# refresh-bio/colord

Measured on AMD Instinct MI355X. Metric: input Gbases/s + archive size vs ref, ONT 50 Gb at 1/2/4/8 MI355X, higher is better.
Workload: dtype u64

## Files before the change

### colord_amd/_native.py

```python
from __future__ import annotations
import ctypes as C
import os

os.environ.setdefault("GPU_MAX_HW_QUEUES", "32")
_HERE = os.path.dirname(os.path.abspath(__file__))
LIB_PATH = os.environ.get("COLORD_HIP_LIBRARY") or os.path.join(_HERE, "libcolord_hip.so")

CL_OK, CL_E_INVALID, CL_E_HIP, CL_E_CAPACITY, CL_E_NOMEM, CL_E_UNSUPPORTED, CL_E_MISMATCH = 0, -1, -2, -3, -4, -5, -6


class ColordHipError(RuntimeError):
    def __init__(self, status, msg):
        super().__init__(f"colord_hip error {status}: {msg}")
        self.status = status


class QualParams(C.Structure):
    _fields_ = [("mode", C.c_int32), ("source", C.c_int32), ("level", C.c_int32), ("n_fwd", C.c_uint32), ("fwd", C.c_uint32 * 8),
                ("n_rev", C.c_uint32), ("rev", C.c_uint32 * 8)]


class KmerStats(C.Structure):
    _fields_ = [("n_reads", C.c_uint64), ("tot_kmers", C.c_uint64), ("n_unique", C.c_uint64),
                ("n_unique_counted", C.c_uint64), ("total_count_filtered", C.c_uint64)]
# ... 32 lines not shown


class PileupSums(C.Structure):
    _fields_ = [("covered", C.c_uint64), ("match", C.c_uint64), ("sub", C.c_uint64), ("del_", C.c_uint64), ("ins", C.c_uint64), ("ins_unplaced", C.c_uint64), ("reads", C.c_uint64)]
    NAMES = ("covered", "match", "sub", "del", "ins", "ins_unplaced", "reads")

    def as_dict(self):
        return {k: int(getattr(self, f[0])) for k, f in zip(self.NAMES, self._fields_)}


KSPEC_EXACT = 4096
class KSpec(C.Structure):
    _fields_ = [("kmers", C.c_uint64), ("distinct", C.c_uint64), ("max_count", C.c_uint64), ("exact", C.c_uint64 * KSPEC_EXACT),
                ("big", C.c_uint64 * 33), ("big_mass", C.c_uint64 * 33)]

    as_dict = Report.as_dict


class SketchEntry(C.Structure):
    _fields_ = [("hash", C.c_uint64), ("count", C.c_uint64)]


class Sketch:

    def __init__(self, size: int, min_count: int):
        self.lib, self.h = load(), _P()
        st = self.lib.cl_sketch_create(size, min_count, C.byref(self.h))
        if st != CL_OK:
            raise ColordHipError(st, "cl_sketch_create failed")

    def close(self):
        if self.h:
            self.lib.cl_sketch_free(self.h)
            self.h = None

    def __del__(self):
        try:
            self.close()
        except Exception:
            pass

    def info(self) -> dict:
        size, mc, q, n = C.c_uint32(0), C.c_uint32(0), C.c_uint64(0), C.c_uint64(0)
        st = self.lib.cl_sketch_info(self.h, C.byref(size), C.byref(mc), C.byref(q), C.byref(n))
        if st != CL_OK:
            raise ColordHipError(st, "cl_sketch_info failed")
        return {"size": size.value, "min_count": mc.value, "qualifying": q.value, "n": n.value}

    def entries(self):
        import numpy as np
        n = self.info()["n"]
        buf = np.zeros((n, 2), np.uint64)
        st = self.lib.cl_sketch_entries(self.h, buf.ctypes.data if n else None, n)
        if st != CL_OK:
            raise ColordHipError(st, "cl_sketch_entries failed")
        return buf[:, 0].copy(), buf[:, 1].copy()

    def as_dict(self) -> dict:
        d = self.info()
        d["hash"], d["count"] = self.entries()
        return d

    def merge(self, hashes, counts, qualifying: int):
        import numpy as np
        h, c = np.asarray(hashes, np.uint64), np.asarray(counts, np.uint64)
        assert h.shape == c.shape and h.ndim == 1
        buf = np.ascontiguousarray(np.stack([h, c], axis=1))
        st = self.lib.cl_sketch_merge(self.h, buf.ctypes.data if len(h) else None, len(h), qualifying)
        if st != CL_OK:
            raise ColordHipError(st, "cl_sketch_merge refused the entries")
        return self


class Overlap(C.Structure):
    _fields_ = [(k, C.c_uint32) for k in ("q", "t", "qlen", "tlen", "qs", "qe", "ts", "te", "matches", "subst", "anchor_bases", "flags")]


_P = C.c_void_p
class CompressParams(C.Structure):
    _fields_ = [("k", C.c_uint32), ("f", C.c_uint32), ("ci", C.c_uint32), ("cs", C.c_uint32), ("c", C.c_uint32),
                ("anchor_len", C.c_uint32), ("min_part_alt", C.c_uint32), ("max_rec", C.c_uint32), ("min_anchors", C.c_uint32),
                ("level", C.c_int32), ("source", C.c_int32), ("sparse", C.c_int32),
                ("sparse_g", C.c_double), ("sparse_exponent", C.c_double),
                ("cost_mult", C.c_double), ("frac_always", C.c_double), ("frac_min", C.c_double), ("max_matches_mult", C.c_double)]


class CompressInfo(C.Structure):
    _fields_ = [(n, C.c_uint64) for n in ("n_reads", "n_bases", "tot_kmers", "n_kept_kmers", "n_refs", "n_anchors", "tuple_bytes", "dna_bytes", "qual_bytes")] + \
               [("sparse_range", C.c_uint32), ("pad", C.c_uint32)]


_EXCH_GATHER_HOST = C.CFUNCTYPE(C.c_int32, C.c_void_p, C.POINTER(C.c_uint64), C.c_uint32, C.POINTER(C.c_uint64))
_EXCH_A2AV = C.CFUNCTYPE(C.c_int32, C.c_void_p, C.c_void_p, C.POINTER(C.c_uint64), C.c_void_p, C.POINTER(C.c_uint64))
_EXCH_GATHERV = C.CFUNCTYPE(C.c_int32, C.c_void_p, C.c_void_p, C.c_uint64, C.c_void_p, C.POINTER(C.c_uint64))


class Exchange(C.Structure):
    _fields_ = [("user", C.c_void_p), ("rank", C.c_uint32), ("world", C.c_uint32),
                ("all_gather_host", _EXCH_GATHER_HOST), ("all_to_all_v", _EXCH_A2AV), ("all_gather_v", _EXCH_GATHERV)]


_SIG = {
    "cl_ctx_create": (C.c_int32, [C.c_int, C.POINTER(_P)]),
    "cl_ctx_destroy": (None, [_P]),
    "cl_last_error": (C.c_char_p, [_P]),
    "cl_ctx_stream": (_P, [_P]),
    "cl_ctx_last_kernel_ms": (C.c_int32, [_P, C.c_char_p, C.POINTER(C.c_double), C.POINTER(C.c_uint32)]),
    "cl_ctx_set_timing": (None, [_P, C.c_int]),
    "cl_ctx_set_verify": (None, [_P, C.c_int]),
    "cl_ctx_verified": (C.c_int32, [_P, C.POINTER(C.c_uint64), C.POINTER(C.c_uint64)]),
    "cl_ctx_gap_paths": (C.c_int32, [_P, C.POINTER(C.c_uint64), C.c_uint32]),
    "cl_ctx_set_verify_streams": (None, [_P, C.c_int]),
    "cl_ctx_verified_streams": (C.c_int32, [_P, C.POINTER(C.c_uint64), C.POINTER(C.c_uint64), C.POINTER(C.c_uint64)]),
    "cl_compressor_verified_streams": (C.c_int32, [_P, C.POINTER(C.c_uint64), C.POINTER(C.c_uint64), C.POINTER(C.c_uint64)]),
    "cl_ctx_set_digest": (None, [_P, C.c_int]),
    "cl_ctx_digest": (C.c_int32, [_P, C.POINTER(Digest), C.POINTER(Digest)]),
    "cl_compressor_digest": (C.c_int32, [_P, C.POINTER(Digest), C.POINTER(Digest)]),
    "cl_ctx_set_digest_values": (None, [_P, C.c_int]),
    "cl_ctx_digest_values": (C.c_int32, [_P, C.POINTER(Digest)]),
    "cl_compressor_digest_values": (C.c_int32, [_P, C.POINTER(Digest)]),
    "cl_digest_qual_values": (C.c_int32, [_P, C.POINTER(QualParams), _P, _P, _P, C.c_uint64, C.POINTER(Digest)]),
    "cl_qual_values": (C.c_int32, [_P, C.POINTER(QualParams), _P, _P, _P, _P, C.c_uint64]),
    "cl_qual_values_host": (C.c_int32, [C.POINTER(QualParams), _P, _P, C.c_uint64, _P]),
    "cl_digest_qual_values_host": (C.c_int32, [_P, _P, C.c_uint64, C.c_uint64, C.POINTER(Digest)]),
    "cl_report_clear": (None, [C.POINTER(Report)]),
    "cl_report_add": (None, [C.POINTER(Report), C.POINTER(Report)]),
    "cl_report_bases": (C.c_int32, [_P, _P, C.POINTER(Report)]),
    "cl_report_quals": (C.c_int32, [_P, C.POINTER(QualParams), _P, _P, _P, C.c_uint64, C.c_uint32, C.POINTER(Report)]),
    "cl_report_bases_host": (C.c_int32, [_P, _P, C.c_uint64, C.POINTER(Report)]),
    "cl_report_quals_host": (C.c_int32, [C.POINTER(QualParams), _P, _P, C.c_uint64, C.POINTER(Report)]),
    "cl_report_values_host": (C.c_int32, [_P, _P, C.c_uint64, C.POINTER(Report)]),
    "cl_ctx_set_report": (None, [_P, C.c_int]),
    "cl_ctx_report": (C.c_int32, [_P, C.POINTER(Report)]),
    "cl_compressor_report": (C.c_int32, [_P, C.POINTER(Report)]),
    "cl_edits_clear": (None, [C.POINTER(Edits)]),
    "cl_edits_add": (None, [C.POINTER(Edits), C.POINTER(Edits)]),
    "cl_edit_profile": (C.c_int32, [_P, _P, _P, _P, C.c_uint32, C.c_uint64, C.c_uint32, C.POINTER(Edits)]),
    "cl_edit_profile_host": (C.c_int32, [_P, _P, C.c_uint32, _P, _P, C.c_uint64, C.POINTER(Edits), C.POINTER(C.c_uint64), C.POINTER(C.c_uint32)]),
    "cl_edit_profile_error": (C.c_char_p, [C.c_uint32]),
    "cl_ctx_set_edit_profile": (None, [_P, C.c_int]),
    "cl_ctx_edit_profile": (C.c_int32, [_P, C.POINTER(Edits)]),
    "cl_compressor_edit_profile": (C.c_int32, [_P, C.POINTER(Edits)]),
    "cl_kspec_clear": (None, [C.POINTER(KSpec)]),
    "cl_kspec_add": (None, [C.POINTER(KSpec), C.POINTER(KSpec)]),
    "cl_kmer_spectrum_heads": (C.c_int32, [_P, _P, C.c_uint64, C.c_uint64, C.c_uint32, C.POINTER(KSpec)]),
    "cl_ctx_set_kmer_spectrum": (None, [_P, C.c_int]),
    "cl_ctx_kmer_spectrum": (C.c_int32, [_P, C.POINTER(KSpec)]),
    "cl_compressor_kmer_spectrum": (C.c_int32, [_P, C.POINTER(KSpec)]),
    "cl_sketch_hash": (C.c_uint64, [C.c_uint64]),
    "cl_sketch_create": (C.c_int32, [C.c_uint32, C.c_uint32, C.POINTER(_P)]),
    "cl_sketch_free": (None, [_P]),
    "cl_sketch_info": (C.c_int32, [_P, C.POINTER(C.c_uint32), C.POINTER(C.c_uint32), C.POINTER(C.c_uint64), C.POINTER(C.c_uint64)]),
    "cl_sketch_entries": (C.c_int32, [_P, _P, C.c_uint64]),
    "cl_sketch_merge": (C.c_int32, [_P, _P, C.c_uint64, C.c_uint64]),
    "cl_kmer_sketch_runs": (C.c_int32, [_P, _P, _P, C.c_uint64, C.c_uint64, C.c_uint32, _P]),
    "cl_ctx_set_kmer_sketch": (C.c_int32, [_P, C.c_int, C.c_uint32, C.c_uint32]),
    "cl_ctx_kmer_sketch": (C.c_int32, [_P, _P]),
    "cl_compressor_kmer_sketch": (C.c_int32, [_P, _P]),
    "cl_overlaps_of": (C.c_int32, [_P, _P, _P, _P, C.c_uint32, C.c_uint64, _P, C.c_uint32, C.c_uint32, _P, C.c_uint64, C.POINTER(C.c_uint64)]),
    "cl_overlaps_host": (C.c_int32, [_P, _P, C.c_uint32, _P, _P, C.c_uint64, C.c_uint64, _P, C.c_uint32, _P, C.c_uint64, C.POINTER(C.c_uint64), C.POINTER(C.c_uint64),
                                     C.POINTER(C.c_uint32)]),
    "cl_ctx_set_overlaps": (None, [_P, C.c_int]),
    "cl_ctx_overlaps": (C.c_int32, [_P, _P, C.c_uint64, C.POINTER(C.c_uint64)]),
    "cl_compressor_overlaps": (C.c_int32, [_P, _P, C.c_uint64, C.POINTER(C.c_uint64)]),
    "cl_mappings_lift": (C.c_int32, [_P, _P, C.c_uint64, _P, C.c_uint32, C.c_uint32, C.c_uint32, _P, C.c_uint64, C.POINTER(C.c_uint64)]),
    "cl_mappings_lift_host": (C.c_int32, [_P, C.c_uint64, _P, C.c_uint32, C.c_uint32, C.c_uint32, _P, C.c_uint64, C.POINTER(C.c_uint64), C.POINTER(C.c_uint64), C.POINTER(C.c_uint32)]),
    "cl_ctx_set_mappings": (None, [_P, C.c_int]),
    "cl_ctx_mappings": (C.c_int32, [_P, _P, C.c_uint64, C.POINTER(C.c_uint64)]),
    "cl_compressor_mappings": (C.c_int32, [_P, _P, C.c_uint64, C.POINTER(C.c_uint64)]),
    "cl_cigars_of": (C.c_int32, [_P, _P, _P, _P, C.c_uint32, C.c_uint32, C.c_uint32, _P, C.c_uint64, C.POINTER(C.c_uint64), _P, C.c_uint64, C.POINTER(C.c_uint64)]),
    "cl_cigars_host": (C.c_int32, [_P, _P, C.c_uint32, _P, _P, C.c_uint64, C.c_uint32, _P, C.c_uint64, C.POINTER(C.c_uint64), _P, C.c_uint64, C.POINTER(C.c_uint64),
                                   C.POINTER(C.c_uint64), C.POINTER(C.c_uint32)]),
    "cl_cigars_error": (C.c_char_p, [C.c_uint32]),
    "cl_ctx_set_cigars": (C.c_int32, [_P, C.c_int]),
    "cl_ctx_cigars": (C.c_int32, [_P, _P, C.c_uint64, C.POINTER(C.c_uint64), _P, C.c_uint64, C.POINTER(C.c_uint64)]),
    "cl_compressor_cigars": (C.c_int32, [_P, _P, C.c_uint64, C.POINTER(C.c_uint64), _P, C.c_uint64, C.POINTER(C.c_uint64)]),
    "cl_compressor_genome_geometry": (C.c_int32, [_P, _P, C.c_uint32, C.c_uint32, C.c_uint32]),
    "cl_pileup_create": (C.c_int32, [_P, _P, _P, C.c_uint32, C.c_uint32, C.c_uint32, C.POINTER(_P)]),
    "cl_pileup_free": (None, [_P]),
    "cl_pileup_positions": (C.c_uint64, [_P]),
    "cl_pileup_add": (C.c_int32, [_P, _P, _P, _P, C.c_uint32, C.c_uint32]),
    "cl_pileup_finish": (C.c_int32, [_P]),
    "cl_pileup_columns": (C.c_int32, [_P, C.c_uint64, C.c_uint64, _P]),
    "cl_pileup_sites": (C.c_int32, [_P, C.c_uint32, C.c_uint32, C.c_uint32, _P, C.c_uint64, C.POINTER(C.c_uint64)]),
    "cl_pileup_totals": (C.c_int32, [_P, C.POINTER(PileupSums)]),
    "cl_pileup_host": (C.c_int32, [_P, _P, C.c_uint32, _P, C.c_uint32, C.c_uint32, C.c_uint32, _P, _P, C.c_uint64, C.c_uint32, C.c_uint32, C.c_uint32, _P, _P, C.c_uint64,
                                   C.POINTER(C.c_uint64), C.POINTER(PileupSums), C.POINTER(C.c_uint64), C.POINTER(C.c_uint32)]),
    "cl_ctx_set_pileup": (None, [_P, C.c_int]),
    "cl_compressor_pileup": (C.c_int32, [_P, C.POINTER(_P)]),
    "cl_digest_bases": (C.c_int32, [_P, _P, C.c_uint64, C.POINTER(Digest)]),
    "cl_digest_quals": (C.c_int32, [_P, C.POINTER(QualParams), _P, _P, _P, C.c_uint64, C.POINTER(Digest)]),
    "cl_digest_bases_host": (C.c_int32, [_P, _P, C.c_uint64, C.c_uint64, C.POINTER(Digest)]),
    "cl_digest_bytes_host": (C.c_int32, [C.c_uint32, _P, _P, C.c_uint64, C.c_uint64, C.POINTER(Digest)]),
    "cl_qual_decoder_set_digest": (C.c_int32, [_P, C.c_int, C.c_uint64]),
    "cl_qual_decoder_digest": (C.c_int32, [_P, C.POINTER(Digest)]),
    "cl_es_expand": (C.c_int32, [_P, _P, _P, _P, _P, C.c_uint32, _P, C.c_uint64, _P, C.POINTER(C.c_uint64)]),
    "cl_es_verify": (C.c_int32, [_P, _P, _P, _P, _P, _P, C.POINTER(C.c_uint64), C.POINTER(C.c_uint32)]),
    "cl_compressor_verified": (C.c_int32, [_P, C.POINTER(C.c_uint64), C.POINTER(C.c_uint64)]),
    "cl_ctx_kernel_times": (C.c_int32, [_P, C.c_char_p, C.c_uint64, C.POINTER(C.c_uint64)]),
    "cl_reads_pack": (C.c_int32, [_P, _P, _P, C.c_uint32, C.c_int, C.POINTER(_P)]),
    "cl_reads_free": (None, [_P]),
    "cl_reads_count": (C.c_uint32, [_P]),
    "cl_reads_total_bases": (C.c_uint64, [_P]),
    "cl_reads_total_words": (C.c_uint64, [_P]),
    "cl_reads_packed": (_P, [_P]),
    "cl_reads_invalid": (_P, [_P]),
    "cl_reads_word_offsets": (_P, [_P]),
    "cl_reads_lengths": (_P, [_P]),
    "cl_reads_has_n": (_P, [_P]),
    "cl_reads_compact": (C.c_int32, [_P, _P, C.c_uint32, _P, C.c_uint64, C.POINTER(C.c_uint64)]),
    "cl_kmer_scan": (C.c_int32, [_P, _P, C.c_uint32, C.c_uint32, _P, C.c_uint64, C.POINTER(C.c_uint64)]),
    "cl_kmer_count_filter": (C.c_int32, [_P, _P, C.c_uint64, C.c_uint32, C.c_uint32, C.c_uint32, C.POINTER(_P), C.POINTER(KmerStats)]),
    "cl_kmer_set_create": (C.c_int32, [_P, _P, _P, C.c_uint64, C.c_uint32, C.POINTER(_P)]),
    "cl_kmer_set_free": (None, [_P]),
    "cl_kmer_set_size": (C.c_uint64, [_P]),
    "cl_kmer_set_keys": (_P, [_P]),
    "cl_kmer_set_counts": (_P, [_P]),
    "cl_kmer_set_check": (C.c_int32, [_P, _P, _P, C.c_uint64, _P]),
    "cl_accepted_kmers": (C.c_int32, [_P, _P, _P, C.c_uint32, C.c_uint32, C.POINTER(_P)]),
    "cl_kmer_lists_free": (None, [_P]),
    "cl_kmer_lists_reads": (C.c_uint32, [_P]),
    "cl_kmer_lists_total": (C.c_uint64, [_P]),
    "cl_kmer_lists_offsets": (_P, [_P]),
    "cl_kmer_lists_kmers": (_P, [_P]),
    "cl_kmer_lists_ids": (_P, [_P]),
    "cl_kmer_lists_pos": (_P, [_P]),
    "cl_ref_accept": (C.c_int32, [C.c_uint32, C.c_uint32, C.c_uint32, C.c_double, _P]),
    "cl_index_build": (C.c_int32, [_P, _P, _P, _P, C.c_uint32, C.c_uint32, C.POINTER(_P)]),
    "cl_index_entries_of": (C.c_int32, [_P, _P, _P, C.c_uint32, _P, _P, C.c_uint64, C.POINTER(C.c_uint64), _P, C.POINTER(C.c_uint32)]),
    "cl_index_build_pairs": (C.c_int32, [_P, _P, _P, _P, C.c_uint64, _P, C.c_uint32, C.c_uint32, C.c_uint32, C.c_uint32, C.POINTER(_P)]),
    "cl_index_free": (None, [_P]),
    "cl_index_n_refs": (C.c_uint32, [_P]),
    "cl_index_entries": (C.c_uint64, [_P]),
    "cl_index_ref_rank": (_P, [_P]),
    "cl_candidates": (C.c_int32, [_P, _P, _P, C.c_uint32, _P, _P, _P]),
    "cl_candidates_common": (C.c_int32, [_P, _P, _P, C.c_uint32, _P, _P, _P, _P, C.c_uint64, C.POINTER(C.c_uint64)]),
    "cl_qual_coder_create": (C.c_int32, [_P, C.POINTER(QualParams), C.POINTER(_P)]),
    "cl_qual_coder_ctx": (_P, [_P]),
    "cl_qual_coder_free": (None, [_P]),
    "cl_qual_coder_set_domain_symbols": (C.c_int32, [_P, C.c_uint64]),
    "cl_qual_coder_domains": (C.c_int32, [_P, _P, C.c_uint64, C.POINTER(C.c_uint64)]),
    "cl_qual_coder_model": (C.c_int32, [_P, C.c_uint32, C.c_uint64, _P, C.c_uint32, C.POINTER(C.c_uint32)]),
    "cl_qual_coder_groups": (C.c_int32, [_P, C.POINTER(C.c_uint64)]),
    "cl_compressor_set_qual_domain_symbols": (C.c_int32, [_P, C.c_uint64]),
    "cl_compressor_qual_domains": (C.c_int32, [_P, _P, C.c_uint64, C.POINTER(C.c_uint64)]),
    "cl_qual_decode_domains": (C.c_int32, [_P, C.POINTER(QualParams), _P, _P, _P, C.c_uint64, _P, _P, C.c_uint32, _P, C.c_uint32, C.c_uint32, _P, _P, C.c_uint64, _P, C.c_uint64]),
    "cl_qual_encode": (C.c_int32, [_P, _P, _P, _P, _P, _P, _P, C.c_uint32, _P, C.c_uint64, _P, C.POINTER(C.c_uint64)]),
    "cl_anchor_candidates": (C.c_int32, [_P, _P, _P, _P, _P, C.c_uint32, C.c_uint32, C.c_double, C.c_double, C.c_double, C.c_uint32, C.POINTER(_P)]),
    "cl_anchor_candidates_hifi": (C.c_int32, [_P, _P, _P, _P, _P, C.c_uint32, C.c_uint32, C.c_double, C.c_double, C.c_double, C.c_uint32, C.c_uint32, C.c_uint32, _P, _P, C.POINTER(_P)]),
    "cl_anchors_free": (None, [_P]),
    "cl_anchors_total": (C.c_uint64, [_P]),
    "cl_anchors_wave_tasks": (C.c_uint64, [_P]),
    "cl_anchors_wave_pairs": (C.c_uint64, [_P]),
    "cl_anchors_lane_tasks": (C.c_uint64, [_P]),
    "cl_anchors_lane_pairs": (C.c_uint64, [_P]),
    "cl_anchors_n_cands": (_P, [_P]),
    "cl_anchors_cands": (_P, [_P]),
    "cl_anchors_cand_offsets": (_P, [_P]),
    "cl_anchors_data": (_P, [_P]),
    "cl_encode_plain": (C.c_int32, [_P, _P, _P, C.c_uint64, _P, _P, C.POINTER(C.c_uint64)]),
    "cl_reads_select": (C.c_int32, [_P, _P, _P, C.POINTER(_P)]),
    "cl_reads_from_arena": (C.c_int32, [_P, _P, _P, _P, C.c_uint32, C.POINTER(_P)]),
    "cl_estimator_logs": (C.c_int32, [_P, _P, _P, C.c_uint64, _P]),
    "cl_es_flags": (C.c_int32, [_P, _P, _P, _P, _P, _P]),
    "cl_id_coder_create": (C.c_int32, [C.c_int32, C.POINTER(_P)]),
    "cl_id_coder_free": (None, [_P]),
    "cl_id_coder_error": (C.c_char_p, [_P]),
    "cl_id_encode_part": (C.c_int32, [_P, _P, _P, _P, C.c_uint32, _P, C.c_uint64, C.POINTER(C.c_uint64)]),
    "cl_compress_shard": (C.c_int32, [_P, C.POINTER(CompressParams), _P, _P, _P, _P, C.c_uint32, _P, C.c_uint32, _P, _P, _P, C.c_uint64, _P, _P, C.c_uint64, _P,
                                      C.POINTER(CompressInfo)]),
    "cl_candidates_at": (C.c_int32, [_P, _P, _P, _P, C.c_uint32, _P, _P, _P]),
    "cl_compressor_create": (C.c_int32, [_P, _P, C.POINTER(CompressParams), C.POINTER(QualParams), C.POINTER(Exchange), C.c_uint64, C.POINTER(_P)]),
    "cl_compressor_free": (None, [_P]),
    "cl_compressor_count_add": (C.c_int32, [_P, _P]),
    "cl_compressor_count_finish": (C.c_int32, [_P, C.POINTER(KmerStats)]),
    "cl_compressor_refs_add": (C.c_int32, [_P, _P]),
    "cl_compressor_refs_finish": (C.c_int32, [_P]),
    "cl_compressor_encode": (C.c_int32, [_P, _P, _P, _P, _P, C.c_uint32, _P, C.c_uint32, _P, C.c_uint64, _P, _P, C.c_uint64, _P, C.POINTER(CompressInfo)]),
    "cl_compressor_genome_add": (C.c_int32, [_P, _P]),
    "cl_compressor_pseudo_reads": (C.c_int32, [_P, _P]),
    "cl_genome_encode": (C.c_int32, [_P, _P, C.c_uint32, _P, C.c_uint64, C.POINTER(C.c_uint64)]),
    "cl_genome_decode": (C.c_int32, [_P, C.c_uint64, C.c_uint32, _P, C.c_uint64, _P, C.POINTER(C.c_uint64)]),
    "cl_genome_md5": (C.c_int32, [_P, _P, C.c_uint32, _P]),
    "cl_compressor_prepare": (C.c_int32, [_P, _P, _P, C.c_uint32]),
    "cl_compressor_prepare_parts": (C.c_int32, [_P, _P, _P, C.c_uint32, _P, C.c_uint32, _P, _P]),
    "cl_compressor_info": (C.c_int32, [_P, C.POINTER(KmerStats), C.POINTER(C.c_uint64), C.POINTER(C.c_uint64), C.POINTER(C.c_uint64), C.POINTER(C.c_uint32), C.POINTER(C.c_uint32)]),
    "cl_dna_decoder_create": (C.c_int32, [C.c_uint32, C.c_int32, C.c_uint32, C.c_uint32, C.c_int32, C.c_uint32, C.c_double, C.POINTER(_P)]),
    "cl_dna_decoder_free": (None, [_P]),
    "cl_dna_decoder_error": (C.c_char_p, [_P]),
    "cl_dna_decoder_add_ref": (C.c_int32, [_P, _P, C.c_uint32]),
    "cl_dna_decoder_new_domain": (C.c_int32, [_P]),
    "cl_dna_decode_part": (C.c_int32, [_P, _P, C.c_uint64, C.c_uint32, _P, C.c_uint64, _P, C.POINTER(C.c_uint64)]),
    "cl_qual_decoder_create": (C.c_int32, [C.POINTER(QualParams), C.POINTER(_P)]),
    "cl_qual_decoder_free": (None, [_P]),
    "cl_qual_decoder_new_domain": (C.c_int32, [_P]),
    "cl_qual_decode_part": (C.c_int32, [_P, _P, C.c_uint64, _P, _P, C.c_uint32, _P]),
    "cl_id_decoder_create": (C.c_int32, [C.c_int32, C.POINTER(_P)]),
    "cl_id_decoder_free": (None, [_P]),
    "cl_id_decode_part": (C.c_int32, [_P, _P, C.c_uint64, C.c_uint32, _P, C.c_uint64, _P, _P, C.POINTER(C.c_uint64)]),
    "cl_encode_reads": (C.c_int32, [_P, _P, _P, _P, C.c_uint32, C.c_uint32, C.c_uint32, C.c_uint32, C.c_double, _P, C.c_uint32, _P, C.c_uint64, _P, _P, C.POINTER(C.c_uint64)]),
    "cl_dna_coder_create": (C.c_int32, [_P, C.c_uint32, C.c_int32, C.c_uint32, C.POINTER(_P)]),
    "cl_dna_coder_free": (None, [_P]),
    "cl_dna_coder_model": (C.c_int32, [_P, C.c_uint32, C.c_uint64, _P]),
    "cl_dna_encode": (C.c_int32, [_P, _P, _P, _P, _P, _P, C.c_uint32, _P, C.c_uint32, _P, C.c_uint64, _P, C.POINTER(C.c_uint64)]),
    "cl_sort_u64": (C.c_int32, [_P, _P, C.c_uint64, C.c_uint32, C.c_uint32]),
    "cl_sort_u64_u32": (C.c_int32, [_P, _P, _P, C.c_uint64, C.c_uint32, C.c_uint32]),
    "cl_sort_u32": (C.c_int32, [_P, _P, C.c_uint64, C.c_uint32, C.c_uint32]),
    "cl_sort_u32_u32": (C.c_int32, [_P, _P, _P, C.c_uint64, C.c_uint32, C.c_uint32]),
    "cl_sort_swap_u32_u32": (C.c_int32, [_P, _P, _P, C.c_uint64, C.c_uint32, C.c_uint32, _P, _P]),
    "cl_sort_swap_u64_u32": (C.c_int32, [_P, _P, _P, C.c_uint64, C.c_uint32, C.c_uint32, _P, _P]),
    "cl_scan_u32": (C.c_int32, [_P, _P, C.c_uint64, C.POINTER(C.c_uint64)]),
    "cl_scan_u32_u64": (C.c_int32, [_P, _P, _P, C.c_uint64, C.POINTER(C.c_uint64)]),
    "cl_run_starts_u32": (C.c_int32, [_P, _P, C.c_uint64, C.c_uint32, _P, C.c_uint64, C.POINTER(C.c_uint64)]),
    "cl_run_starts_u64": (C.c_int32, [_P, _P, C.c_uint64, C.c_uint32, _P, C.c_uint64, C.POINTER(C.c_uint64)]),
}

_lib = None


def load():
    global _lib
    if _lib is None:
        if not os.path.exists(LIB_PATH):
            raise ColordHipError(CL_E_HIP, f"{LIB_PATH} is missing: run `make -C colord_amd/csrc` "
                                 "(or __graft_entry__.build()); there is no CPU fallback")
        lib = C.CDLL(LIB_PATH)
        for name, (res, args) in _SIG.items():
            fn = getattr(lib, name)
            fn.restype, fn.argtypes = res, args
        _lib = lib
    return _lib


def exported_names():
    return sorted(_SIG)
```

### colord_amd/csrc/capi.hip

```cpp
#include "common.hpp"
#include "objects.hpp"
#include "sketch.hpp"
#include <cmath>
#include <random>

extern "C" cl_status cl_ctx_create(int device, cl_ctx** out)
{
	if (!out) return CL_E_INVALID;
	*out = nullptr;
	int n = 0;
	hipError_t e = hipGetDeviceCount(&n);
	if (e != hipSuccess || n <= 0) { fprintf(stderr, "colord_hip: no HIP device available (%s)\n", hipGetErrorString(e)); return CL_E_HIP; }
	if (device < 0 || device >= n) return CL_E_INVALID;
	if (hipSetDevice(device) != hipSuccess) return CL_E_HIP;
	cl_ctx* c = new cl_ctx(device);
	if (hipStreamCreateWithFlags(&c->stream, hipStreamNonBlocking) != hipSuccess) { cl_ctx_destroy(c); return CL_E_HIP; }
	hipDeviceProp_t p;
	if (hipGetDeviceProperties(&p, device) == hipSuccess) c->n_cu = p.multiProcessorCount;
	*out = c;
	return CL_OK;
}
void cl_ctx_set_priority(cl_ctx* c, int level, int role)
{
	if (!c) return;
	(void)hipSetDevice(c->device);
	int least = 0, greatest = 0;
	if (hipDeviceGetStreamPriorityRange(&least, &greatest) != hipSuccess) { (void)hipGetLastError(); least = greatest = 0; }
	level = cl_role_level(role >= 0 ? role : c->role, level);
	const int prio = level > 0 ? greatest : level < 0 ? least : 0;
	const bool role_changes = role >= 0 && role < CL_N_ROLES && cl_cu_mask_cfg().on[role] && (role != c->role || !c->masked);
	if (role >= 0) c->role = role;
	if (prio == c->prio && !role_changes) return;
	c->prio = prio; c->masked = c->role < CL_N_ROLES && cl_cu_mask_cfg().on[c->role];
	auto drop_scan_ctl = [&](hipStream_t old) {
		auto it = c->scan_ctl.find((void*)old);
		if (it == c->scan_ctl.end()) return;
		if (it->second.p) c->pool.put(it->second.p, it->second.got, c->pool_id);
		c->scan_ctl.erase(it);
	};
	if (c->stream)
	{
		(void)hipStreamSynchronize(c->stream); drop_scan_ctl(c->stream); (void)hipStreamDestroy(c->stream); c->stream = nullptr;
		if (cl_stream_create(c, &c->stream) != hipSuccess) { (void)hipGetLastError(); (void)hipStreamCreateWithFlags(&c->stream, hipStreamNonBlocking); }
	}
	for (std::atomic<hipStream_t>* s : { &c->side, &c->side2, &c->side3 })
		if (hipStream_t old = s->load())
		{
			(void)hipStreamSynchronize(old); drop_scan_ctl(old); (void)hipStreamDestroy(old);
			hipStream_t ns = nullptr;
			if (cl_stream_create(c, &ns) != hipSuccess) { (void)hipGetLastError(); (void)hipStreamCreateWithFlags(&ns, hipStreamNonBlocking); }
			s->store(ns);
		}
}
namespace { __global__ void k_poison_check(const uint32_t* __restrict__ p, uint64_t n, unsigned long long* __restrict__ bad)
{
	uint64_t mine = 0;
	for (uint64_t i = (uint64_t)blockIdx.x * blockDim.x + threadIdx.x; i < n; i += (uint64_t)gridDim.x * blockDim.x) mine += p[i] != 0xCDCDCDCDu;
	if (mine) atomicAdd(bad, (unsigned long long)mine);
} }
void cl_ctx_poison(cl_ctx* c, void* p, uint64_t bytes)
{
	if (!c || !c->stream) return;
	(void)hipSetDevice(c->device);
	if (hipMemsetAsync(p, 0xCD, bytes, c->stream) != hipSuccess) { (void)hipGetLastError(); return; }
	(void)hipStreamSynchronize(c->stream);
}
uint64_t cl_pool_poison_check(void* p, uint64_t bytes)
{
	static unsigned long long* d_bad = nullptr;
	if (!d_bad && hipMalloc((void**)&d_bad, 8) != hipSuccess) { (void)hipGetLastError(); return 0; }
	(void)hipDeviceSynchronize();
	(void)hipMemset(d_bad, 0, 8);
	hipLaunchKernelGGL(k_poison_check, dim3(1024), dim3(256), 0, nullptr, (const uint32_t*)p, bytes / 4, d_bad);
	unsigned long long h = 0;
	if (hipGetLastError() != hipSuccess || hipMemcpy(&h, d_bad, 8, hipMemcpyDeviceToHost) != hipSuccess) { (void)hipGetLastError(); fprintf(stderr, "colord_hip: pool poison: the check itself failed\n"); return 0; }
	return h;
}
void cl_ctx_drain(cl_ctx* c)
{
	if (!c) return;
	(void)hipSetDevice(c->device);
	for (hipStream_t s : { c->stream, c->side.load(std::memory_order_acquire), c->side2.load(std::memory_order_acquire), c->side3.load(std::memory_order_acquire) }) if (s) (void)hipStreamSynchronize(s);
}
int cl_ctx_fence(cl_ctx* c, hipEvent_t* ev)
{
	if (!c) return 0;
	int n = 0;
	for (hipStream_t s : { c->stream, c->side.load(std::memory_order_acquire), c->side2.load(std::memory_order_acquire), c->side3.load(std::memory_order_acquire) }) if (s && n < 4) { if (hipEventRecord(ev[n], s) == hipSuccess) ++n; else (void)hipGetLastError(); }
	return n;
}
extern "C" void cl_ctx_destroy(cl_ctx* c)
{
	if (!c) return;
	for (cl_ctx* l : c->lanes) cl_ctx_destroy(l);
	c->lanes.clear();
	if (c->prep) { cl_ctx_destroy(c->prep); c->prep = nullptr; }
	if (c->qprep) { cl_ctx_destroy(c->qprep); c->qprep = nullptr; }
	(void)hipSetDevice(c->device);
	cl_ctx_drain(c);
	for (auto& kv : c->scan_ctl) if (kv.second.p) c->pool.put(kv.second.p, kv.second.got, c->pool_id);
	c->scan_ctl.clear();
	c->pool.drop_owner(c->pool_id);
	for (auto& p : c->pending) { (void)hipEventDestroy(p.second.first); (void)hipEventDestroy(p.second.second); }
	for (auto e : c->ev_pool) (void)hipEventDestroy(e);
	if (c->stream) (void)hipStreamDestroy(c->stream);
	for (std::atomic<hipStream_t>* s : { &c->side, &c->side2, &c->side3 }) if (hipStream_t x = s->load()) (void)hipStreamDestroy(x);
	if (c->inv_tab) (void)hipFree(c->inv_tab);
	if (c->slots_h) (void)hipHostFree(c->slots_h);
	delete c->report_acc;
	delete c->edits_acc;
	delete c->kspec_acc;
	delete c->sketch_acc;
	const int dev = c->device;
	delete c;
	cl_device_pool_release(dev);
}
extern "C" const char* cl_last_error(const cl_ctx* c) { return c ? c->err.c_str() : "null context"; }
extern "C" void* cl_ctx_stream(cl_ctx* c) { return c ? (void*)c->stream : nullptr; }
extern "C" void cl_ctx_set_timing(cl_ctx* c, int on) { if (c) c->timing = on != 0; }
extern "C" void cl_ctx_set_verify(cl_ctx* c, int on) { if (c) c->verify = on != 0; }
extern "C" cl_status cl_ctx_verified(const cl_ctx* c, uint64_t* reads, uint64_t* bases)
{
	if (!c) return CL_E_INVALID;
	uint64_t r = c->verified_reads.load(), b = c->verified_bases.load();
	for (const cl_ctx* l : c->lanes) { r += l->verified_reads.load(); b += l->verified_bases.load(); }
	if (reads) *reads = r;
	if (bases) *bases = b;
	return CL_OK;
}
extern "C" cl_status cl_ctx_gap_paths(const cl_ctx* c, uint64_t* out, uint32_t cap)
{
	if (!c || (!out && cap)) return CL_E_INVALID;
	for (uint32_t i = 0; i < cap && i < 11; ++i) out[i] = c->gap_paths[i];
	return CL_OK;
}
extern "C" cl_status cl_dna_coder_model(const cl_dna_coder* d, uint32_t family, uint64_t context, uint32_t* out)
{
	if (!d || !out) return CL_E_INVALID;
	return cl_dna_model_read(d, family, context, out);
}
extern "C" cl_status cl_qual_coder_model(const cl_qual_coder* q, uint32_t family, uint64_t context, uint32_t* out, uint32_t cap, uint32_t* n_out)
{
	if (!q || !out || !n_out) return CL_E_INVALID;
	return cl_qual_model_read(q, family, context, out, cap, n_out);
}
extern "C" void cl_ctx_set_verify_streams(cl_ctx* c, int on) { if (c) c->verify_streams = on != 0; }
extern "C" cl_status cl_ctx_verified_streams(const cl_ctx* c, uint64_t* parts, uint64_t* symbols, uint64_t* bytes)
{
	if (!c) return CL_E_INVALID;
	if (parts) *parts = c->verified_stream_parts.load();
	if (symbols) *symbols = c->verified_stream_symbols.load();
	if (bytes) *bytes = c->verified_stream_bytes.load();
	return CL_OK;
}
extern "C" cl_status cl_ctx_last_kernel_ms(const cl_ctx* c, const char* kernel, double* ms, uint32_t* launches)
{
	if (!c || !kernel) return CL_E_INVALID;
	auto it = c->times.find(kernel);
	if (it == c->times.end()) { if (ms) *ms = 0; if (launches) *launches = 0; return CL_E_INVALID; }
	if (ms) *ms = it->second.ms;
	if (launches) *launches = it->second.launches;
	return CL_OK;
}

extern "C" cl_status cl_ctx_kernel_times(cl_ctx* c, char* buf, uint64_t cap, uint64_t* needed)
{
	if (!c) return CL_E_INVALID;
	cl_timing_collect(c);
	std::string out;
	for (auto& kv : c->times) out += kv.first + "\t" + std::to_string(kv.second.ms) + "\t" + std::to_string(kv.second.launches) + "\t" + std::to_string(kv.second.bytes) + "\t" + std::to_string(kv.second.cells) + "\n";
	if (needed) *needed = out.size() + 1;
	if (!buf || cap < out.size() + 1) return CL_E_CAPACITY;
	memcpy(buf, out.c_str(), out.size() + 1);
	c->times.clear();
	return CL_OK;
}

extern "C" cl_status cl_ref_accept(uint32_t n_reads, uint32_t n_pseudo, uint32_t range, double exponent, uint8_t* h_out)
{
	if (!h_out || range == 0) return CL_E_INVALID;
	std::mt19937 mt;
	std::uniform_real_distribution<double> dist(0.0, 1.0);
	for (uint64_t i = 0; i < (uint64_t)n_reads + n_pseudo; ++i)
	{
		if (i < n_pseudo) { h_out[i] = 1; continue; }
		uint32_t range_no = (uint32_t)((i - n_pseudo) / range);
		double p = std::pow(1.0 / (range_no + 1ul), exponent);
		h_out[i] = dist(mt) <= p;
	}
	return CL_OK;
}

extern "C" cl_status cl_sort_u64(cl_ctx* ctx, uint64_t* d_keys, uint64_t n, uint32_t begin_bit, uint32_t end_bit)
{
	if (!ctx || (!d_keys && n)) return cl_fail(ctx, CL_E_INVALID, "cl_sort_u64: null argument");
	HIP_TRY(ctx, hipSetDevice(ctx->device));
	cl_timing_begin(ctx);
	cl_status s = dev_sort_pairs(ctx, d_keys, nullptr, n, begin_bit, end_bit);
	cl_timing_collect(ctx);
	return s;
}
extern "C" cl_status cl_sort_u64_u32(cl_ctx* ctx, uint64_t* d_keys, uint32_t* d_vals, uint64_t n, uint32_t begin_bit, uint32_t end_bit)
{
	if (!ctx || ((!d_keys || !d_vals) && n)) return cl_fail(ctx, CL_E_INVALID, "cl_sort_u64_u32: null argument");
	HIP_TRY(ctx, hipSetDevice(ctx->device));
	cl_timing_begin(ctx);
	cl_status s = dev_sort_pairs(ctx, d_keys, d_vals, n, begin_bit, end_bit);
	cl_timing_collect(ctx);
	return s;
}

extern "C" cl_status cl_scan_u32(cl_ctx* ctx, uint32_t* d_data, uint64_t n, uint64_t* h_total)
{
	if (!ctx || (!d_data && n)) return cl_fail(ctx, CL_E_INVALID, "cl_scan_u32: null argument");
	HIP_TRY(ctx, hipSetDevice(ctx->device));
	cl_timing_begin(ctx);
	cl_status s = dev_exclusive_scan_u32(ctx, d_data, n, h_total);
	hipError_t e = hipStreamSynchronize(ctx->stream);
	cl_timing_collect(ctx);
	if (s == CL_OK) HIP_TRY(ctx, e);
	return s;
}
extern "C" cl_status cl_scan_u32_u64(cl_ctx* ctx, const uint32_t* d_in, uint64_t* d_out, uint64_t n, uint64_t* h_total)
{
	if (!ctx || !d_out || (!d_in && n)) return cl_fail(ctx, CL_E_INVALID, "cl_scan_u32_u64: null argument");
	HIP_TRY(ctx, hipSetDevice(ctx->device));
	cl_timing_begin(ctx);
	cl_status s = dev_exclusive_scan_u64(ctx, d_in, d_out, n, h_total);
	hipError_t e = hipStreamSynchronize(ctx->stream);
	cl_timing_collect(ctx);
	if (s == CL_OK) HIP_TRY(ctx, e);
	return s;
}
extern "C" cl_status cl_run_starts_u32(cl_ctx* ctx, const uint32_t* d_keys, uint64_t n, uint32_t shift, uint32_t* d_seg, uint64_t seg_cap, uint64_t* h_n_runs)
{
	if (!ctx || !h_n_runs || ((!d_keys || !d_seg) && n)) return cl_fail(ctx, CL_E_INVALID, "cl_run_starts_u32: null argument");
	HIP_TRY(ctx, hipSetDevice(ctx->device));
	cl_timing_begin(ctx);
	cl_status s = dev_run_starts_u32(ctx, d_keys, n, shift, d_seg, seg_cap, h_n_runs);
	cl_timing_collect(ctx);
	return s;
}
extern "C" cl_status cl_run_starts_u64(cl_ctx* ctx, const uint64_t* d_keys, uint64_t n, uint32_t shift, uint32_t* d_seg, uint64_t seg_cap, uint64_t* h_n_runs)
{
	if (!ctx || !h_n_runs || ((!d_keys || !d_seg) && n)) return cl_fail(ctx, CL_E_INVALID, "cl_run_starts_u64: null argument");
	HIP_TRY(ctx, hipSetDevice(ctx->device));
	cl_timing_begin(ctx);
	cl_status s = dev_run_starts_u64(ctx, d_keys, n, shift, d_seg, seg_cap, h_n_runs);
	cl_timing_collect(ctx);
	return s;
}
extern "C" cl_status cl_sort_u32(cl_ctx* ctx, uint32_t* d_keys, uint64_t n, uint32_t begin_bit, uint32_t end_bit)
{
	return cl_sort_u32_u32(ctx, d_keys, nullptr, n, begin_bit, end_bit);
}
extern "C" cl_status cl_sort_u32_u32(cl_ctx* ctx, uint32_t* d_keys, uint32_t* d_vals, uint64_t n, uint32_t begin_bit, uint32_t end_bit)
{
	if (!ctx || (!d_keys && n)) return cl_fail(ctx, CL_E_INVALID, "cl_sort_u32_u32: null argument");
	HIP_TRY(ctx, hipSetDevice(ctx->device));
	cl_timing_begin(ctx);
	cl_status s = dev_sort_keys32_pairs(ctx, d_keys, d_vals, n, begin_bit, end_bit);
	cl_timing_collect(ctx);
	return s;
}
namespace {
template<typename K, typename Sort>
cl_status sort_swap_copy(cl_ctx* ctx, const char* who, const K* d_keys_in, const uint32_t* d_vals_in, uint64_t n, uint32_t begin_bit, uint32_t end_bit, K* d_keys_out, uint32_t* d_vals_out, Sort sort)
{
	if (!ctx || ((!d_keys_in || !d_vals_in || !d_keys_out || !d_vals_out) && n)) return cl_fail(ctx, CL_E_INVALID, std::string(who) + ": null argument");
	HIP_TRY(ctx, hipSetDevice(ctx->device));
	cl_timing_begin(ctx);
	DevBuf<K> keys; DEV_ALLOC(ctx, keys, n);
	DevBuf<uint32_t> vals; DEV_ALLOC(ctx, vals, n);
	if (n)
	{
		HIP_TRY(ctx, hipMemcpyAsync(keys.p, d_keys_in, n * sizeof(K), hipMemcpyDeviceToDevice, ctx->stream));
		HIP_TRY(ctx, hipMemcpyAsync(vals.p, d_vals_in, n * 4, hipMemcpyDeviceToDevice, ctx->stream));
	}
	cl_status s = sort(ctx, keys, vals, n, begin_bit, end_bit);
	if (s == CL_OK && n)
	{
		HIP_TRY(ctx, hipMemcpyAsync(d_keys_out, keys.p, n * sizeof(K), hipMemcpyDeviceToDevice, ctx->stream));
		HIP_TRY(ctx, hipMemcpyAsync(d_vals_out, vals.p, n * 4, hipMemcpyDeviceToDevice, ctx->stream));
	}
	hipError_t e = hipStreamSynchronize(ctx->stream);
	cl_timing_collect(ctx);
	if (s == CL_OK) HIP_TRY(ctx, e);
	return s;
}
}
extern "C" cl_status cl_sort_swap_u32_u32(cl_ctx* ctx, const uint32_t* d_keys_in, const uint32_t* d_vals_in, uint64_t n, uint32_t begin_bit, uint32_t end_bit, uint32_t* d_keys_out, uint32_t* d_vals_out)
{
	return sort_swap_copy<uint32_t>(ctx, "cl_sort_swap_u32_u32", d_keys_in, d_vals_in, n, begin_bit, end_bit, d_keys_out, d_vals_out, dev_sort_keys32_pairs_swap);
}
extern "C" cl_status cl_sort_swap_u64_u32(cl_ctx* ctx, const uint64_t* d_keys_in, const uint32_t* d_vals_in, uint64_t n, uint32_t begin_bit, uint32_t end_bit, uint64_t* d_keys_out, uint32_t* d_vals_out)
{
	return sort_swap_copy<uint64_t>(ctx, "cl_sort_swap_u64_u32", d_keys_in, d_vals_in, n, begin_bit, end_bit, d_keys_out, d_vals_out, dev_sort_pairs_swap);
}
```

### colord_amd/csrc/dna.hip

```cpp
#include "common.hpp"
#include <functional>
#include "objects.hpp"
#include "rc_dev.hpp"
#include "rc_check.hpp"
#include "es_format.hpp"
#include <algorithm>
#include <deque>
#include <thread>
#include <chrono>

namespace {
enum { F_READ_TYPE = 0, F_REV_COMP, F_SEEN, F_LEN_BITS, F_LEN_DATA, F_SYMBOLS, F_SYMBOLS_N, F_READ_ID, F_READ_ID_SHORT,
       F_ANCHOR_LEN, F_SKIP_LOCAL, F_SKIP_DISTANT, F_TUPLE_TYPE, N_FAM };
constexpr uint32_t MAX_ALT = 64;

struct FamTab {
	uint32_t n_sym[N_FAM], max_total[N_FAM], adder[N_FAM];
	uint32_t ctx_base[N_FAM + 1];
	uint64_t state_base[N_FAM + 1];
	uint32_t n_ctx[N_FAM];
	int32_t level, T, S;
	uint32_t sym_B;
	uint32_t max_alt;
	uint32_t long_run;
// ... 384 lines not shown
			break;
		case T_SUBST:
		{
			const uint32_t rs = ref_symbol & 3;
			const uint32_t sym = (rs == 0) ? (v1 == 0 ? 1u : v1 == 1 ? 2u : 3u) : (rs == 1) ? (v1 == 0 ? 0u : v1 == 1 ? 2u : 3u)
			                   : (rs == 2) ? (v1 == 0 ? 0u : v1 == 1 ? 1u : 3u) : (v1 == 0 ? 0u : v1 == 1 ? 1u : 2u);
			uint32_t shift = 2, c = 1;
			c += (uint32_t)(ctx_symbol & 0x3f) << shift; shift += 6;
			if (ft.level == 3) { c += (uint32_t)(((ctx_symbol >> 6) & 3) == ((ctx_symbol >> 4) & 3)) << shift; ++shift; }
			c += rs << shift; shift += 2;
			c += (uint32_t)(ctx_tuple & 07777) << shift;
			em(F_SYMBOLS, c, sym, (int)rs);
			ctx_symbol = ((ctx_symbol << 2) + sym) & mask_symbol; ++known;
			if (is_main) ++ref_pos; else ++alt_pos;
			break;
		}
		case T_SKIP:
		{
			const int32_t skip_len = (int32_t)v2;
			delta -= skip_len;
			if (!is_main && last_type == T_ALT_ID)
			{
				const int32_t mod = skip_len - (alt_slot >= 0 ? alt_pos_of[alt_slot] : 0);
				if (mod > 0) emit_skip_len(em, (uint32_t)mod, false);
				else { emit_skip_len(em, 0, false); emit_skip_len(em, (uint32_t)(-mod), false); }
			}
			else emit_skip_len(em, (uint32_t)skip_len, last_type != T_ALT_ID && last_type != T_NONE);
			if (is_main) ref_pos += v2; else alt_pos += v2;
			break;
		}
		case T_MAIN_REF:
			is_main = true;
			if (alt_slot >= 0) alt_pos_of[alt_slot] = (int32_t)alt_pos;
			delta = 0;
			break;
		default: break;
		}
		last_type = type;
	}
	em.finish();
	if (!WRITE)
	{
		hdr_counts[r] = em.count; counts[r] = em.count;
		if (t_idx != ntup - 1 && err) atomicOr(err, 2u);
	}
}

__global__ void k_read_flags(const uint8_t* __restrict__ es, const uint64_t* __restrict__ es_off, uint32_t r0, uint32_t r1, uint8_t* __restrict__ flag)
{
	uint32_t r = r0 + blockIdx.x * blockDim.x + threadIdx.x;
	if (r >= r1) return;
	uint32_t t = es[es_off[r]] >> 4;
	flag[r - r0] = t == T_START_PLAIN ? 0 : t == T_START_PLAIN_N ? 1 : 2;
}

__global__ __launch_bounds__(256) void k_fill_sidx(const uint64_t* __restrict__ sym_off, uint64_t s0, uint32_t r0, uint32_t r1, TripLayoutDev lay, uint32_t* __restrict__ sidx)
{
	const uint32_t r = r0 + blockIdx.x * 4 + (threadIdx.x >> 6);
	if (r >= r1) return;
	const uint32_t lane = threadIdx.x & 63;
	const uint64_t a = sym_off[r] - s0, b = sym_off[r + 1] - s0;
	if (a == b) return;
	const uint32_t part = part_of_read(lay, r), pl = lay.rank ? lay.rank[part] : part;
	const uint64_t gb = lay.group_base[pl >> 6], p0 = lay.part_sym_start[part];
	for (uint64_t i = a + lane; i < b; i += 64) sidx[i] = (uint32_t)trip_slot(gb, pl & 63, i - p0);
}
template<typename K>
__global__ __launch_bounds__(256) void k_dna_plain(const FamTab* __restrict__ ftp, const uint8_t* __restrict__ es, const uint64_t* __restrict__ es_off,
                                                  const uint32_t* __restrict__ es_ntup, const uint8_t* __restrict__ read_flag, const uint32_t* __restrict__ hdr_counts,
                                                  const uint64_t* __restrict__ sym_off, uint32_t r0, uint32_t r1, K* __restrict__ key)
{
	const uint32_t r = r0 + blockIdx.x * 4 + (threadIdx.x >> 6);
	if (r >= r1) return;
	const uint32_t fl = read_flag[r - r0];
	if (fl == 2) return;
	const FamTab& ft = *ftp;
	const uint32_t lane = threadIdx.x & 63;
	const uint8_t* b = es + es_off[r] + 1;
	const uint32_t len = es_ntup[r] - 1;
	const uint64_t off = sym_off[r - r0] + hdr_counts[r - r0];
	const uint32_t S2 = 2 * ft.S; const uint32_t mask = (1u << S2) - 1;
	const uint32_t fam = fl == 0 ? F_SYMBOLS : F_SYMBOLS_N;
	const uint32_t cbase = ft.ctx_base[fam];
	for (uint32_t i = lane; i < len; i += 64)
	{
		uint32_t ctx = mask;
		if (fl == 0)
		{
			const uint32_t n = i < (uint32_t)ft.S ? i : (uint32_t)ft.S;
			for (uint32_t t = n; t >= 1; --t) ctx = ((ctx << 2) + (b[i - t] & 3u)) & mask;
			ctx <<= 2;
		}
		else
		{
			const uint32_t n = i < 4 ? i : 4;
			for (uint32_t t = n; t >= 1; --t) ctx = ((ctx << 4) + (b[i - t] & 0xfu)) & mask;
		}
		key[off + i] = KeyFmt<K>::make(cbase + ctx, b[i] & 0xfu);
	}
}


constexpr uint32_t LONG_RUN = 1u << 19;
struct LongRun { uint32_t s, e, fam, gctx; uint64_t step0, group0, epoch0; uint32_t epoch_cap, pad; };
template<int NS> struct EpochRec { uint32_t start, tot; uint32_t st[NS]; uint32_t cnt0[NS]; };
__device__ inline uint32_t find_run(const LongRun* runs, uint32_t n_runs, uint64_t step)
{
	uint32_t lo = 0, hi = n_runs;
	while (hi - lo > 1) { const uint32_t mid = (lo + hi) >> 1; if (runs[mid].step0 <= step) lo = mid; else hi = mid; }
	return lo;
}
template<typename K>
__global__ void k_long_find(const uint32_t* __restrict__ seg_start, uint32_t n_seg, const K* __restrict__ skey, const FamTab* __restrict__ ftp, LongRun* __restrict__ runs , uint32_t cap, uint32_t* __restrict__ n_runs )
{
	const uint32_t sg = blockIdx.x * blockDim.x + threadIdx.x;
	if (sg >= n_seg) return;
	const uint32_t s = seg_start[sg], e = seg_start[sg + 1];
	const FamTab& ft = *ftp;
	if (e - s < ft.long_run) return;
	const uint32_t gctx = KeyFmt<K>::ctx(skey[s]);
	uint32_t fam = 0;
	for (uint32_t f = 1; f < N_FAM; ++f) if (gctx >= ft.ctx_base[f]) fam = f;
	if (ft.n_sym[fam] > 32) return;
	const uint32_t which = ft.n_sym[fam] > 8 ? 1u : 0u;
	const uint32_t i = atomicAdd(n_runs + which, 1u);
	if (i < cap) { LongRun r; r.s = s; r.e = e; r.fam = fam; r.gctx = gctx; r.step0 = r.group0 = r.epoch0 = 0; r.epoch_cap = 0; r.pad = 0; runs[which * cap + i] = r; }
}
template<int NS, typename K>
__global__ __launch_bounds__(256) void k_long_hist(const LongRun* __restrict__ runs, uint32_t n_runs, uint64_t n_groups, const K* __restrict__ skey,
                                                  uint32_t* __restrict__ step_pfx, uint32_t* __restrict__ group_tot)
{
	const uint64_t g = ((uint64_t)blockIdx.x * blockDim.x + threadIdx.x) >> 6; const uint32_t lane = threadIdx.x & 63;
	if (g >= n_groups) return;
	uint32_t lo = 0, hi = n_runs;
	while (hi - lo > 1) { const uint32_t mid = (lo + hi) >> 1; if (runs[mid].group0 <= g) lo = mid; else hi = mid; }
	const LongRun R = runs[lo];
	const uint64_t gl = g - R.group0;
	const uint32_t smask = key_sym_mask(R.fam);
	uint32_t c[NS];
#pragma unroll
	for (int a = 0; a < NS; ++a) c[a] = 0;
	for (uint32_t k = 0; k < 64; ++k)
	{
		const uint64_t j = (uint64_t)R.s + (gl * 64 + k) * 64 + lane;
		const bool valid = j < R.e;
		const uint32_t sym = valid ? (uint32_t)skey[j] & smask : 0xffu;
#pragma unroll
		for (uint32_t a = 0; a < NS; ++a) { const uint32_t n = (uint32_t)__popcll(__ballot(sym == a)); if (lane == k) c[a] = n; }
	}
	const uint64_t n_steps = ((uint64_t)(R.e - R.s) + 63) / 64;
	const uint64_t step = R.step0 + gl * 64 + lane;
#pragma unroll
	for (uint32_t a = 0; a < NS; ++a)
	{
		const uint32_t incl = wave_incl_scan(c[a]);
		if (gl * 64 + lane < n_steps) step_pfx[step * NS + a] = incl - c[a];
		if (lane == 63) group_tot[g * NS + a] = incl;
	}
}
template<int NS>
__global__ __launch_bounds__(64) void k_long_groups(const LongRun* __restrict__ runs, uint32_t n_runs, uint32_t* __restrict__ group_tot )
{
	const uint32_t r = blockIdx.x, lane = threadIdx.x;
	if (r >= n_runs) return;
	const LongRun R = runs[r];
	const uint64_t n_steps = ((uint64_t)(R.e - R.s) + 63) / 64, n_groups = (n_steps + 63) / 64;
	uint32_t carry[NS];
#pragma unroll
	for (int a = 0; a < NS; ++a) carry[a] = 0;
	for (uint64_t g0 = 0; g0 < n_groups; g0 += 64)
	{
		const uint64_t g = g0 + lane; const bool valid = g < n_groups;
#pragma unroll
		for (uint32_t a = 0; a < NS; ++a)
		{
			const uint32_t v = valid ? group_tot[(R.group0 + g) * NS + a] : 0u;
			const uint32_t incl = wave_incl_scan(v);
			if (valid) group_tot[(R.group0 + g) * NS + a] = carry[a] + incl - v;
			carry[a] += __shfl(incl, 63);
		}
	}
}
template<int NS, typename K>
__device__ inline uint32_t long_prefix(const LongRun& R, const K* skey, const uint32_t* step_pfx, const uint32_t* group_pfx, uint32_t x, uint32_t lane)
{
	const uint32_t smask = key_sym_mask(R.fam);
	const uint64_t step = x >> 6; const uint32_t off = x & 63;
	const uint32_t a = lane & (NS - 1);
	uint32_t v = group_pfx[(R.group0 + (step >> 6)) * NS + a] + (step * 64 < (uint64_t)(R.e - R.s) || off ? step_pfx[(R.step0 + step) * NS + a] : 0u);
	if (x == R.e - R.s && off == 0)
	{
		const uint64_t last = step - 1;
		const uint64_t j = (uint64_t)R.s + last * 64 + lane; const uint32_t sym = j < R.e ? (uint32_t)skey[j] & smask : 0xffu;
		uint32_t mine = 0;
#pragma unroll
		for (uint32_t b = 0; b < NS; ++b) { const uint32_t n = (uint32_t)__popcll(__ballot(sym == b)); if (a == b) mine = n; }
		return group_pfx[(R.group0 + (last >> 6)) * NS + a] + step_pfx[(R.step0 + last) * NS + a] + mine;
	}
	if (off)
	{
		const uint64_t j = (uint64_t)R.s + step * 64 + lane; const uint32_t sym = j < R.e ? (uint32_t)skey[j] & smask : 0xffu;
		const uint64_t below = (1ULL << off) - 1;
		uint32_t mine = 0;
#pragma unroll
		for (uint32_t b = 0; b < NS; ++b) { const uint32_t n = (uint32_t)__popcll(__ballot(sym == b) & below); if (a == b) mine = n; }
		v += mine;
	}
	return v;
}
template<int NS, typename K>
__global__ __launch_bounds__(64) void k_long_epochs(const FamTab* __restrict__ ftp, const LongRun* __restrict__ runs, uint32_t n_runs, const K* __restrict__ skey,
                                                   const uint32_t* __restrict__ step_pfx, const uint32_t* __restrict__ group_pfx, uint32_t* __restrict__ state,
                                                   EpochRec<NS>* __restrict__ epochs, uint32_t* __restrict__ n_epochs, uint32_t* __restrict__ group_epoch, uint32_t* __restrict__ err)
{
	const uint32_t r = blockIdx.x, lane = threadIdx.x;
	if (r >= n_runs) return;
	const LongRun R = runs[r];
	const FamTab& ft = *ftp;
	const uint32_t n_sym = ft.n_sym[R.fam], max_total = ft.max_total[R.fam], adder = ft.adder[R.fam];
	uint32_t* sp = state + ft.state_base[R.fam] + (uint64_t)(R.gctx - ft.ctx_base[R.fam]) * (n_sym + 1);
	const uint32_t L = R.e - R.s;
	uint32_t st = lane < n_sym ? sp[lane] : 0u, tot = sp[n_sym];
	uint32_t cnt0 = 0, p = 0, ne = 0;
	EpochRec<NS>* E = epochs + R.epoch0;
	for (;;)
	{
		if (ne >= R.epoch_cap) { if (lane == 0) atomicOr(err, 8u); break; }
		if (lane < NS) { E[ne].st[lane] = st; E[ne].cnt0[lane] = cnt0; }
		if (lane == 0) { E[ne].start = p; E[ne].tot = tot; }
		++ne;
		const uint32_t rr = (max_total - tot + adder - 1) / adder;
		if ((uint64_t)p + rr > L) break;
		p += rr;
		const uint32_t c1 = long_prefix<NS, K>(R, skey, step_pfx, group_pfx, p, lane);
		st += adder * (c1 - cnt0); cnt0 = c1;
		tot += adder * rr;
		while (tot >= max_total)
		{
			st = (st + 1) / 2;
			uint32_t sm = lane < NS ? st : 0u;
			for (int o = NS / 2; o; o >>= 1) sm += __shfl_xor(sm, o);
			tot = __shfl(sm, 0);
		}
		if (p == L) { if (lane < NS && ne < R.epoch_cap) { E[ne].st[lane] = st; E[ne].cnt0[lane] = cnt0; } if (lane == 0 && ne < R.epoch_cap) { E[ne].start = p; E[ne].tot = tot; } ++ne; break; }
	}
	const uint32_t cl = long_prefix<NS, K>(R, skey, step_pfx, group_pfx, L, lane);
	if (p < L) { st += adder * (cl - cnt0); tot += adder * (L - p); }
	if (lane < n_sym) sp[lane] = st;
	if (lane == 0) { sp[n_sym] = tot; n_epochs[r] = ne; }
	__builtin_amdgcn_s_waitcnt(0);
	__builtin_amdgcn_fence(__ATOMIC_SEQ_CST, "workgroup");
	const uint64_t n_groups = (((uint64_t)L + 63) / 64 + 63) / 64;
	for (uint64_t g0 = 0; g0 < n_groups; g0 += 64)
	{
		const uint64_t g = g0 + lane;
		if (g >= n_groups) continue;
		const uint32_t pos = (uint32_t)(g * 4096);
		uint32_t lo = 0, hi = ne;
		while (hi - lo > 1) { const uint32_t mid = (lo + hi) >> 1; if (E[mid].start <= pos) lo = mid; else hi = mid; }
		group_epoch[R.group0 + g] = lo;
	}
}
template<int NS, typename K>
__global__ __launch_bounds__(256) void k_long_apply(const LongRun* __restrict__ runs, uint32_t n_runs, uint64_t n_steps, const K* __restrict__ skey, const uint32_t* __restrict__ sval,
                                                   const uint32_t* __restrict__ step_pfx, const uint32_t* __restrict__ group_pfx, const EpochRec<NS>* __restrict__ epochs,
                                                   const uint32_t* __restrict__ n_epochs, const uint32_t* __restrict__ group_epoch, const FamTab* __restrict__ ftp, triple_t* __restrict__ trip)
{
	const uint64_t step = ((uint64_t)blockIdx.x * blockDim.x + threadIdx.x) >> 6; const uint32_t lane = threadIdx.x & 63;
	if (step >= n_steps) return;
	const uint32_t ri = find_run(runs, n_runs, step);
	const LongRun R = runs[ri];
	const uint32_t adder = ftp->adder[R.fam];
	const uint64_t sl = step - R.step0;
	const uint32_t x0 = (uint32_t)(sl * 64), x = x0 + lane;
	const uint64_t j = (uint64_t)R.s + x; const bool valid = j < R.e;
	uint32_t sym = 0xffu, e1 = 15u, e2 = 15u;
	if (valid) key_decode(R.fam, KeyFmt<K>::payload(skey[j]), sym, e1, e2);
	uint64_t m[NS];
#pragma unroll
	for (uint32_t a = 0; a < NS; ++a) m[a] = __ballot(sym == a);
	const EpochRec<NS>* E = epochs + R.epoch0; const uint32_t ne = n_epochs[ri];
	uint32_t e = group_epoch[R.group0 + (sl >> 6)];
	while (e + 1 < ne && E[e + 1].start <= x0) ++e;
	uint32_t me = e;
	while (me + 1 < ne && E[me + 1].start <= x) ++me;
	if (!valid) return;
	const EpochRec<NS>& ep = E[me];
	const uint64_t lt = (1ULL << lane) - 1;
	uint32_t cum = 0, freq = 0, excl = 0;
#pragma unroll
	for (uint32_t a = 0; a < NS; ++a)
	{
		const uint32_t pre = group_pfx[(R.group0 + (sl >> 6)) * NS + a] + step_pfx[step * NS + a] + (uint32_t)__popcll(m[a] & lt);
		const uint32_t v = ep.st[a] + adder * (pre - ep.cnt0[a]);
		const bool ex = NS <= 8 && (a == e1 || a == e2);
		if (ex) excl += v;
		if (a < sym && !ex) cum += v;
		if (a == sym) freq = v;
	}
	trip[sval[j]] = pack_triple(cum, freq, ep.tot + adder * (x - ep.start) - excl);
}

template<typename K>
__global__ __launch_bounds__(256) void k_dna_evolve(const FamTab* __restrict__ ftp, const K* __restrict__ skey, const uint32_t* __restrict__ sval,
                                                   const uint32_t* __restrict__ seg_start, uint32_t n_seg, uint32_t* __restrict__ state, triple_t* __restrict__ trip)
{
	__shared__ uint32_t s_cnt[4][256];
	__shared__ uint32_t s_pre[4][256];
	const uint32_t w = threadIdx.x >> 6, lane = threadIdx.x & 63;
	const uint32_t sg = blockIdx.x * 4 + w;
	if (sg >= n_seg) return;
	const uint32_t s = seg_start[sg], e = seg_start[sg + 1];
	const FamTab& ft = *ftp;
	const uint32_t gctx = KeyFmt<K>::ctx(skey[s]);
	uint32_t fam = 0;
	for (uint32_t f = 1; f < N_FAM; ++f) if (gctx >= ft.ctx_base[f]) fam = f;
	const uint32_t n_sym = ft.n_sym[fam], max_total = ft.max_total[fam], adder = ft.adder[fam];
	uint32_t* sp = state + ft.state_base[fam] + (uint64_t)(gctx - ft.ctx_base[fam]) * (n_sym + 1);
	const uint64_t lt = (1ULL << lane) - 1;
	if (n_sym <= 8)
	{
		if (e - s >= ft.long_run) return;
		uint32_t st[8]; uint32_t tot = sp[n_sym];
#pragma unroll
		for (uint32_t a = 0; a < 8; ++a) st[a] = a < n_sym ? sp[a] : 0u;
		for (uint32_t j0 = s; j0 < e; j0 += 64)
		{
			const uint32_t j = j0 + lane; const bool valid = j < e;
			uint32_t sym = 0xffu, e1 = 15u, e2 = 15u;
			if (valid) key_decode(fam, KeyFmt<K>::payload(skey[j]), sym, e1, e2);
			const uint32_t dst = valid ? sval[j] : 0u;
			uint64_t m[8];
#pragma unroll
			for (uint32_t a = 0; a < 8; ++a) m[a] = __ballot(valid && sym == a);
			const uint32_t cnt = (e - j0) < 64 ? (e - j0) : 64;
			uint32_t start = 0;
			while (start < cnt)
			{
				const uint32_t r = (max_total - tot + adder - 1) / adder;
				const uint32_t now = (cnt - start) < r ? (cnt - start) : r;
				const uint64_t win = (now == 64 ? ~0ULL : ((1ULL << now) - 1)) << start;
				if (lane >= start && lane < start + now)
				{
					const uint64_t before = lt & win;
					uint32_t cum = 0, freq = 0, excl = 0;
#pragma unroll
					for (uint32_t a = 0; a < 8; ++a)
					{
						const uint32_t v = st[a] + adder * (uint32_t)__popcll(m[a] & before);
						const bool ex = a == e1 || a == e2;
						if (ex) excl += v;
						if (a < sym && !ex) cum += v;
						if (a == sym) freq = v;
					}
					trip[dst] = pack_triple(cum, freq, tot + adder * (lane - start) - excl);
				}
#pragma unroll
				for (uint32_t a = 0; a < 8; ++a) st[a] += adder * (uint32_t)__popcll(m[a] & win);
				tot += adder * now;
				while (tot >= max_total)
				{
					tot = 0;
#pragma unroll
					for (uint32_t a = 0; a < 8; ++a) { st[a] = (st[a] + 1) / 2; tot += st[a]; }
				}
				start += now;
			}
		}
		if (lane == 0)
		{
			for (uint32_t a = 0; a < n_sym; ++a) sp[a] = st[a];
			sp[n_sym] = tot;
		}
		return;
	}
	if (n_sym <= 32 && e - s >= ft.long_run) return;
	uint32_t* cnt = s_cnt[w]; uint32_t* pre = s_pre[w];
#pragma unroll
	for (uint32_t t = 0; t < 4; ++t) { uint32_t a = lane * 4 + t; cnt[a] = a < n_sym ? sp[a] : 0u; }
	uint32_t tot = sp[n_sym];
	auto rebuild_prefix = [&]() {
		uint32_t v0 = cnt[lane * 4], v1 = cnt[lane * 4 + 1], v2 = cnt[lane * 4 + 2], v3 = cnt[lane * 4 + 3];
		uint32_t sum = v0 + v1 + v2 + v3;
		uint32_t ex = wave_incl_scan(sum) - sum;
		pre[lane * 4] = ex; pre[lane * 4 + 1] = ex + v0; pre[lane * 4 + 2] = ex + v0 + v1; pre[lane * 4 + 3] = ex + v0 + v1 + v2;
		__builtin_amdgcn_wave_barrier();
	};
	__builtin_amdgcn_wave_barrier();
	rebuild_prefix();
	for (uint32_t j0 = s; j0 < e; j0 += 64)
	{
		const uint32_t j = j0 + lane; const bool valid = j < e;
		const uint32_t sym = valid ? KeyFmt<K>::payload(skey[j]) : 0u;
		const uint32_t dst = valid ? sval[j] : 0u;
		const uint32_t n_here = (e - j0) < 64 ? (e - j0) : 64;
		uint32_t start = 0;
		while (start < n_here)
		{
			const uint32_t r = (max_total - tot + adder - 1) / adder;
			const uint32_t now = (n_here - start) < r ? (n_here - start) : r;
			uint32_t less = 0, eq = 0;
			for (uint32_t l = start; l < start + now; ++l)
			{
				const uint32_t o = __builtin_amdgcn_readlane(sym, l);
				if (l < lane) { less += (o < sym) ? 1u : 0u; eq += (o == sym) ? 1u : 0u; }
			}
			const bool mine = lane >= start && lane < start + now;
			if (mine) trip[dst] = pack_triple(pre[sym] + adder * less, cnt[sym] + adder * eq, tot + adder * (lane - start));
			__builtin_amdgcn_wave_barrier();
			if (mine) atomicAdd(&cnt[sym], adder);
			__builtin_amdgcn_wave_barrier();
			tot += adder * now;
			while (tot >= max_total)
			{
				uint32_t sum = 0;
#pragma unroll
				for (uint32_t t = 0; t < 4; ++t) { uint32_t a = lane * 4 + t; if (a < n_sym) { uint32_t v = (cnt[a] + 1) / 2; cnt[a] = v; sum += v; } }
				tot = wave_sum(sum);
			}
			__builtin_amdgcn_wave_barrier();
			rebuild_prefix();
			start += now;
		}
	}
#pragma unroll
	for (uint32_t t = 0; t < 4; ++t) { uint32_t a = lane * 4 + t; if (a < n_sym) sp[a] = cnt[a]; }
	if (lane == 0) sp[n_sym] = tot;
}

__global__ void k_init_fam_state(const FamTab* __restrict__ ftp, uint32_t fam, uint32_t* __restrict__ state)
{
	const FamTab& ft = *ftp;
	const uint32_t ns = ft.n_sym[fam];
	const uint64_t n = (uint64_t)ft.n_ctx[fam] * (ns + 1);
	for (uint64_t i = (uint64_t)blockIdx.x * blockDim.x + threadIdx.x; i < n; i += (uint64_t)gridDim.x * blockDim.x)
		state[ft.state_base[fam] + i] = (i % (ns + 1)) == ns ? ns : 1u;
}
__global__ void k_gather_bytes2(const uint8_t* __restrict__ src, const uint64_t* __restrict__ src_off, const uint64_t* __restrict__ dst_off,
                                const uint64_t* __restrict__ size, uint8_t* __restrict__ dst)
{
	const uint32_t p = blockIdx.x;
	const uint64_t n = size[p]; const uint8_t* s = src + src_off[p]; uint8_t* d = dst + dst_off[p];
	for (uint64_t i = threadIdx.x; i < n; i += blockDim.x) d[i] = s[i];
}
__global__ void k_last_types(const uint8_t* __restrict__ flag, uint32_t n, uint32_t prev, uint32_t* __restrict__ out)
{
	uint32_t v = prev;
	uint32_t start = n > 4 ? n - 4 : 0;
	for (uint32_t i = start; i < n; ++i) v = ((v << 2) + flag[i]) & 0xff;
	*out = v;
}
}

struct DnaGroupPrep {
	uint32_t p0 = 0, p1 = 0, r0 = 0, r1 = 0; uint64_t s0 = 0, n_syms = 0, n_seg = 0, trip_words = 0;
	std::vector<uint32_t> rank, plen_r;
	DevBuf<uint64_t> d_gbase; DevBuf<uint32_t> d_plen;
	DevBuf<uint32_t> sidx, seg;
	struct LongPrep { uint32_t n_runs = 0; uint64_t steps = 0, groups = 0, eps = 0; DevBuf<LongRun> runs; DevBuf<uint32_t> step_pfx, group_pfx; } lp[2];
	bool long_ready = false;
};
struct DnaWalked {
	const uint8_t* d_es = nullptr; uint32_t n_reads = 0;
	uint32_t prev_types_in = 0, cur_read_id_in = 0, prev_types_out = 0;
	DevBuf<uint8_t> rflag; DevBuf<uint32_t> hdr; DevBuf<uint64_t> sym_off, key; DevBuf<uint32_t> key32; bool narrow = false;
	std::vector<uint64_t> h_sym_off;
	bool presorted = false; std::vector<uint32_t> part_bounds; std::vector<std::unique_ptr<DnaGroupPrep>> groups;
};
struct cl_dna_coder {
	cl_ctx* ctx = nullptr;
	FamTab ft;
	DevBuf<FamTab> d_ft;
	DevBuf<uint32_t> state;
	uint32_t ctx_bits = 0; bool narrow = false;
	uint32_t cur_read_id = 0;
	uint32_t prev_types = 0;
	uint32_t next_read_id = 0, next_prev_types = 0; bool next_valid = false;
	std::unique_ptr<DnaWalked> ahead;
	std::function<cl_status()> before_tail;
	std::deque<std::unique_ptr<struct DnaEvolved>> evolved;
	uint32_t ahead_prev_types = 0, ahead_read_id = 0;
	std::vector<hipStream_t> cstreams; uint32_t next_cstream = 0;
	~cl_dna_coder();
};

extern "C" cl_status cl_dna_coder_create(cl_ctx* ctx, uint32_t max_alt_refs, int32_t level, uint32_t start_read_id, cl_dna_coder** out)
{
	if (!ctx || !out) return cl_fail(ctx, CL_E_INVALID, "cl_dna_coder_create: null argument");
	if (level < 1 || level > 3 || max_alt_refs < 1 || max_alt_refs > MAX_ALT) return cl_fail(ctx, CL_E_INVALID, "cl_dna_coder_create: level 1..3, 1 <= max_alt_refs <= 64");
	HIP_TRY(ctx, hipSetDevice(ctx->device));
	cl_dna_coder* D = new cl_dna_coder(); D->ctx = ctx; D->cur_read_id = start_read_id;
	std::unique_ptr<cl_dna_coder> guard(D);
	FamTab& f = D->ft; memset(&f, 0, sizeof(f));
	f.level = level; f.max_alt = max_alt_refs;
	f.T = level == 3 ? 4 : level == 2 ? 3 : 2;
	f.S = level == 3 ? 8 : level == 2 ? 7 : 5;
	f.sym_B = level == 3 ? 24 : level == 2 ? 23 : 22;
	f.long_run = LONG_RUN;
	if (const char* lr = getenv("COLORD_HIP_LONG_RUN")) f.long_run = (uint32_t)std::max(64, atoi(lr));
	f.walk_chunk = WALK_CHUNK; f.walk_warm = WALK_WARM;
	if (const char* v = getenv("COLORD_HIP_WALK_CHUNK")) f.walk_chunk = (uint32_t)std::min(1 << 20, std::max(32, atoi(v)));
	if (const char* v = getenv("COLORD_HIP_WALK_WARM")) f.walk_warm = (uint32_t)std::max(0, atoi(v));
	f.walk_warm = std::min(f.walk_warm, f.walk_chunk / 2);
	auto set = [&](int i, uint32_t ns, uint32_t mt, uint32_t ad, uint32_t nc) { f.n_sym[i] = ns; f.max_total[i] = mt; f.adder[i] = ad; f.n_ctx[i] = nc; };
	set(F_READ_TYPE, 3, 1u << 15, 1, 256);
	set(F_REV_COMP, 2, 1u << 15, 1, 16);
	set(F_SEEN, 2, 1u << 15, 1, MAX_ALT + 1);
	set(F_LEN_BITS, 32, 1u << 18, 8, 1);
	set(F_LEN_DATA, 256, 1u << 18, 8, 512);
	set(F_SYMBOLS, 4, 1u << 10, 1, 1u << (f.sym_B + 1));
	set(F_SYMBOLS_N, 5, 1u << 10, 1, 1u << 16);
	set(F_READ_ID, 256, 1u << 13, 1, 2048);
	set(F_READ_ID_SHORT, max_alt_refs, 1u << 13, 1, MAX_ALT + 1);
	set(F_ANCHOR_LEN, 24, 1u << 15, 1, 1u << 17);
	set(F_SKIP_LOCAL, 256, 1u << 15, 1, 1u << 14);
	set(F_SKIP_DISTANT, 256, 1u << 15, 1, 256);
	set(F_TUPLE_TYPE, 8, 1u << 15, 1, 1u << (3 * f.T + 10));
	uint64_t cb = 0, sb = 0;
	for (int i = 0; i < N_FAM; ++i) { f.ctx_base[i] = (uint32_t)cb; f.state_base[i] = sb; cb += f.n_ctx[i]; sb += (uint64_t)f.n_ctx[i] * (f.n_sym[i] + 1); }
	f.ctx_base[N_FAM] = (uint32_t)cb; f.state_base[N_FAM] = sb;
	if (cb >= (1ull << 32)) return cl_fail(ctx, CL_E_UNSUPPORTED, "cl_dna_coder_create: context space too large");
	D->ctx_bits = 1; while ((1ull << D->ctx_bits) < cb) ++D->ctx_bits;
	D->narrow = D->ctx_bits + 8 <= 32 && !getenv("COLORD_HIP_DNA_WIDE_KEYS");
	DEV_ALLOC(ctx, D->d_ft, 1);
	HIP_TRY(ctx, hipMemcpyAsync(D->d_ft.p, &f, sizeof(f), hipMemcpyHostToDevice, ctx->stream));
	DEV_ALLOC(ctx, D->state, sb);
	for (uint32_t i = 0; i < N_FAM; ++i) LAUNCH(ctx, k_init_fam_state, 2048, 256, (const FamTab*)D->d_ft.p, i, D->state.p);
	HIP_TRY(ctx, hipGetLastError());
	HIP_TRY(ctx, hipStreamSynchronize(ctx->stream));
	*out = guard.release();
	return CL_OK;
}
extern "C" void cl_dna_coder_free(cl_dna_coder* d) { delete d; }

namespace {
struct SideSync { hipStream_t s = nullptr; ~SideSync() { if (s) (void)hipStreamSynchronize(s); } };
struct PendingGroup {
	DevBuf<triple_t> trip; DevBuf<uint64_t> d_gbase, d_out_off, d_size, d_dst_off; DevBuf<uint32_t> d_plen; DevBuf<uint8_t> tmp;
	std::vector<uint64_t> out_off; std::vector<uint32_t> rank; uint32_t p0 = 0, np = 0; uint64_t n_syms = 0;
	hipStream_t stream = nullptr;
	SideSync sync;
};
}
struct DnaEvolved {
	const uint8_t* d_es = nullptr; uint32_t n_reads = 0, prev_types_in = 0, read_id_in = 0, prev_types_out = 0;
	std::vector<uint32_t> part_bounds;
	std::vector<std::unique_ptr<PendingGroup>> groups;
};
cl_dna_coder::~cl_dna_coder() { evolved.clear(); for (hipStream_t s : cstreams) (void)hipStreamDestroy(s); }

namespace {
cl_status dna_walk(cl_ctx* ctx, cl_dna_coder* D, const cl_reads* refs, const uint8_t* d_es, const uint64_t* d_es_off, const uint32_t* d_es_ntuples, uint32_t n_reads,
                   uint32_t prev_types, uint32_t cur_read_id, DnaWalked& W)
{
	const FamTab& f = D->ft;
	RefStore R{ refs->packed.p, refs->word_off.p, refs->lens.p, refs->n_reads };
	W.d_es = d_es; W.n_reads = n_reads; W.prev_types_in = prev_types; W.cur_read_id_in = cur_read_id;
	DevBuf<uint8_t>& rflag = W.rflag; DevBuf<uint32_t>& hdr = W.hdr; DevBuf<uint64_t>& sym_off = W.sym_off; std::vector<uint64_t>& h_sym_off = W.h_sym_off;
	W.narrow = D->narrow;
	DEV_ALLOC(ctx, rflag, (uint64_t)n_reads + 1); DEV_ALLOC(ctx, hdr, (uint64_t)n_reads + 1); DEV_ALLOC(ctx, sym_off, (uint64_t)n_reads + 1);
	DevBuf<uint32_t> err; DEV_ALLOC(ctx, err, 1);
	HIP_TRY(ctx, hipMemsetAsync(err.p, 0, 4, ctx->stream));
	h_sym_off.assign((size_t)n_reads + 1, 0);
	if (n_reads)
	{
		uint64_t total_syms = 0, h_eb[2] = { 0, 0 };
		HIP_TRY(ctx, hipMemcpyAsync(&h_eb[0], d_es_off, 8, hipMemcpyDeviceToHost, ctx->stream));
		HIP_TRY(ctx, hipMemcpyAsync(&h_eb[1], d_es_off + n_reads, 8, hipMemcpyDeviceToHost, ctx->stream));
		HIP_TRY(ctx, hipStreamSynchronize(ctx->stream));
		DevBuf<uint64_t> chunk_off; DEV_ALLOC(ctx, chunk_off, (uint64_t)n_reads + 1);
		DevBuf<WalkCk> cks; uint64_t n_chunks = 0;
		{
			DevBuf<uint32_t> counts; DEV_ALLOC(ctx, counts, n_reads);
			LAUNCH(ctx, k_read_flags, grid_for(n_reads, 256), 256, d_es, d_es_off, 0u, n_reads, rflag.p);
			LAUNCH(ctx, k_walk_chunks, grid_for(n_reads, 256), 256, d_es_ntuples, (const uint8_t*)rflag.p, n_reads, f.walk_chunk, counts.p);
			CL_TRY(dev_exclusive_scan_u64(ctx, counts.p, chunk_off.p, n_reads, &n_chunks));
			if (n_chunks >= (1ull << 32)) return cl_fail(ctx, CL_E_UNSUPPORTED, "cl_dna_encode: too many tuples in one call");
			DEV_ALLOC(ctx, cks, n_chunks);
			LAUNCHB_NAMED(ctx, "k_dna_walk<false>", (double)(h_eb[1] - h_eb[0]) + 8.0 * n_reads + (double)n_chunks * sizeof(WalkCk), (k_dna_walk<false, uint32_t>), grid_for(n_reads, WALK_LPW), 64,
				(const FamTab*)D->d_ft.p, R, d_es, d_es_off, d_es_ntuples, (const uint8_t*)rflag.p, n_reads,
				prev_types, cur_read_id, (const uint64_t*)chunk_off.p, cks.p, (uint32_t)n_chunks, counts.p, hdr.p, (const uint64_t*)nullptr, (uint32_t*)nullptr, err.p, 0u);
			HIP_TRY(ctx, hipGetLastError());
			CL_TRY(dev_exclusive_scan_u64(ctx, counts.p, sym_off.p, n_reads, &total_syms));
		}
		HIP_TRY(ctx, hipMemcpy(h_sym_off.data(), sym_off.p, ((uint64_t)n_reads + 1) * 8, hipMemcpyDeviceToHost));
		uint32_t herr0 = 0;
		HIP_TRY(ctx, hipMemcpy(&herr0, err.p, 4, hipMemcpyDeviceToHost));
		if (herr0 & 2) return cl_fail(ctx, CL_E_INVALID, "cl_dna_encode: the tuple count of a read does not match its stream");
		if (herr0) return cl_fail(ctx, CL_E_UNSUPPORTED, "cl_dna_encode: a read uses more than 64 alternative references");
		if (W.narrow)
		{
			DEV_ALLOC(ctx, W.key32, total_syms);
			LAUNCHB_NAMED(ctx, "k_dna_walk<true>", total_syms * 5.0, (k_dna_walk<true, uint32_t>), grid_for(n_chunks, WALK_LPW), 64,
				(const FamTab*)D->d_ft.p, R, d_es, d_es_off, d_es_ntuples, (const uint8_t*)rflag.p, n_reads,
				prev_types, cur_read_id, (const uint64_t*)chunk_off.p, cks.p, (uint32_t)n_chunks, (uint32_t*)nullptr, (uint32_t*)nullptr, (const uint64_t*)sym_off.p, W.key32.p, err.p, 1u);
			LAUNCH_NAMED(ctx, "k_dna_plain", (k_dna_plain<uint32_t>), grid_for(n_reads, 4), 256, (const FamTab*)D->d_ft.p, d_es, d_es_off, d_es_ntuples, (const uint8_t*)rflag.p, (const uint32_t*)hdr.p,
				(const uint64_t*)sym_off.p, 0u, n_reads, W.key32.p);
		}
		else
		{
			DEV_ALLOC(ctx, W.key, total_syms);
			LAUNCHB_NAMED(ctx, "k_dna_walk<true>", total_syms * 9.0, (k_dna_walk<true, uint64_t>), grid_for(n_chunks, WALK_LPW), 64,
				(const FamTab*)D->d_ft.p, R, d_es, d_es_off, d_es_ntuples, (const uint8_t*)rflag.p, n_reads,
				prev_types, cur_read_id, (const uint64_t*)chunk_off.p, cks.p, (uint32_t)n_chunks, (uint32_t*)nullptr, (uint32_t*)nullptr, (const uint64_t*)sym_off.p, W.key.p, err.p, 1u);
			LAUNCH_NAMED(ctx, "k_dna_plain", (k_dna_plain<uint64_t>), grid_for(n_reads, 4), 256, (const FamTab*)D->d_ft.p, d_es, d_es_off, d_es_ntuples, (const uint8_t*)rflag.p, (const uint32_t*)hdr.p,
				(const uint64_t*)sym_off.p, 0u, n_reads, W.key.p);
		}
		HIP_TRY(ctx, hipGetLastError());
	}
	{
		DevBuf<uint32_t> lt; DEV_ALLOC(ctx, lt, 1);
		LAUNCH(ctx, k_last_types, 1, 1, (const uint8_t*)rflag.p, n_reads, prev_types, lt.p);
		HIP_TRY(ctx, hipGetLastError());
		HIP_TRY(ctx, hipMemcpyAsync(&W.prev_types_out, lt.p, 4, hipMemcpyDeviceToHost, ctx->stream));
		HIP_TRY(ctx, hipStreamSynchronize(ctx->stream));
	}
	return CL_OK;
}
}

namespace {
template<typename K>
cl_status dna_long_prepare(cl_ctx* ctx, cl_dna_coder* D, const K* gkey, uint64_t n_syms, DnaGroupPrep& G)
{
	const FamTab& f = D->ft;
	const uint32_t RUN_CAP = (uint32_t)std::max<uint64_t>(4096, n_syms / f.long_run + 2);
	DevBuf<LongRun> runs; DEV_ALLOC(ctx, runs, 2 * RUN_CAP);
	DevBuf<uint32_t> n_runs; DEV_ALLOC(ctx, n_runs, 2);
	HIP_TRY(ctx, hipMemsetAsync(n_runs.p, 0, 8, ctx->stream));
	LAUNCH_NAMED(ctx, "k_long_find", (k_long_find<K>), grid_for(G.n_seg, 256), 256, (const uint32_t*)G.seg.p, (uint32_t)G.n_seg, gkey, (const FamTab*)D->d_ft.p, runs.p, RUN_CAP, n_runs.p);
	uint32_t nlr2[2] = { 0, 0 };
	HIP_TRY(ctx, hipMemcpyAsync(nlr2, n_runs.p, 8, hipMemcpyDeviceToHost, ctx->stream));
	HIP_TRY(ctx, hipStreamSynchronize(ctx->stream));
	if (nlr2[0] > RUN_CAP || nlr2[1] > RUN_CAP) return cl_fail(ctx, CL_E_UNSUPPORTED, "cl_dna_encode: more than 4096 long context runs in one group");
	for (int which = 0; which < 2; ++which)
	{
		DnaGroupPrep::LongPrep& L = G.lp[which];
		const uint32_t nlr = nlr2[which], NS = which ? 32 : 8;
		L.n_runs = nlr; L.steps = L.groups = L.eps = 0;
		if (!nlr) continue;
		std::vector<LongRun> h(nlr);
		HIP_TRY(ctx, hipMemcpy(h.data(), runs.p + (uint64_t)which * RUN_CAP, nlr * sizeof(LongRun), hipMemcpyDeviceToHost));
		std::sort(h.begin(), h.end(), [](const LongRun& a, const LongRun& b) { return a.s < b.s; });
		for (auto& r : h)
		{
			const uint64_t Ln = r.e - r.s, ns = (Ln + 63) / 64, ngp = (ns + 63) / 64;
			const uint64_t half = f.max_total[r.fam] / 2 / f.adder[r.fam];
			r.step0 = L.steps; r.group0 = L.groups; r.epoch0 = L.eps; r.epoch_cap = (uint32_t)(Ln / (half > 80 ? half - 40 : 1) + 8);
			L.steps += ns; L.groups += ngp; L.eps += r.epoch_cap;
		}
		DEV_ALLOC(ctx, L.runs, nlr);
		HIP_TRY(ctx, hipMemcpyAsync(L.runs.p, h.data(), nlr * sizeof(LongRun), hipMemcpyHostToDevice, ctx->stream));
		DEV_ALLOC(ctx, L.step_pfx, (L.steps + 1) * NS); DEV_ALLOC(ctx, L.group_pfx, (L.groups + 1) * NS);
		const LongRun* cr = L.runs.p;
		if (which == 0)
		{
			LAUNCHB_NAMED(ctx, "k_long_hist<8>", L.steps * 64.0 * sizeof(K), (k_long_hist<8, K>), grid_for(L.groups * 64, 256), 256, cr, nlr, L.groups, gkey, L.step_pfx.p, L.group_pfx.p);
			LAUNCH(ctx, (k_long_groups<8>), nlr, 64, cr, nlr, L.group_pfx.p);
		}
		else
		{
			LAUNCHB_NAMED(ctx, "k_long_hist<32>", L.steps * 64.0 * sizeof(K), (k_long_hist<32, K>), grid_for(L.groups * 64, 256), 256, cr, nlr, L.groups, gkey, L.step_pfx.p, L.group_pfx.p);
			LAUNCH(ctx, (k_long_groups<32>), nlr, 64, cr, nlr, L.group_pfx.p);
		}
		HIP_TRY(ctx, hipGetLastError());
		HIP_TRY(ctx, hipStreamSynchronize(ctx->stream));
	}
	G.long_ready = true;
	return CL_OK;
}
}

namespace {
cl_status dna_group_prepare(cl_ctx* ctx, cl_dna_coder* D, DnaWalked& W, uint32_t p0, const uint32_t* h_part_bounds, uint32_t n_parts, DnaGroupPrep& G)
{
	const std::vector<uint64_t>& h_sym_off = W.h_sym_off;
	const uint64_t GROUP_SYMS = 5ull << 28;
	uint32_t p1 = p0; const uint32_t r0 = h_part_bounds[p0];
	while (p1 < n_parts)
	{
		const uint64_t pl = h_sym_off[h_part_bounds[p1 + 1]] - h_sym_off[h_part_bounds[p1]];
		if (pl >= (1ull << 31) - 64) return cl_fail(ctx, CL_E_UNSUPPORTED, "cl_dna_encode: one part has >= 2^31 symbols");
		if (p1 > p0 && h_sym_off[h_part_bounds[p1 + 1]] - h_sym_off[r0] >= GROUP_SYMS) break;
		++p1;
	}
	const uint32_t r1 = h_part_bounds[p1], nr = r1 - r0, np = p1 - p0, ng = (np + 63) / 64;
	const uint64_t s0 = h_sym_off[r0], n_syms = h_sym_off[r1] - s0;
	G.p0 = p0; G.p1 = p1; G.r0 = r0; G.r1 = r1; G.s0 = s0; G.n_syms = n_syms;
	std::vector<uint64_t> sym_start(np + 1);
	std::vector<uint32_t> plen(np), pfirst(np + 1);
	for (uint32_t p = 0; p <= np; ++p) { pfirst[p] = h_part_bounds[p0 + p]; sym_start[p] = h_sym_off[pfirst[p]] - s0; }
	for (uint32_t p = 0; p < np; ++p) plen[p] = (uint32_t)(sym_start[p + 1] - sym_start[p]);
	std::vector<uint32_t> order(np); std::vector<uint32_t>& rank = G.rank; std::vector<uint32_t>& plen_r = G.plen_r;
	rank.resize(np); plen_r.resize(np);
	for (uint32_t p = 0; p < np; ++p) order[p] = p;
	std::stable_sort(order.begin(), order.end(), [&](uint32_t a, uint32_t b) { return plen[a] > plen[b]; });
	for (uint32_t i = 0; i < np; ++i) { rank[order[i]] = i; plen_r[i] = plen[order[i]]; }
	std::vector<uint64_t> gbase(ng + 1, 0);
	for (uint32_t g = 0; g < ng; ++g) gbase[g + 1] = gbase[g] + trip_group_words(plen_r[g * 64]);
	if (gbase[ng] >= (1ull << 32)) return cl_fail(ctx, CL_E_UNSUPPORTED, "cl_dna_encode: group too large for 32-bit triple indices");
	G.trip_words = gbase[ng];
	DevBuf<uint64_t> d_sym_start; DevBuf<uint32_t> d_pfirst, d_rank;
	DEV_ALLOC(ctx, d_rank, np);
	HIP_TRY(ctx, hipMemcpyAsync(d_rank.p, rank.data(), np * 4, hipMemcpyHostToDevice, ctx->stream));
	DEV_ALLOC(ctx, d_sym_start, np + 1); DEV_ALLOC(ctx, G.d_gbase, ng + 1); DEV_ALLOC(ctx, G.d_plen, np); DEV_ALLOC(ctx, d_pfirst, np + 1);
	HIP_TRY(ctx, hipMemcpyAsync(d_sym_start.p, sym_start.data(), (np + 1) * 8, hipMemcpyHostToDevice, ctx->stream));
	HIP_TRY(ctx, hipMemcpyAsync(G.d_gbase.p, gbase.data(), (ng + 1) * 8, hipMemcpyHostToDevice, ctx->stream));
	HIP_TRY(ctx, hipMemcpyAsync(G.d_plen.p, plen_r.data(), np * 4, hipMemcpyHostToDevice, ctx->stream));
	HIP_TRY(ctx, hipMemcpyAsync(d_pfirst.p, pfirst.data(), (np + 1) * 4, hipMemcpyHostToDevice, ctx->stream));
	TripLayoutDev lay{ d_pfirst.p, d_sym_start.p, G.d_gbase.p, np, d_rank.p };
	if (n_syms)
	{
		DEV_ALLOC(ctx, G.sidx, n_syms);
		LAUNCHB(ctx, n_syms * 4.0, k_fill_sidx, grid_for(nr, 4), 256, (const uint64_t*)W.sym_off.p, s0, r0, r1, lay, G.sidx.p);
		HIP_TRY(ctx, hipGetLastError());
		const uint32_t cbits = D->ctx_bits;
		const uint64_t seg_cap = std::min<uint64_t>(n_syms, D->ft.ctx_base[N_FAM]) + 1;
		DEV_ALLOC(ctx, G.seg, seg_cap);
		if (W.narrow)
		{
			if (s0 == 0 && W.key32.n == n_syms) CL_TRY(dev_sort_keys32_pairs_swap(ctx, W.key32, G.sidx, n_syms, 8, 8 + cbits));
			else CL_TRY(dev_sort_keys32_pairs(ctx, W.key32.p + s0, G.sidx.p, n_syms, 8, 8 + cbits));
			CL_TRY(dev_run_starts_u32(ctx, W.key32.p + s0, n_syms, 8, G.seg.p, seg_cap, &G.n_seg));
			CL_TRY(dna_long_prepare<uint32_t>(ctx, D, W.key32.p + s0, n_syms, G));
		}
		else
		{
			if (s0 == 0 && W.key.n == n_syms) CL_TRY(dev_sort_pairs_swap(ctx, W.key, G.sidx, n_syms, 8, 8 + cbits));
			else CL_TRY(dev_sort_pairs(ctx, W.key.p + s0, G.sidx.p, n_syms, 8, 8 + cbits));
			CL_TRY(dev_run_starts_u64(ctx, W.key.p + s0, n_syms, 8, G.seg.p, seg_cap, &G.n_seg));
			CL_TRY(dna_long_prepare<uint64_t>(ctx, D, W.key.p + s0, n_syms, G));
		}
	}
	HIP_TRY(ctx, hipStreamSynchronize(ctx->stream));
	return CL_OK;
}
}

cl_status cl_dna_prepare_batch(cl_ctx* ctx, cl_dna_coder* D, const cl_reads* refs, const uint8_t* d_es, const uint64_t* d_es_off, const uint32_t* d_es_ntuples, uint32_t n_reads,
                               uint32_t prev_types, uint32_t read_id, const uint32_t* h_part_bounds, uint32_t n_parts, DnaWalked** out, uint32_t* prev_types_out)
{
	if (!ctx || !D || !refs || !d_es || !d_es_off || !d_es_ntuples || !n_reads || !out) return CL_E_INVALID;
	HIP_TRY(ctx, hipSetDevice(ctx->device));
	auto W = std::make_unique<DnaWalked>();
	CL_TRY(dna_walk(ctx, D, refs, d_es, d_es_off, d_es_ntuples, n_reads, prev_types, read_id, *W));
	if (h_part_bounds && n_parts && h_part_bounds[0] == 0 && h_part_bounds[n_parts] == n_reads)
	{
		W->part_bounds.assign(h_part_bounds, h_part_bounds + n_parts + 1);
		for (uint32_t p0 = 0; p0 < n_parts; )
		{
			auto G = std::make_unique<DnaGroupPrep>();
			CL_TRY(dna_group_prepare(ctx, D, *W, p0, h_part_bounds, n_parts, *G));
			p0 = G->p1;
			W->groups.push_back(std::move(G));
		}
		W->presorted = true;
	}
	if (prev_types_out) *prev_types_out = W->prev_types_out;
	*out = W.release();
	return CL_OK;
}
namespace {
__global__ void k_batch_types(const uint8_t* __restrict__ es, const uint64_t* __restrict__ es_off, uint32_t n_reads, uint64_t es_bytes, uint32_t prev, unsigned long long* __restrict__ out)
{
	uint32_t v = prev; bool ok = true;
	const uint32_t start = n_reads > 4 ? n_reads - 4 : 0;
	for (uint32_t r = start; r < n_reads; ++r)
	{
		const uint64_t a = es_off[r], b = es_off[r + 1];
		if (a >= b || b > es_bytes) { ok = false; break; }
		const uint32_t t = es[a] >> 4;
		v = ((v << 2) + (t == T_START_PLAIN ? 0u : t == T_START_PLAIN_N ? 1u : 2u)) & 0xff;
	}
	*out = ok ? (unsigned long long)v : ~0ull;
}
}
cl_status cl_dna_batch_types(cl_ctx* ctx, const uint8_t* d_es, const uint64_t* d_es_off, uint32_t n_reads, uint64_t es_bytes, uint32_t prev_types, uint32_t* out)
{
	if (!ctx || !d_es || !d_es_off || !out) return CL_E_INVALID;
	HIP_TRY(ctx, hipSetDevice(ctx->device));
	uint64_t* hs = nullptr; uint64_t* ds = nullptr;
	HIP_TRY(ctx, cl_slot(ctx, 1, &hs, &ds));
	LAUNCH(ctx, k_batch_types, 1, 1, d_es, d_es_off, n_reads, es_bytes, prev_types, (unsigned long long*)ds);
	HIP_TRY(ctx, hipGetLastError());
	HIP_TRY(ctx, hipStreamSynchronize(ctx->stream));
	const uint64_t v = *(volatile uint64_t*)hs;
	if (v == ~0ull) return cl_fail(ctx, CL_E_INVALID, "cl_dna_batch_types: a tuple stream offset of the last reads lies outside the stream");
	*out = (uint32_t)v;
	return CL_OK;
}
void cl_dna_walked_free(DnaWalked* W) { delete W; }
void cl_dna_set_ahead(cl_dna_coder* D, DnaWalked* W) { if (D) D->ahead.reset(W); else delete W; }
cl_status cl_dna_model_read(const cl_dna_coder* D, uint32_t family, uint64_t context, uint32_t* out)
{
	cl_ctx* ctx = D->ctx;
	const FamTab& f = D->ft;
	if (family >= N_FAM || context >= f.n_ctx[family]) return cl_fail(ctx, CL_E_INVALID, "cl_dna_coder_model: no such family or context");
	if (!D->evolved.empty()) return cl_fail(ctx, CL_E_INVALID, "cl_dna_coder_model: a batch evolved ahead has changed the models");
	HIP_TRY(ctx, hipSetDevice(ctx->device));
	HIP_TRY(ctx, hipStreamSynchronize(ctx->stream));
	const uint32_t n = f.n_sym[family] + 1;
	HIP_TRY(ctx, hipMemcpy(out, D->state.p + f.state_base[family] + context * n, (size_t)n * 4, hipMemcpyDeviceToHost));
	return CL_OK;
}
void cl_dna_coder_state(const cl_dna_coder* D, uint32_t* prev_types, uint32_t* read_id) { if (prev_types) *prev_types = D->prev_types; if (read_id) *read_id = D->cur_read_id; }

cl_status cl_dna_walk_ahead(cl_ctx* ctx, cl_dna_coder* D, const cl_reads* refs, const uint8_t* d_es, const uint64_t* d_es_off, const uint32_t* d_es_ntuples, uint32_t n_reads)
{
	if (!ctx || !D || !refs || !d_es || !d_es_off || !d_es_ntuples || !n_reads) return CL_E_INVALID;
	if (!D->next_valid) return cl_fail(ctx, CL_E_INVALID, "cl_dna_walk_ahead: only while a batch is being coded");
	auto W = std::make_unique<DnaWalked>();
	CL_TRY(dna_walk(ctx, D, refs, d_es, d_es_off, d_es_ntuples, n_reads, D->next_prev_types, D->next_read_id, *W));
	D->ahead = std::move(W);
	return CL_OK;
}
void cl_dna_set_before_tail(cl_dna_coder* D, std::function<cl_status()> fn) { if (D) D->before_tail = std::move(fn); }

namespace {
cl_status dna_evolve_batch(cl_ctx* ctx, cl_dna_coder* D, const cl_reads* refs, const uint8_t* d_es, const uint64_t* d_es_off, const uint32_t* d_es_ntuples, uint32_t n_reads,
                           const uint32_t* h_part_bounds, uint32_t n_parts, std::unique_ptr<DnaWalked> Wp, uint32_t prev_types, uint32_t read_id, DnaEvolved& E)
{
	const uint64_t* inv_tab = nullptr;
	CL_TRY(cl_inv_table(ctx, &inv_tab));
	if (Wp && Wp->presorted && (Wp->part_bounds.size() != (size_t)n_parts + 1 || memcmp(Wp->part_bounds.data(), h_part_bounds, ((size_t)n_parts + 1) * 4) != 0)) Wp.reset();
	if (!Wp) { Wp = std::make_unique<DnaWalked>(); CL_TRY(dna_walk(ctx, D, refs, d_es, d_es_off, d_es_ntuples, n_reads, prev_types, read_id, *Wp)); }
	DnaWalked& W = *Wp;
	DevBuf<uint32_t> err; DEV_ALLOC(ctx, err, 1);
	HIP_TRY(ctx, hipMemsetAsync(err.p, 0, 4, ctx->stream));
	E.d_es = d_es; E.n_reads = n_reads; E.prev_types_in = prev_types; E.read_id_in = read_id; E.prev_types_out = W.prev_types_out;
	E.part_bounds.assign(h_part_bounds, h_part_bounds + n_parts + 1);
	uint32_t p0 = 0; size_t gi = 0;
	while (p0 < n_parts)
	{
		std::unique_ptr<DnaGroupPrep> GP;
		if (W.presorted) { if (gi >= W.groups.size() || !W.groups[gi] || W.groups[gi]->p0 != p0) return cl_fail(ctx, CL_E_INVALID, "cl_dna_encode: prepared groups do not match"); GP = std::move(W.groups[gi++]); }
		else { GP = std::make_unique<DnaGroupPrep>(); CL_TRY(dna_group_prepare(ctx, D, W, p0, h_part_bounds, n_parts, *GP)); }
		const uint32_t p1 = GP->p1, np = p1 - p0, ng = (np + 63) / 64;
		const uint64_t s0 = GP->s0, n_syms = GP->n_syms;
		const std::vector<uint32_t>& rank = GP->rank; const std::vector<uint32_t>& plen_r = GP->plen_r;
		auto G = std::make_unique<PendingGroup>(); G->p0 = p0; G->np = np; G->rank = rank; G->n_syms = GP->n_syms;
		G->d_gbase = std::move(GP->d_gbase); G->d_plen = std::move(GP->d_plen);
		DevBuf<uint64_t>& d_gbase = G->d_gbase; DevBuf<uint32_t>& d_plen = G->d_plen; DevBuf<triple_t>& trip = G->trip;
		DEV_ALLOC(ctx, trip, GP->trip_words);
		if (n_syms)
		{
			DevBuf<uint32_t>& sidx = GP->sidx; DevBuf<uint32_t>& seg = GP->seg; const uint64_t n_seg = GP->n_seg;
			auto models = [&](auto* gkey) -> cl_status {
				typedef std::remove_cv_t<std::remove_pointer_t<decltype(gkey)>> K;
				LAUNCHB_NAMED(ctx, "k_dna_evolve", n_syms * (12.0 + sizeof(K)), (k_dna_evolve<K>), grid_for(n_seg, 4), 256, (const FamTab*)D->d_ft.p, (const K*)gkey, (const uint32_t*)sidx.p, (const uint32_t*)seg.p,
					(uint32_t)n_seg, D->state.p, trip.p);
				HIP_TRY(ctx, hipGetLastError());
				for (int which = 0; which < 2; ++which)
				{
					DnaGroupPrep::LongPrep& L = GP->lp[which];
					const uint32_t nlr = L.n_runs, NS = which ? 32 : 8;
					if (!nlr) continue;
					DevBuf<uint32_t> d_ne, group_epoch, epochs;
					DEV_ALLOC(ctx, d_ne, nlr); DEV_ALLOC(ctx, group_epoch, L.groups + 1); DEV_ALLOC(ctx, epochs, (L.eps + 1) * (2 + 2 * NS));
					const LongRun* cr = L.runs.p; const uint64_t steps = L.steps;
					if (which == 0)
					{
						LAUNCH_NAMED(ctx, "k_long_epochs<8>", (k_long_epochs<8, K>), nlr, 64, (const FamTab*)D->d_ft.p, cr, nlr, (const K*)gkey, (const uint32_t*)L.step_pfx.p, (const uint32_t*)L.group_pfx.p,
							D->state.p, (EpochRec<8>*)epochs.p, d_ne.p, group_epoch.p, err.p);
						LAUNCHB_NAMED(ctx, "k_long_apply<8>", steps * 64 * (12.0 + sizeof(K)), (k_long_apply<8, K>), grid_for(steps * 64, 256), 256, cr, nlr, steps, (const K*)gkey, (const uint32_t*)sidx.p,
							(const uint32_t*)L.step_pfx.p, (const uint32_t*)L.group_pfx.p, (const EpochRec<8>*)epochs.p, (const uint32_t*)d_ne.p, (const uint32_t*)group_epoch.p, (const FamTab*)D->d_ft.p, trip.p);
					}
					else
					{
						LAUNCH_NAMED(ctx, "k_long_epochs<32>", (k_long_epochs<32, K>), nlr, 64, (const FamTab*)D->d_ft.p, cr, nlr, (const K*)gkey, (const uint32_t*)L.step_pfx.p, (const uint32_t*)L.group_pfx.p,
							D->state.p, (EpochRec<32>*)epochs.p, d_ne.p, group_epoch.p, err.p);
						LAUNCHB_NAMED(ctx, "k_long_apply<32>", steps * 64 * (12.0 + sizeof(K)), (k_long_apply<32, K>), grid_for(steps * 64, 256), 256, cr, nlr, steps, (const K*)gkey, (const uint32_t*)sidx.p,
							(const uint32_t*)L.step_pfx.p, (const uint32_t*)L.group_pfx.p, (const EpochRec<32>*)epochs.p, (const uint32_t*)d_ne.p, (const uint32_t*)group_epoch.p, (const FamTab*)D->d_ft.p, trip.p);
					}
					HIP_TRY(ctx, hipGetLastError());
					HIP_TRY(ctx, hipStreamSynchronize(ctx->stream));
				}
				return CL_OK;
			};
			if (W.narrow) CL_TRY(models((const uint32_t*)(W.key32.p + s0))); else CL_TRY(models((const uint64_t*)(W.key.p + s0)));
			HIP_TRY(ctx, hipStreamSynchronize(ctx->stream));
		}
		uint32_t herr = 0;
		HIP_TRY(ctx, hipMemcpy(&herr, err.p, 4, hipMemcpyDeviceToHost));
		if (herr & 8) return cl_fail(ctx, CL_E_UNSUPPORTED, "cl_dna_encode: epoch table of a long context run too small");
		if (herr) return cl_fail(ctx, CL_E_UNSUPPORTED, "cl_dna_encode: a read uses more than 64 alternative references");
		if (D->cstreams.size() < 4) { hipStream_t ns = nullptr; HIP_TRY(ctx, cl_stream_create_role(CL_ROLE_CODER, cl_level_to_prio(cl_role_level(CL_ROLE_CODER, 0)), &ns)); D->cstreams.push_back(ns); }
		G->stream = D->cstreams[D->next_cstream++ % D->cstreams.size()];
		G->out_off.resize(np + 1);
		G->out_off[0] = 0;
		for (uint32_t p = 0; p < np; ++p) { uint64_t sy = plen_r[p]; G->out_off[p + 1] = G->out_off[p] + ((sy * 18 + 7) / 8 + sy / 16 + 64 + 7) / 8 * 8; }
		DEV_ALLOC(ctx, G->tmp, G->out_off[np]);
		DEV_ALLOC(ctx, G->d_out_off, np + 1); DEV_ALLOC(ctx, G->d_size, np); DEV_ALLOC(ctx, G->d_dst_off, np);
		HIP_TRY(ctx, hipStreamSynchronize(ctx->stream));
		{
			LaunchOn on(ctx, G->stream);
			G->sync.s = G->stream;
			hipError_t e1 = hipMemcpyAsync(G->d_out_off.p, G->out_off.data(), (np + 1) * 8, hipMemcpyHostToDevice, G->stream);
			LAUNCH_RANGE_CODE(ctx, n_syms * 8.0, ng, (const triple_t*)trip.p, (const uint64_t*)d_gbase.p, (const uint32_t*)d_plen.p, np, G->tmp.p, (const uint64_t*)G->d_out_off.p, G->d_size.p, inv_tab);
			hipError_t e2 = hipGetLastError();
			HIP_TRY(ctx, e1); HIP_TRY(ctx, e2);
		}
		E.groups.push_back(std::move(G));
		p0 = p1;
	}
	return CL_OK;
}
}

cl_status cl_dna_evolve_ahead(cl_ctx* ctx, cl_dna_coder* D, const cl_reads* refs, const uint8_t* d_es, const uint64_t* d_es_off, const uint32_t* d_es_ntuples, uint32_t n_reads,
                              const uint32_t* h_part_bounds, uint32_t n_parts, DnaWalked* W)
{
	std::unique_ptr<DnaWalked> Wp(W);
	if (!ctx || !D || !refs || !d_es || !h_part_bounds || !n_parts || !W) return CL_E_INVALID;
	if (!D->next_valid || D->evolved.size() >= 4) return cl_fail(ctx, CL_E_INVALID, "cl_dna_evolve_ahead: only while a batch is being coded, at most four batches ahead");
	const uint32_t pt = D->evolved.empty() ? D->next_prev_types : D->ahead_prev_types, rid = D->evolved.empty() ? D->next_read_id : D->ahead_read_id;
	if (W->prev_types_in != pt || W->cur_read_id_in != rid || W->d_es != d_es || W->n_reads != n_reads) return cl_fail(ctx, CL_E_INVALID, "cl_dna_evolve_ahead: not the batch that follows");
	auto E = std::make_unique<DnaEvolved>();
	CL_TRY(dna_evolve_batch(ctx, D, refs, d_es, d_es_off, d_es_ntuples, n_reads, h_part_bounds, n_parts, std::move(Wp), pt, rid, *E));
	D->ahead_prev_types = E->prev_types_out; D->ahead_read_id = rid + n_reads;
	D->evolved.push_back(std::move(E));
	return CL_OK;
}

extern "C" cl_status cl_dna_encode(cl_ctx* ctx, cl_dna_coder* D, const cl_reads* refs, const uint8_t* d_es, const uint64_t* d_es_off,
                                   const uint32_t* d_es_ntuples, uint32_t n_reads, const uint32_t* h_part_bounds, uint32_t n_parts,
                                   uint8_t* d_out, uint64_t cap, uint64_t* h_part_sizes, uint64_t* n_out)
{
	if (!ctx || !D || !refs || !d_es || !d_es_off || !d_es_ntuples || !h_part_bounds || !h_part_sizes || !n_out) return cl_fail(ctx, CL_E_INVALID, "cl_dna_encode: null argument");
	HIP_TRY(ctx, hipSetDevice(ctx->device));
	for (uint32_t p = 0; p < n_parts; ++p) if (h_part_bounds[p] > h_part_bounds[p + 1]) return cl_fail(ctx, CL_E_INVALID, "cl_dna_encode: part bounds must ascend");
	if (n_parts && (h_part_bounds[0] != 0 || h_part_bounds[n_parts] != n_reads)) return cl_fail(ctx, CL_E_INVALID, "cl_dna_encode: parts must cover reads [0, n_reads)");
	*n_out = 0;
	if (!n_parts) return CL_OK;
	uint64_t written = 0;
	std::unique_ptr<DnaEvolved> Ep;
	if (!D->evolved.empty()) { Ep = std::move(D->evolved.front()); D->evolved.pop_front(); }
	if (Ep)
	{
		if (Ep->d_es != d_es || Ep->n_reads != n_reads || Ep->prev_types_in != D->prev_types || Ep->read_id_in != D->cur_read_id || Ep->part_bounds.size() != (size_t)n_parts + 1 ||
		    memcmp(Ep->part_bounds.data(), h_part_bounds, ((size_t)n_parts + 1) * 4) != 0)
			return cl_fail(ctx, CL_E_INVALID, "cl_dna_encode: the batch evolved ahead is not the one encoded next");
		D->ahead.reset();
	}
	else
	{
		std::unique_ptr<DnaWalked> Wp;
		if (D->ahead && D->ahead->d_es == d_es && D->ahead->n_reads == n_reads && D->ahead->prev_types_in == D->prev_types && D->ahead->cur_read_id_in == D->cur_read_id) Wp = std::move(D->ahead);
		D->ahead.reset();
		Ep = std::make_unique<DnaEvolved>();
		CL_TRY(dna_evolve_batch(ctx, D, refs, d_es, d_es_off, d_es_ntuples, n_reads, h_part_bounds, n_parts, std::move(Wp), D->prev_types, D->cur_read_id, *Ep));
	}
	DnaEvolved& E = *Ep;
	D->next_prev_types = E.prev_types_out; D->next_read_id = D->cur_read_id + n_reads; D->next_valid = true;
	struct NextOff { cl_dna_coder* D; ~NextOff() { D->next_valid = false; } } next_off{ D };
	auto finish_group = [&](PendingGroup& g) -> cl_status {
		HIP_TRY(ctx, hipStreamSynchronize(g.stream));
		g.sync.s = nullptr;
		std::vector<uint64_t> size_r(g.np);
		HIP_TRY(ctx, hipMemcpy(size_r.data(), g.d_size.p, g.np * 8, hipMemcpyDeviceToHost));
		for (uint32_t p = 0; p < g.np; ++p) { h_part_sizes[g.p0 + p] = size_r[g.rank[p]]; if (h_part_sizes[g.p0 + p] == ~0ULL) return cl_fail(ctx, CL_E_CAPACITY, "cl_dna_encode: internal part buffer overflow"); }
		std::vector<uint64_t> dst_off(g.np);
		uint64_t w = written;
		for (uint32_t p = 0; p < g.np; ++p) { dst_off[g.rank[p]] = w; w += h_part_sizes[g.p0 + p]; }
		if (w > cap) { *n_out = w; return cl_fail(ctx, CL_E_CAPACITY, "cl_dna_encode: output capacity " + std::to_string(cap) + " too small"); }
		HIP_TRY(ctx, hipMemcpyAsync(g.d_dst_off.p, dst_off.data(), g.np * 8, hipMemcpyHostToDevice, ctx->stream));
		LAUNCH(ctx, k_gather_bytes2, g.np, 256, (const uint8_t*)g.tmp.p, (const uint64_t*)g.d_out_off.p, (const uint64_t*)g.d_dst_off.p, (const uint64_t*)g.d_size.p, d_out);
		HIP_TRY(ctx, hipGetLastError());
		RcCheckRun check;
		if (ctx->verify_streams) CL_TRY(rc_check_launch(ctx, check, g.trip.p, g.d_gbase.p, g.d_plen.p, g.np, g.n_syms, d_out, w, w - written, g.d_dst_off.p, g.d_size.p));
		HIP_TRY(ctx, hipStreamSynchronize(ctx->stream));
		if (ctx->verify_streams) CL_TRY(rc_check_collect(ctx, check, "dna", g.trip.p, g.d_gbase.p, g.d_plen.p, d_out, dst_off, g.rank, g.p0, h_part_sizes + g.p0));
		written = w;
		return CL_OK;
	};
	if (D->before_tail)
		for (;;)
		{
			const cl_status hs = D->before_tail();
			if (hs == CL_OK) break;
			if (hs != CL_HOOK_RETRY) return hs;
			bool running = false;
			for (auto& g : E.groups) if (hipStreamQuery(g->stream) == hipErrorNotReady) running = true;
			(void)hipGetLastError();
			if (!running) break;
			std::this_thread::sleep_for(std::chrono::milliseconds(1));
		}
	for (auto& g : E.groups) CL_TRY(finish_group(*g));
	D->prev_types = E.prev_types_out;
	D->cur_read_id += n_reads;
	cl_timing_collect(ctx);
	*n_out = written;
	return CL_OK;
}
```

### colord_amd/csrc/objects.hpp

```cpp
#pragma once
#include "common.hpp"
#include <memory>

struct cl_reads {
	cl_ctx* ctx = nullptr;
	uint32_t n_reads = 0;
	uint64_t total_bases = 0, total_words = 0;
	DevBuf<uint64_t> packed;
	DevBuf<uint32_t> inv;
	DevBuf<uint64_t> word_off;
	DevBuf<uint32_t> lens;
	DevBuf<uint8_t> has_n;
};

struct cl_kmer_set {
	cl_ctx* ctx = nullptr;
	uint32_t k = 0;
	uint64_t n = 0;
	DevBuf<uint64_t> keys;
	DevBuf<uint32_t> counts;
	DevBuf<uint64_t> slots;
	uint64_t bmask = 0;
};

struct cl_kmer_lists {
	cl_ctx* ctx = nullptr;
	uint32_t n_reads = 0;
	uint64_t total = 0;
	DevBuf<uint64_t> off;
	DevBuf<uint64_t> kmers;
	DevBuf<uint32_t> ids;
	DevBuf<uint32_t> pos;
	DevBuf<uint32_t> read;
};

struct cl_index {
	cl_ctx* ctx = nullptr;
	uint32_t n_reads = 0, n_refs = 0, n_pseudo = 0;
	uint64_t n_keys = 0, n_entries = 0;
	DevBuf<uint32_t> ref_rank;
	DevBuf<uint64_t> off;
	DevBuf<uint32_t> refs;
};

uint32_t cl_part_shift(uint32_t k);
cl_status cl_key_histogram(cl_ctx* ctx, const uint64_t* d_kmers, uint64_t n, uint32_t k, std::vector<uint64_t>& h_bins);
cl_status cl_key_gather(cl_ctx* ctx, const uint64_t* d_kmers, uint64_t n, uint32_t k, uint32_t b0, uint32_t b1, uint64_t* d_out, uint64_t expect);

cl_status cl_ref_bounds(cl_ctx* ctx, const uint8_t* d_accept, uint32_t n, uint32_t ref_base, uint32_t* d_bounds, uint32_t* n_accepted);

cl_status cl_es_verify_at(cl_ctx* ctx, const cl_reads* reads, const cl_reads* refs, const uint8_t* d_es, const uint64_t* d_es_off, const uint32_t* d_es_ntuples,
                          uint64_t es_bytes, uint64_t* n_bad, uint32_t* first_bad, uint32_t* first_diff);

cl_status digest_chunk(cl_ctx* ctx, const cl_reads* reads, const cl_qual_params* qparams, const uint8_t* d_quals, const uint64_t* d_base_off, uint64_t first_read);
cl_status digest_values_chunk(cl_ctx* ctx, const cl_reads* reads, const cl_qual_params* qparams, const uint8_t* d_quals, const uint64_t* d_base_off, uint64_t first_read);
cl_status report_chunk(cl_ctx* ctx, const cl_reads* reads, const cl_qual_params* qparams, const uint8_t* d_quals, const uint64_t* d_base_off);
cl_status edit_profile_chunk(cl_ctx* ctx, const cl_reads* refs, const uint8_t* d_es, const uint64_t* d_es_off, uint32_t n_reads);
cl_status kmer_spectrum_range(cl_ctx* ctx, const uint32_t* d_head_pos, uint64_t n_heads, uint64_t n);
cl_status kmer_sketch_range(cl_ctx* ctx, const uint64_t* d_keys, const uint32_t* d_head_pos, uint64_t n_heads, uint64_t n);
cl_status overlaps_chunk(cl_ctx* ctx, const cl_reads* refs, const uint8_t* d_es, const uint64_t* d_es_off, uint32_t n_reads, uint64_t first_read, const uint32_t* d_ref_read, uint32_t n_ref_read);
cl_status overlaps_ref_reads(cl_ctx* ctx, const uint32_t* d_bounds, uint32_t n, uint32_t first_read, uint32_t* d_ref_read, uint32_t n_ref_read);
cl_status overlaps_records(cl_ctx* ctx, const cl_reads* refs, const uint8_t* d_es, const uint64_t* d_es_off, uint32_t n_reads, uint64_t first_read, DevBuf<cl_overlap>& out, uint64_t* n_out,
                           DevBuf<uint64_t>* rec_off = nullptr);
cl_status overlaps_offsets(cl_ctx* ctx, const char* who, const cl_reads* refs, const uint8_t* d_es, const uint64_t* d_es_off, uint32_t n_reads, uint32_t max_blocks, DevBuf<uint64_t>& rec_off,
                           uint64_t* n_out);
cl_status cigars_chunk(cl_ctx* ctx, const cl_reads* refs, const uint8_t* d_es, const uint64_t* d_es_off, uint32_t n_reads, uint64_t first_read, uint32_t id_limit, const uint64_t* d_rec_off,
                       uint64_t n_rec, uint64_t n_lifted);
struct MapGeom;
cl_status mappings_chunk(cl_ctx* ctx, const cl_reads* refs, const uint8_t* d_es, const uint64_t* d_es_off, uint32_t n_reads, uint64_t first_read, const MapGeom* geom);
struct cl_compressor;
cl_status pileup_chunk(cl_ctx* ctx, cl_pileup* p, const cl_reads* refs, const uint8_t* d_es, const uint64_t* d_es_off, uint32_t n_reads);
cl_status pileup_for_compressor(cl_compressor* c);
const cl_qual_params* cl_qual_coder_params(const cl_qual_coder* q);

#include <functional>
struct cl_dna_coder;
cl_status cl_dna_walk_ahead(cl_ctx* ctx, cl_dna_coder* D, const cl_reads* refs, const uint8_t* d_es, const uint64_t* d_es_off, const uint32_t* d_es_ntuples, uint32_t n_reads);
void cl_dna_set_before_tail(cl_dna_coder* D, std::function<cl_status()> fn);
struct DnaWalked;
cl_status cl_dna_prepare_batch(cl_ctx* ctx, cl_dna_coder* D, const cl_reads* refs, const uint8_t* d_es, const uint64_t* d_es_off, const uint32_t* d_es_ntuples, uint32_t n_reads,
                               uint32_t prev_types, uint32_t read_id, const uint32_t* h_part_bounds, uint32_t n_parts, DnaWalked** out, uint32_t* prev_types_out);
void cl_dna_walked_free(DnaWalked* W);
void cl_dna_set_ahead(cl_dna_coder* D, DnaWalked* W);
void cl_dna_coder_state(const cl_dna_coder* D, uint32_t* prev_types, uint32_t* read_id);
cl_status cl_dna_model_read(const cl_dna_coder* D, uint32_t family, uint64_t context, uint32_t* out);
cl_status cl_qual_model_read(const cl_qual_coder* Q, uint32_t family, uint64_t context, uint32_t* out, uint32_t cap, uint32_t* n_out);
cl_status cl_dna_batch_types(cl_ctx* ctx, const uint8_t* d_es, const uint64_t* d_es_off, uint32_t n_reads, uint64_t es_bytes, uint32_t prev_types, uint32_t* out);
struct QualPrepared;
cl_status cl_qual_prepare_batch(cl_ctx* ctx, cl_qual_coder* Q, const cl_reads* R, const uint8_t* d_quals, const uint64_t* d_qual_off,
                                const uint8_t* d_flags, const uint32_t* h_part_bounds, uint32_t n_parts, QualPrepared** out);
void cl_qual_prepared_free(QualPrepared* P);
void cl_qual_set_ahead(cl_qual_coder* Q, QualPrepared* P);
cl_status cl_dna_evolve_ahead(cl_ctx* ctx, cl_dna_coder* D, const cl_reads* refs, const uint8_t* d_es, const uint64_t* d_es_off, const uint32_t* d_es_ntuples, uint32_t n_reads,
                              const uint32_t* h_part_bounds, uint32_t n_parts, DnaWalked* W);
cl_status cl_qual_evolve_ahead(cl_ctx* ctx, cl_qual_coder* Q, const cl_reads* R, const uint8_t* d_quals, const uint64_t* d_qual_off, const uint32_t* h_part_bounds, uint32_t n_parts, QualPrepared* P);
void cl_qual_set_before_tail(cl_qual_coder* Q, std::function<cl_status()> fn);
constexpr cl_status CL_HOOK_RETRY = (cl_status)1000;
```

### colord_amd/device.py

```python
from __future__ import annotations
import ctypes as C
import numpy as np
import torch
from . import _native as N


def _check(ctx, st):
    if ctx is not None and getattr(ctx, "timing", False):
        for n, (ms, k, b, cells) in ctx.kernel_times().items():
            a = ctx.acc.setdefault(n, [0.0, 0, 0.0, 0.0])
            a[0] += ms
            a[1] += k
            a[2] += b
            a[3] += cells
    if st != N.CL_OK:
        msg = N.load().cl_last_error(ctx.h).decode() if ctx is not None and ctx.h else ""
        raise N.ColordHipError(st, msg)


def _view(ptr, n, dtype, device):
    out = torch.empty(int(n), dtype=dtype, device=device)
    if n:
        torch.cuda.synchronize(device)
        rc = _hip().hipMemcpy(C.c_void_p(out.data_ptr()), C.c_void_p(ptr), C.c_size_t(int(n) * out.element_size()), 3)
# ... 680 lines not shown

    def finish(self):
        _check(self.ctx, self.ctx.lib.cl_pileup_finish(self.h))

    def columns(self, first: int = 0, n: "int | None" = None) -> np.ndarray:
        n = self.n_pos - first if n is None else n
        out = np.zeros((n, 8), np.uint32)
        _check(self.ctx, self.ctx.lib.cl_pileup_columns(self.h, first, n, out.ctypes.data if n else None))
        return out

    def sites(self, min_depth: int = 4, min_alt: int = 3, min_permille: int = 250, cap: "int | None" = None) -> np.ndarray:
        need = C.c_uint64(0)
        args = (self.h, min_depth, min_alt, min_permille)
        if cap is None:
            st = self.ctx.lib.cl_pileup_sites(*args, None, 0, C.byref(need))
            if st not in (N.CL_OK, N.CL_E_CAPACITY):
                _check(self.ctx, st)
            cap = need.value
        out = np.zeros((cap, 12), np.uint32)
        _check(self.ctx, self.ctx.lib.cl_pileup_sites(*args, out.ctypes.data if cap else None, cap, C.byref(need)))
        return out[:need.value]

    def totals(self) -> dict:
        s = N.PileupSums()
        _check(self.ctx, self.ctx.lib.cl_pileup_totals(self.h, C.byref(s)))
        return s.as_dict()


class Reads(_Obj):
    _free = "cl_reads_free"

    @property
    def n_reads(self): return self.ctx.lib.cl_reads_count(self.h)
    @property
    def total_bases(self): return self.ctx.lib.cl_reads_total_bases(self.h)
    @property
    def total_words(self): return self.ctx.lib.cl_reads_total_words(self.h)
    def packed(self): return self._arr("cl_reads_packed", self.total_words + 1, torch.int64)
    def invalid(self): return self._arr("cl_reads_invalid", self.total_words + 1, torch.int32)
    def word_offsets(self): return self._arr("cl_reads_word_offsets", self.n_reads + 1, torch.int64)
    def lengths(self): return self._arr("cl_reads_lengths", self.n_reads, torch.int32)
    def has_n(self): return self._arr("cl_reads_has_n", self.n_reads, torch.uint8)

    def compact(self, i: int) -> bytes:
        buf = np.zeros(1 << 20, np.uint8)
        n = C.c_uint64(0)
        st = self.ctx.lib.cl_reads_compact(self.ctx.h, self.h, i, buf.ctypes.data, buf.size, C.byref(n))
        if st == N.CL_E_CAPACITY:
            buf = np.zeros(n.value, np.uint8)
            st = self.ctx.lib.cl_reads_compact(self.ctx.h, self.h, i, buf.ctypes.data, buf.size, C.byref(n))
        _check(self.ctx, st)
        return bytes(buf[:n.value])


class KmerSet(_Obj):
    _free = "cl_kmer_set_free"

    @property
    def size(self): return self.ctx.lib.cl_kmer_set_size(self.h)
    def keys(self): return self._arr("cl_kmer_set_keys", self.size, torch.int64)
    def counts(self): return self._arr("cl_kmer_set_counts", self.size, torch.int32)

    def check(self, kmers: torch.Tensor) -> torch.Tensor:
        out = torch.empty(kmers.numel(), dtype=torch.uint8, device=self.ctx.device)
        _check(self.ctx, self.ctx.lib.cl_kmer_set_check(self.ctx.h, self.h, kmers.data_ptr(), kmers.numel(), out.data_ptr()))
        return out


class KmerLists(_Obj):
    _free = "cl_kmer_lists_free"

    @property
    def n_reads(self): return self.ctx.lib.cl_kmer_lists_reads(self.h)
    @property
    def total(self): return self.ctx.lib.cl_kmer_lists_total(self.h)
    def offsets(self): return self._arr("cl_kmer_lists_offsets", self.n_reads + 1, torch.int64)
    def kmers(self): return self._arr("cl_kmer_lists_kmers", self.total, torch.int64)
    def ids(self): return self._arr("cl_kmer_lists_ids", self.total, torch.int32)
    def pos(self): return self._arr("cl_kmer_lists_pos", self.total, torch.int32)


class Index(_Obj):
    _free = "cl_index_free"

    @property
    def n_refs(self): return self.ctx.lib.cl_index_n_refs(self.h)
    @property
    def entries(self): return self.ctx.lib.cl_index_entries(self.h)


class QualCoder(_Obj):
    _free = "cl_qual_coder_free"

    def encode(self, reads: "Reads", quals: torch.Tensor, qual_off: torch.Tensor, part_bounds, flags: torch.Tensor | None = None):
        ctx = self.ctx
        pb = np.ascontiguousarray(part_bounds, dtype=np.uint32)
        n_parts = len(pb) - 1
        sizes = np.zeros(max(n_parts, 1), np.uint64)
        cap = max(4096, int(quals.numel() * 1.35) + 64 * n_parts)
        while True:
            out = torch.empty(cap, dtype=torch.uint8, device=ctx.device)
            n = C.c_uint64(0)
            st = ctx.lib.cl_qual_encode(ctx.h, self.h, reads.h, quals.data_ptr(), qual_off.data_ptr(),
                                        None if flags is None else flags.data_ptr(), pb.ctypes.data, n_parts,
                                        out.data_ptr(), cap, sizes.ctypes.data, C.byref(n))
            if st == N.CL_E_CAPACITY and n.value > cap:
                raise N.ColordHipError(st, "qual output capacity exceeded after models advanced; retry with a larger cap")
            _check(ctx, st)
            return out[:n.value], [int(x) for x in sizes[:n_parts]]

    def set_domain_symbols(self, n: int):
        _check(self.ctx, self.ctx.lib.cl_qual_coder_set_domain_symbols(self.h, n))

    def domains(self) -> list:
        return _domain_list(self.ctx, self.ctx.lib.cl_qual_coder_domains, self.h)

    def model(self, family: int, context: int) -> np.ndarray:
        out = np.zeros(257, np.uint32)
        n = C.c_uint32(0)
        _check(self.ctx, self.ctx.lib.cl_qual_coder_model(self.h, family, context, out.ctypes.data, len(out), C.byref(n)))
        return out[:n.value].copy()

    def groups(self) -> int:
        n = C.c_uint64(0)
        _check(self.ctx, self.ctx.lib.cl_qual_coder_groups(self.h, C.byref(n)))
        return n.value


def _domain_list(ctx, fn, h):
    n = C.c_uint64(0)
    st = fn(h, None, 0, C.byref(n))
    if st not in (N.CL_OK, N.CL_E_CAPACITY):
        _check(ctx, st)
    out = np.zeros(max(1, n.value), np.uint64)
    _check(ctx, fn(h, out.ctypes.data, out.size, C.byref(n)))
    return [int(x) for x in out[:n.value]]


def _overlap_records(fn, h) -> np.ndarray:
    n = C.c_uint64(0)
    st = fn(h, None, 0, C.byref(n))
    if st not in (N.CL_OK, N.CL_E_CAPACITY):
        _check(None, st)
    out = np.zeros((n.value, 12), np.uint32)
    if n.value:
        _check(None, fn(h, out.ctypes.data, n.value, C.byref(n)))
    return out[:n.value]


def _cigar_records(fn, h):
    nr, no = C.c_uint64(0), C.c_uint64(0)
    st = fn(h, None, 0, C.byref(nr), None, 0, C.byref(no))
    if st not in (N.CL_OK, N.CL_E_CAPACITY):
        _check(None, st)
    rec, ops = np.zeros(nr.value, np.uint32), np.zeros(no.value, np.uint32)
    if nr.value:
        _check(None, fn(h, rec.ctypes.data, nr.value, C.byref(nr), ops.ctypes.data if no.value else None, no.value, C.byref(no)))
    return rec[:nr.value], ops[:no.value]


class Compressor(_Obj):
    _free = "cl_compressor_free"

    def cigars(self):
        return _cigar_records(self.ctx.lib.cl_compressor_cigars, self.h)

    def overlaps(self) -> np.ndarray:
        return _overlap_records(self.ctx.lib.cl_compressor_overlaps, self.h)

    def __init__(self, ctx, h, qual_ctx, has_qual, exchange):
        super().__init__(ctx, h)
        self.qual_ctx, self.has_qual, self.exchange = qual_ctx, has_qual, exchange

    def count_add(self, reads: "Reads"):
        _check(self.ctx, self.ctx.lib.cl_compressor_count_add(self.h, reads.h))

    def count_finish(self):
        st = N.KmerStats()
        _check(self.ctx, self.ctx.lib.cl_compressor_count_finish(self.h, C.byref(st)))
        return st

    def refs_add(self, reads: "Reads"):
        _check(self.ctx, self.ctx.lib.cl_compressor_refs_add(self.h, reads.h))

    def refs_finish(self):
        _check(self.ctx, self.ctx.lib.cl_compressor_refs_finish(self.h))

    def info(self) -> dict:
        st = N.KmerStats(); a, b, m = C.c_uint64(0), C.c_uint64(0), C.c_uint64(0); r, nr = C.c_uint32(0), C.c_uint32(0)
        _check(self.ctx, self.ctx.lib.cl_compressor_info(self.h, C.byref(st), C.byref(a), C.byref(b), C.byref(m), C.byref(r), C.byref(nr)))
        return dict(tot_kmers=st.tot_kmers, n_unique_counted=st.n_unique_counted, first_read=a.value, n_reads_total=b.value, mean_read_len=m.value,
                    sparse_range=r.value, n_refs_total=nr.value)

    def verified(self):
        r, b = C.c_uint64(0), C.c_uint64(0)
        _check(None, self.ctx.lib.cl_compressor_verified(self.h, C.byref(r), C.byref(b)))
        return r.value, b.value

    def verified_streams(self):
        p, s, b = C.c_uint64(0), C.c_uint64(0), C.c_uint64(0)
        _check(None, self.ctx.lib.cl_compressor_verified_streams(self.h, C.byref(p), C.byref(s), C.byref(b)))
        return p.value, s.value, b.value

    def digest(self):
        d, q = N.Digest(), N.Digest()
        _check(None, self.ctx.lib.cl_compressor_digest(self.h, C.byref(d), C.byref(q)))
        return d.triple(), q.triple()

    def edit_profile(self) -> "N.Edits":
        e = N.Edits()
        _check(None, self.ctx.lib.cl_compressor_edit_profile(self.h, C.byref(e)))
        return e

    def report(self) -> "N.Report":
        r = N.Report()
        _check(None, self.ctx.lib.cl_compressor_report(self.h, C.byref(r)))
        return r

    def digest_values(self):
        d = N.Digest()
        _check(None, self.ctx.lib.cl_compressor_digest_values(self.h, C.byref(d)))
        return d.triple()

    def set_qual_domain_symbols(self, n: int):
        _check(self.ctx, self.ctx.lib.cl_compressor_set_qual_domain_symbols(self.h, n))

    def qual_domains(self) -> list:
        return _domain_list(self.ctx, self.ctx.lib.cl_compressor_qual_domains, self.h)

    def genome_add(self, sequences: "Reads"):
        _check(self.ctx, self.ctx.lib.cl_compressor_genome_add(self.h, sequences.h))

    def pseudo_reads(self, pseudo: "Reads"):
        _check(self.ctx, self.ctx.lib.cl_compressor_pseudo_reads(self.h, pseudo.h))

    def genome_geometry(self, seq_len, read_len: int, overlap: int):
        sl = np.ascontiguousarray(np.asarray(seq_len, dtype=np.uint64))
        _check(self.ctx, self.ctx.lib.cl_compressor_genome_geometry(self.h, sl.ctypes.data if len(sl) else None, len(sl), read_len, overlap))

    def mappings(self) -> np.ndarray:
        return _overlap_records(self.ctx.lib.cl_compressor_mappings, self.h)

    def pileup(self) -> "Pileup":
        h = N._P()
        _check(self.ctx, self.ctx.lib.cl_compressor_pileup(self.h, C.byref(h)))
        return Pileup(self.ctx, h, owned=False)

    def prepare(self, reads: "Reads", pack_bounds, part_bounds=None, quals: torch.Tensor | None = None, base_off: torch.Tensor | None = None):
        kb = np.ascontiguousarray(np.asarray(pack_bounds, dtype=np.uint32))
        if part_bounds is None:
            _check(self.ctx, self.ctx.lib.cl_compressor_prepare(self.h, reads.h, kb.ctypes.data, len(kb) - 1))
        else:
            pb = np.ascontiguousarray(np.asarray(part_bounds, dtype=np.uint32))
            _check(self.ctx, self.ctx.lib.cl_compressor_prepare_parts(self.h, reads.h, kb.ctypes.data, len(kb) - 1, pb.ctypes.data, len(pb) - 1,
                                                                      quals.data_ptr() if quals is not None else None, base_off.data_ptr() if (quals is not None and base_off is not None) else None))

    def encode(self, reads: "Reads", part_bounds, pack_bounds, quals: torch.Tensor | None = None, base_off: torch.Tensor | None = None,
               dna_out: torch.Tensor | None = None, qual_out: torch.Tensor | None = None):
        ctx = self.ctx
        pb = np.ascontiguousarray(np.asarray(part_bounds, dtype=np.uint32)); kb = np.ascontiguousarray(np.asarray(pack_bounds, dtype=np.uint32))
        npart = len(pb) - 1
        if dna_out is None:
            dna_out = torch.empty(int(reads.total_bases) + 64 * npart + 4096, dtype=torch.uint8, device=ctx.device)
        dsz, qsz = np.zeros(max(npart, 1), np.uint64), np.zeros(max(npart, 1), np.uint64)
        if self.has_qual and qual_out is None:
            qual_out = torch.empty(int(int(reads.total_bases) * 1.35) + 64 * npart + 4096, dtype=torch.uint8, device=ctx.device)
        info = N.CompressInfo()
        _check(ctx, ctx.lib.cl_compressor_encode(self.h, reads.h, quals.data_ptr() if self.has_qual else None, base_off.contiguous().data_ptr() if self.has_qual else None,
                                                 pb.ctypes.data, npart, kb.ctypes.data, len(kb) - 1, dna_out.data_ptr(), dna_out.numel(), dsz.ctypes.data,
                                                 qual_out.data_ptr() if self.has_qual else None, qual_out.numel() if self.has_qual else 0, qsz.ctypes.data, C.byref(info)))
        if self.qual_ctx is not None and self.qual_ctx is not ctx:
            _check(self.qual_ctx, N.CL_OK)
        inf = {n_: getattr(info, n_) for n_, _ in N.CompressInfo._fields_ if n_ != "pad"}
        return dna_out[:inf["dna_bytes"]], dsz[:npart], (qual_out[:inf["qual_bytes"]] if self.has_qual else None), qsz[:npart], inf


class DnaCoder(_Obj):
    _free = "cl_dna_coder_free"
    N_SYM = (3, 2, 2, 32, 256, 4, 5, 256, 0, 24, 256, 256, 8)

    def __init__(self, ctx, h, max_alt_refs):
        super().__init__(ctx, h)
        self.max_alt_refs = max_alt_refs

    def encode(self, refs: "Reads", es: torch.Tensor, es_off: torch.Tensor, es_ntuples: torch.Tensor, part_bounds):
        ctx = self.ctx
        pb = np.ascontiguousarray(part_bounds, dtype=np.uint32)
        n_parts = len(pb) - 1
        n_reads = es_off.numel() - 1
        sizes = np.zeros(max(n_parts, 1), np.uint64)
        cap = max(4096, int(es.numel() * 0.6) + 64 * n_parts)
        out = torch.empty(cap, dtype=torch.uint8, device=ctx.device)
        n = C.c_uint64(0)
        st = ctx.lib.cl_dna_encode(ctx.h, self.h, refs.h, es.data_ptr(), es_off.data_ptr(), es_ntuples.data_ptr(), n_reads,
                                   pb.ctypes.data, n_parts, out.data_ptr(), cap, sizes.ctypes.data, C.byref(n))
        _check(ctx, st)
        return out[:n.value], [int(x) for x in sizes[:n_parts]]

    def model(self, family: int, context: int) -> np.ndarray:
        out = np.zeros(257, np.uint32)
        _check(self.ctx, self.ctx.lib.cl_dna_coder_model(self.h, family, context, out.ctypes.data))
        return out[:(self.N_SYM[family] or self.max_alt_refs) + 1].copy()


class Anchors(_Obj):
    _free = "cl_anchors_free"

    def __init__(self, ctx, h, n_reads, c):
        super().__init__(ctx, h)
        self.n_reads, self.c = n_reads, c

    @property
    def total(self): return self.ctx.lib.cl_anchors_total(self.h)

    def lis_counts(self):
        lib = self.ctx.lib
        return ((lib.cl_anchors_wave_tasks(self.h), lib.cl_anchors_wave_pairs(self.h)), (lib.cl_anchors_lane_tasks(self.h), lib.cl_anchors_lane_pairs(self.h)))

    def n_cands(self): return self._arr("cl_anchors_n_cands", self.n_reads, torch.int32)
    def cands(self): return self._arr("cl_anchors_cands", self.n_reads * self.c * 4, torch.int32).view(self.n_reads, self.c, 4)
    def cand_offsets(self): return self._arr("cl_anchors_cand_offsets", self.n_reads * self.c + 1, torch.int64)
    def data(self): return self._arr("cl_anchors_data", self.total * 3, torch.int32).view(-1, 3)
```

### include/colord_hip.h

```cpp
#ifndef COLORD_HIP_H
#define COLORD_HIP_H
#include <stdint.h>
#include <stddef.h>

#ifdef __cplusplus
extern "C" {
#endif

typedef int32_t cl_status;
enum {
	CL_OK = 0,
	CL_E_INVALID = -1,
	CL_E_HIP = -2,
	CL_E_CAPACITY = -3,
	CL_E_NOMEM = -4,
	CL_E_UNSUPPORTED = -5,
	CL_E_MISMATCH = -6
};

typedef struct cl_ctx cl_ctx;
typedef struct cl_reads cl_reads;
typedef struct cl_kmer_set cl_kmer_set;
typedef struct cl_kmer_lists cl_kmer_lists;
typedef struct cl_index cl_index;

cl_status cl_ctx_create(int device, cl_ctx** out);
void cl_ctx_destroy(cl_ctx* ctx);
const char* cl_last_error(const cl_ctx* ctx);
void* cl_ctx_stream(cl_ctx* ctx);
cl_status cl_ctx_last_kernel_ms(const cl_ctx* ctx, const char* kernel, double* ms, uint32_t* launches);
cl_status cl_ctx_kernel_times(cl_ctx* ctx, char* buf, uint64_t cap, uint64_t* needed);
void cl_ctx_set_timing(cl_ctx* ctx, int on);
void cl_ctx_set_verify(cl_ctx* ctx, int on);
cl_status cl_ctx_verified(const cl_ctx* ctx, uint64_t* reads, uint64_t* bases);
void cl_ctx_set_verify_streams(cl_ctx* ctx, int on);
cl_status cl_ctx_verified_streams(const cl_ctx* ctx, uint64_t* parts, uint64_t* symbols, uint64_t* bytes);
cl_status cl_ctx_gap_paths(const cl_ctx* ctx, uint64_t* out, uint32_t cap);
typedef struct cl_digest { uint64_t reads, symbols, sum; } cl_digest;
void cl_ctx_set_digest(cl_ctx* ctx, int on);
cl_status cl_ctx_digest(const cl_ctx* ctx, cl_digest* dna, cl_digest* qual);
void cl_ctx_set_digest_values(cl_ctx* ctx, int on);
cl_status cl_ctx_digest_values(const cl_ctx* ctx, cl_digest* out);

cl_status cl_reads_pack(cl_ctx* ctx, const uint8_t* d_codes, const uint64_t* d_offsets, uint32_t n_reads,
                        int ascii, cl_reads** out);
void cl_reads_free(cl_reads* r);
uint32_t cl_reads_count(const cl_reads* r);
uint64_t cl_reads_total_bases(const cl_reads* r);
uint64_t cl_reads_total_words(const cl_reads* r);
const uint64_t* cl_reads_packed(const cl_reads* r);
const uint32_t* cl_reads_invalid(const cl_reads* r);
const uint64_t* cl_reads_word_offsets(const cl_reads* r);
const uint32_t* cl_reads_lengths(const cl_reads* r);
const uint8_t* cl_reads_has_n(const cl_reads* r);

cl_status cl_kmer_scan(cl_ctx* ctx, const cl_reads* reads, uint32_t k, uint32_t f,
                       uint64_t* d_out, uint64_t cap, uint64_t* n_out);

typedef struct {
	uint64_t n_reads;
	uint64_t tot_kmers;
	uint64_t n_unique;
	uint64_t n_unique_counted;
	uint64_t total_count_filtered;
} cl_kmer_stats;
cl_status cl_kmer_count_filter(cl_ctx* ctx, uint64_t* d_kmers, uint64_t n, uint32_t k, uint32_t ci, uint32_t cs,
                               cl_kmer_set** out, cl_kmer_stats* stats);
cl_status cl_kmer_set_create(cl_ctx* ctx, const uint64_t* d_keys, const uint32_t* d_counts, uint64_t n, uint32_t k, cl_kmer_set** out);
void cl_kmer_set_free(cl_kmer_set* s);
uint64_t cl_kmer_set_size(const cl_kmer_set* s);
const uint64_t* cl_kmer_set_keys(const cl_kmer_set* s);
const uint32_t* cl_kmer_set_counts(const cl_kmer_set* s);
cl_status cl_kmer_set_check(cl_ctx* ctx, const cl_kmer_set* s, const uint64_t* d_kmers, uint64_t n, uint8_t* d_found);

cl_status cl_accepted_kmers(cl_ctx* ctx, const cl_kmer_set* set, const cl_reads* reads, uint32_t k, uint32_t f,
                            cl_kmer_lists** out);
void cl_kmer_lists_free(cl_kmer_lists* l);
uint32_t cl_kmer_lists_reads(const cl_kmer_lists* l);
uint64_t cl_kmer_lists_total(const cl_kmer_lists* l);
const uint64_t* cl_kmer_lists_offsets(const cl_kmer_lists* l);
const uint64_t* cl_kmer_lists_kmers(const cl_kmer_lists* l);
const uint32_t* cl_kmer_lists_ids(const cl_kmer_lists* l);
const uint32_t* cl_kmer_lists_pos(const cl_kmer_lists* l);

cl_status cl_ref_accept(uint32_t n_reads, uint32_t n_pseudo, uint32_t range, double exponent, uint8_t* h_out);

cl_status cl_index_build(cl_ctx* ctx, const cl_kmer_set* set, const cl_kmer_lists* lists, const uint8_t* d_accept,
                         uint32_t n_pseudo, uint32_t max_kmer_count, cl_index** out);
cl_status cl_index_entries_of(cl_ctx* ctx, const cl_kmer_lists* lists, const uint8_t* d_accept, uint32_t ref_base,
                              uint32_t* d_ids, uint32_t* d_refs, uint64_t cap, uint64_t* n_out,
                              uint32_t* d_bounds, uint32_t* n_accepted);
cl_status cl_index_build_pairs(cl_ctx* ctx, const cl_kmer_set* set, uint32_t* d_ids, uint32_t* d_refs, uint64_t n,
                               const uint32_t* d_bounds, uint32_t n_reads, uint32_t n_refs_total,
                               uint32_t n_pseudo, uint32_t max_kmer_count, cl_index** out);
void cl_index_free(cl_index* ix);
uint32_t cl_index_n_refs(const cl_index* ix);
uint64_t cl_index_entries(const cl_index* ix);
const uint32_t* cl_index_ref_rank(const cl_index* ix);
cl_status cl_candidates(cl_ctx* ctx, const cl_index* ix, const cl_kmer_lists* lists, uint32_t max_candidates,
                        uint32_t* d_refs, uint32_t* d_votes, uint32_t* d_n);
cl_status cl_candidates_at(cl_ctx* ctx, const cl_index* ix, const cl_kmer_lists* lists, const uint32_t* d_bounds, uint32_t max_candidates,
                           uint32_t* d_refs, uint32_t* d_votes, uint32_t* d_n);
cl_status cl_candidates_common(cl_ctx* ctx, const cl_index* ix, const cl_kmer_lists* lists, uint32_t max_candidates,
                               const uint32_t* d_refs, const uint32_t* d_n,
                               uint64_t* d_common_off, uint64_t* d_common, uint64_t cap, uint64_t* n_common);

typedef struct cl_qual_coder cl_qual_coder;
typedef struct {
	int32_t mode;
	int32_t source;
	int32_t level;
	uint32_t n_fwd;
	uint32_t fwd[8];
	uint32_t n_rev;
	uint32_t rev[8];
} cl_qual_params;
cl_status cl_qual_coder_create(cl_ctx* ctx, const cl_qual_params* params, cl_qual_coder** out);
void cl_qual_coder_free(cl_qual_coder* q);
cl_ctx* cl_qual_coder_ctx(const cl_qual_coder* q);
cl_status cl_qual_encode(cl_ctx* ctx, cl_qual_coder* q, const cl_reads* reads, const uint8_t* d_quals, const uint64_t* d_qual_off,
                         const uint8_t* d_flags, const uint32_t* h_part_bounds, uint32_t n_parts,
                         uint8_t* d_out, uint64_t cap, uint64_t* h_part_sizes, uint64_t* n_out);

cl_status cl_qual_coder_set_domain_symbols(cl_qual_coder* q, uint64_t n);
cl_status cl_qual_coder_domains(const cl_qual_coder* q, uint64_t* h_first_part, uint64_t cap, uint64_t* n_out);
cl_status cl_qual_coder_model(const cl_qual_coder* q, uint32_t family, uint64_t context, uint32_t* out, uint32_t cap, uint32_t* n_out);
cl_status cl_qual_coder_groups(const cl_qual_coder* q, uint64_t* n_out);

typedef struct cl_anchors cl_anchors;
cl_status cl_anchor_candidates(cl_ctx* ctx, const cl_reads* reads, const cl_reads* refs, const uint32_t* d_cand_refs, const uint32_t* d_cand_n,
                               uint32_t c, uint32_t anchor_len, double frac_always, double frac_min, double max_matches_mult,
                               uint32_t min_anchors, cl_anchors** out);
cl_status cl_anchor_candidates_hifi(cl_ctx* ctx, const cl_reads* reads, const cl_reads* refs, const uint32_t* d_cand_refs, const uint32_t* d_cand_n,
                                    uint32_t c, uint32_t anchor_len, double frac_always, double frac_min, double max_matches_mult,
                                    uint32_t min_anchors, uint32_t kmer_len, uint32_t modulo, const uint64_t* d_common_off, const uint64_t* d_common,
                                    cl_anchors** out);
void cl_anchors_free(cl_anchors* a);
uint64_t cl_anchors_total(const cl_anchors* a);
uint64_t cl_anchors_wave_tasks(const cl_anchors* a);
uint64_t cl_anchors_wave_pairs(const cl_anchors* a);
uint64_t cl_anchors_lane_tasks(const cl_anchors* a);
uint64_t cl_anchors_lane_pairs(const cl_anchors* a);
const uint32_t* cl_anchors_n_cands(const cl_anchors* a);
const uint32_t* cl_anchors_cands(const cl_anchors* a);
const uint64_t* cl_anchors_cand_offsets(const cl_anchors* a);
const uint32_t* cl_anchors_data(const cl_anchors* a);

cl_status cl_encode_plain(cl_ctx* ctx, const cl_reads* reads, uint8_t* d_es, uint64_t cap, uint64_t* d_es_off,
                          uint32_t* d_es_ntuples, uint64_t* n_out);

cl_status cl_encode_reads(cl_ctx* ctx, const cl_reads* reads, const cl_reads* refs, const cl_anchors* anchors, uint32_t c, uint32_t anchor_len,
                          uint32_t min_part_alt, uint32_t max_rec, double cost_mult, const uint32_t* h_pack_bounds, uint32_t n_packs,
                          uint8_t* d_es, uint64_t cap, uint64_t* d_es_off, uint32_t* d_es_ntuples, uint64_t* n_out);

cl_status cl_estimator_logs(cl_ctx* ctx, const uint32_t* d_count, const uint32_t* d_total, uint64_t n, double* d_out);

cl_status cl_es_flags(cl_ctx* ctx, const cl_reads* reads, const uint8_t* d_es, const uint64_t* d_es_off, const uint64_t* d_base_off, uint8_t* d_flags);

cl_status cl_es_expand(cl_ctx* ctx, const cl_reads* refs, const uint8_t* d_es, const uint64_t* d_es_off, const uint32_t* d_es_ntuples, uint32_t n_reads,
                       uint8_t* d_codes, uint64_t cap, uint64_t* d_base_off, uint64_t* n_out);
cl_status cl_es_verify(cl_ctx* ctx, const cl_reads* reads, const cl_reads* refs, const uint8_t* d_es, const uint64_t* d_es_off, const uint32_t* d_es_ntuples,
                       uint64_t* n_bad, uint32_t* first_bad);

cl_status cl_digest_bases(cl_ctx* ctx, const cl_reads* reads, uint64_t first_read, cl_digest* acc);
cl_status cl_digest_quals(cl_ctx* ctx, const cl_qual_params* qparams, const cl_reads* reads, const uint8_t* d_quals, const uint64_t* d_qual_off,
                          uint64_t first_read, cl_digest* acc);
cl_status cl_digest_bases_host(const uint8_t* h_codes, const uint64_t* h_off, uint64_t n, uint64_t first_read, cl_digest* acc);
cl_status cl_digest_bytes_host(uint32_t kind, const uint8_t* h_bytes, const uint64_t* h_off, uint64_t n, uint64_t first_read, cl_digest* acc);
cl_status cl_digest_qual_values(cl_ctx* ctx, const cl_qual_params* qparams, const cl_reads* reads, const uint8_t* d_quals, const uint64_t* d_qual_off,
                                uint64_t first_read, cl_digest* acc);
cl_status cl_qual_values(cl_ctx* ctx, const cl_qual_params* qparams, const cl_reads* reads, const uint8_t* d_quals, const uint64_t* d_qual_off,
                         uint8_t* d_values, uint64_t cap);
cl_status cl_qual_values_host(const cl_qual_params* qparams, const uint8_t* h_quals, const uint64_t* h_off, uint64_t n, uint8_t* h_values);
cl_status cl_digest_qual_values_host(const uint8_t* h_ascii_quals, const uint64_t* h_off, uint64_t n, uint64_t first_read, cl_digest* acc);

typedef struct cl_report {
	uint64_t reads, bases, base_count[5], len_min, len_max, len_hist[33], len_bases[33];
	uint64_t has_qual, q_reads, q_symbols, mean_q_hist[96], q_joint[96][96];
} cl_report;
void cl_report_clear(cl_report* r);
void cl_report_add(cl_report* dst, const cl_report* src);
cl_status cl_report_bases(cl_ctx* ctx, const cl_reads* reads, cl_report* acc);
cl_status cl_report_quals(cl_ctx* ctx, const cl_qual_params* qparams, const cl_reads* reads, const uint8_t* d_quals, const uint64_t* d_qual_off,
                          uint64_t flush_bytes, uint32_t max_blocks, cl_report* acc);
cl_status cl_report_bases_host(const uint8_t* h_codes, const uint64_t* h_off, uint64_t n, cl_report* acc);
cl_status cl_report_quals_host(const cl_qual_params* qparams, const uint8_t* h_ascii_quals_in, const uint64_t* h_off, uint64_t n, cl_report* acc);
cl_status cl_report_values_host(const uint8_t* h_ascii_values_out, const uint64_t* h_off, uint64_t n, cl_report* acc);
void cl_ctx_set_report(cl_ctx* ctx, int on);
cl_status cl_ctx_report(const cl_ctx* ctx, cl_report* out);

typedef struct cl_edits {
	uint64_t reads, bases, kind_reads[3], kind_bases[3], kind_bytes[3], main_rev[2], tuples[8];
	uint64_t anchor_bases, anchor_len_hist[29], skip_entries, skip_entry_sum, skip_bases, skip_len_hist[29];
	uint64_t ins_base[4], del_base[4], match_base[4], sub[4][4], ins_run_hist[17], del_run_hist[17];
	uint64_t identity_hist[101], identity_none, alt_hist[65];
} cl_edits;
void cl_edits_clear(cl_edits* e);
void cl_edits_add(cl_edits* dst, const cl_edits* src);
cl_status cl_edit_profile(cl_ctx* ctx, const cl_reads* refs, const uint8_t* d_es, const uint64_t* d_es_off, uint32_t n_reads,
                          uint64_t flush_bytes, uint32_t max_blocks, cl_edits* acc);
cl_status cl_edit_profile_host(const uint8_t* h_ref_codes, const uint64_t* h_ref_off, uint32_t n_refs, const uint8_t* h_es, const uint64_t* h_es_off,
                               uint64_t n_reads, cl_edits* acc, uint64_t* bad_read, uint32_t* bad_code);
const char* cl_edit_profile_error(uint32_t code);
void cl_ctx_set_edit_profile(cl_ctx* ctx, int on);
cl_status cl_ctx_edit_profile(const cl_ctx* ctx, cl_edits* out);

#define CL_KSPEC_EXACT 4096
typedef struct cl_kspec {
	uint64_t kmers, distinct, max_count;
	uint64_t exact[CL_KSPEC_EXACT];
	uint64_t big[33], big_mass[33];
} cl_kspec;
void cl_kspec_clear(cl_kspec* s);
void cl_kspec_add(cl_kspec* dst, const cl_kspec* src);
cl_status cl_kmer_spectrum_heads(cl_ctx* ctx, const uint32_t* d_head_pos, uint64_t n_heads, uint64_t n, uint32_t max_blocks, cl_kspec* acc);
void cl_ctx_set_kmer_spectrum(cl_ctx* ctx, int on);
cl_status cl_ctx_kmer_spectrum(const cl_ctx* ctx, cl_kspec* out);

#define CL_SKETCH_MAX_SIZE (1u << 20)
typedef struct cl_sketch_entry { uint64_t hash, count; } cl_sketch_entry;
typedef struct cl_sketch cl_sketch;
uint64_t cl_sketch_hash(uint64_t kmer);
cl_status cl_sketch_create(uint32_t size, uint32_t min_count, cl_sketch** out);
void cl_sketch_free(cl_sketch* s);
cl_status cl_sketch_info(const cl_sketch* s, uint32_t* size, uint32_t* min_count, uint64_t* qualifying, uint64_t* n);
cl_status cl_sketch_entries(const cl_sketch* s, cl_sketch_entry* h_out, uint64_t cap);
cl_status cl_sketch_merge(cl_sketch* dst, const cl_sketch_entry* e, uint64_t n, uint64_t qualifying);
cl_status cl_kmer_sketch_runs(cl_ctx* ctx, const uint64_t* d_keys, const uint32_t* d_head_pos, uint64_t n_heads, uint64_t n, uint32_t max_blocks, cl_sketch* acc);
cl_status cl_ctx_set_kmer_sketch(cl_ctx* ctx, int on, uint32_t size, uint32_t min_count);
cl_status cl_ctx_kmer_sketch(const cl_ctx* ctx, cl_sketch* out);

typedef struct cl_overlap { uint32_t q, t, qlen, tlen, qs, qe, ts, te, matches, subst, anchor_bases, flags; } cl_overlap;
cl_status cl_overlaps_of(cl_ctx* ctx, const cl_reads* refs, const uint8_t* d_es, const uint64_t* d_es_off, uint32_t n_reads, uint64_t first_read,
                         const uint32_t* d_ref_read, uint32_t n_ref_read, uint32_t max_blocks, cl_overlap* d_out, uint64_t cap, uint64_t* n_out);
cl_status cl_overlaps_host(const uint8_t* h_ref_codes, const uint64_t* h_ref_off, uint32_t n_refs, const uint8_t* h_es, const uint64_t* h_es_off, uint64_t n_reads,
                           uint64_t first_read, const uint32_t* h_ref_read, uint32_t n_ref_read, cl_overlap* h_out, uint64_t cap, uint64_t* n_out, uint64_t* bad_read, uint32_t* bad_code);
void cl_ctx_set_overlaps(cl_ctx* ctx, int on);
cl_status cl_ctx_overlaps(const cl_ctx* ctx, cl_overlap* h_out, uint64_t cap, uint64_t* n_out);

cl_status cl_mappings_lift(cl_ctx* ctx, const cl_overlap* d_recs, uint64_t n, const uint64_t* h_seq_len, uint32_t n_seqs, uint32_t read_len, uint32_t overlap,
                           cl_overlap* d_out, uint64_t cap, uint64_t* n_out);
cl_status cl_mappings_lift_host(const cl_overlap* h_recs, uint64_t n, const uint64_t* h_seq_len, uint32_t n_seqs, uint32_t read_len, uint32_t overlap,
                                cl_overlap* h_out, uint64_t cap, uint64_t* n_out, uint64_t* bad_record, uint32_t* bad_code);
void cl_ctx_set_mappings(cl_ctx* ctx, int on);
cl_status cl_ctx_mappings(const cl_ctx* ctx, cl_overlap* h_out, uint64_t cap, uint64_t* n_out);

cl_status cl_cigars_of(cl_ctx* ctx, const cl_reads* refs, const uint8_t* d_es, const uint64_t* d_es_off, uint32_t n_reads, uint32_t id_limit, uint32_t max_blocks,
                       uint32_t* d_rec_ops, uint64_t rec_cap, uint64_t* n_rec, uint32_t* d_ops, uint64_t ops_cap, uint64_t* n_ops);
cl_status cl_cigars_host(const uint8_t* h_ref_codes, const uint64_t* h_ref_off, uint32_t n_refs, const uint8_t* h_es, const uint64_t* h_es_off, uint64_t n_reads, uint32_t id_limit,
                         uint32_t* h_rec_ops, uint64_t rec_cap, uint64_t* n_rec, uint32_t* h_ops, uint64_t ops_cap, uint64_t* n_ops, uint64_t* bad_read, uint32_t* bad_code);
const char* cl_cigars_error(uint32_t code);
cl_status cl_ctx_set_cigars(cl_ctx* ctx, int on);
cl_status cl_ctx_cigars(const cl_ctx* ctx, uint32_t* h_rec_ops, uint64_t rec_cap, uint64_t* n_rec, uint32_t* h_ops, uint64_t ops_cap, uint64_t* n_ops);

typedef struct cl_pileup cl_pileup;
typedef struct cl_pileup_site { uint32_t seq, pos, ref, kind, match, sub[4], del, ins, depth; } cl_pileup_site;
typedef struct cl_pileup_sums { uint64_t covered, match, sub, del, ins, ins_unplaced, reads; } cl_pileup_sums;
cl_status cl_pileup_create(cl_ctx* ctx, const cl_reads* refs, const uint64_t* h_seq_len, uint32_t n_seqs, uint32_t read_len, uint32_t overlap, cl_pileup** out);
void cl_pileup_free(cl_pileup* p);
cl_status cl_pileup_add(cl_pileup* p, const cl_reads* refs, const uint8_t* d_es, const uint64_t* d_es_off, uint32_t n_reads, uint32_t max_blocks);
cl_status cl_pileup_finish(cl_pileup* p);
cl_status cl_pileup_columns(const cl_pileup* p, uint64_t first, uint64_t n, uint32_t* h_out);
cl_status cl_pileup_sites(const cl_pileup* p, uint32_t min_depth, uint32_t min_alt, uint32_t min_permille, cl_pileup_site* h_out, uint64_t cap, uint64_t* n_out);
cl_status cl_pileup_totals(const cl_pileup* p, cl_pileup_sums* out);
uint64_t cl_pileup_positions(const cl_pileup* p);
cl_status cl_pileup_host(const uint8_t* h_ref_codes, const uint64_t* h_ref_off, uint32_t n_refs, const uint64_t* h_seq_len, uint32_t n_seqs, uint32_t read_len, uint32_t overlap,
                         const uint8_t* h_es, const uint64_t* h_es_off, uint64_t n_reads, uint32_t min_depth, uint32_t min_alt, uint32_t min_permille,
                         uint32_t* h_cols, cl_pileup_site* h_sites, uint64_t cap, uint64_t* n_sites, cl_pileup_sums* sums, uint64_t* bad_read, uint32_t* bad_code);
void cl_ctx_set_pileup(cl_ctx* ctx, int on);

typedef struct cl_dna_coder cl_dna_coder;
cl_status cl_dna_coder_create(cl_ctx* ctx, uint32_t max_alt_refs, int32_t level, uint32_t start_read_id, cl_dna_coder** out);
void cl_dna_coder_free(cl_dna_coder* d);
cl_status cl_dna_coder_model(const cl_dna_coder* d, uint32_t family, uint64_t context, uint32_t* out);
cl_status cl_dna_encode(cl_ctx* ctx, cl_dna_coder* d, const cl_reads* refs, const uint8_t* d_es, const uint64_t* d_es_off,
                        const uint32_t* d_es_ntuples, uint32_t n_reads, const uint32_t* h_part_bounds, uint32_t n_parts,
                        uint8_t* d_out, uint64_t cap, uint64_t* h_part_sizes, uint64_t* n_out);

cl_status cl_reads_select(cl_ctx* ctx, const cl_reads* src, const uint8_t* d_keep, cl_reads** out);
cl_status cl_reads_from_arena(cl_ctx* ctx, const uint64_t* d_packed, const uint32_t* d_inv, const uint32_t* d_lens, uint32_t n_reads, cl_reads** out);

typedef struct cl_id_coder cl_id_coder;
cl_status cl_id_coder_create(int32_t header_mode, cl_id_coder** out);
void cl_id_coder_free(cl_id_coder* c);
const char* cl_id_coder_error(const cl_id_coder* c);
cl_status cl_id_encode_part(cl_id_coder* c, const uint8_t* h_ids, const uint64_t* h_off, const uint8_t* h_plus, uint32_t n,
                            uint8_t* h_out, uint64_t cap, uint64_t* n_out);

typedef struct {
	uint32_t k, f, ci, cs, c;
	uint32_t anchor_len, min_part_alt, max_rec, min_anchors;
	int32_t level, source;
	int32_t sparse;
	double sparse_g, sparse_exponent;
	double cost_mult, frac_always, frac_min, max_matches_mult;
} cl_compress_params;
typedef struct {
	uint64_t n_reads, n_bases, tot_kmers, n_kept_kmers, n_refs, n_anchors, tuple_bytes, dna_bytes, qual_bytes;
	uint32_t sparse_range, pad;
} cl_compress_info;
cl_status cl_compress_shard(cl_ctx* ctx, const cl_compress_params* params, const cl_reads* reads, const uint8_t* d_quals, const uint64_t* d_base_off,
                            const uint32_t* h_part_bounds, uint32_t n_parts, const uint32_t* h_pack_bounds, uint32_t n_packs,
                            cl_dna_coder* dna, cl_qual_coder* qual,
                            uint8_t* d_dna_out, uint64_t dna_cap, uint64_t* h_dna_part_sizes,
                            uint8_t* d_qual_out, uint64_t qual_cap, uint64_t* h_qual_part_sizes, cl_compress_info* info);

typedef struct cl_compressor cl_compressor;
typedef struct {
	void* user;
	uint32_t rank, world;
	cl_status (*all_gather_host)(void* user, const uint64_t* h_vals, uint32_t n, uint64_t* h_out);
	cl_status (*all_to_all_v)(void* user, const void* d_send, const uint64_t* h_send_bytes, void* d_recv, const uint64_t* h_recv_bytes);
	cl_status (*all_gather_v)(void* user, const void* d_send, uint64_t send_bytes, void* d_recv, const uint64_t* h_recv_bytes);
} cl_exchange;
cl_status cl_compressor_create(cl_ctx* ctx, cl_ctx* qual_ctx, const cl_compress_params* params, const cl_qual_params* qparams,
                               const cl_exchange* exchange, uint64_t expected_bases, cl_compressor** out);
void cl_compressor_free(cl_compressor* c);
cl_status cl_compressor_count_add(cl_compressor* c, const cl_reads* chunk);
cl_status cl_compressor_count_finish(cl_compressor* c, cl_kmer_stats* stats);
cl_status cl_compressor_refs_add(cl_compressor* c, const cl_reads* chunk);
cl_status cl_compressor_refs_finish(cl_compressor* c);
cl_status cl_compressor_encode(cl_compressor* c, const cl_reads* chunk, const uint8_t* d_quals, const uint64_t* d_base_off,
                               const uint32_t* h_part_bounds, uint32_t n_parts, const uint32_t* h_pack_bounds, uint32_t n_packs,
                               uint8_t* d_dna_out, uint64_t dna_cap, uint64_t* h_dna_part_sizes,
                               uint8_t* d_qual_out, uint64_t qual_cap, uint64_t* h_qual_part_sizes, cl_compress_info* info);
cl_status cl_compressor_genome_add(cl_compressor* c, const cl_reads* sequences);
cl_status cl_compressor_pseudo_reads(cl_compressor* c, const cl_reads* pseudo_reads);
cl_status cl_compressor_prepare(cl_compressor* c, const cl_reads* chunk, const uint32_t* h_pack_bounds, uint32_t n_packs);
cl_status cl_compressor_prepare_parts(cl_compressor* c, const cl_reads* chunk, const uint32_t* h_pack_bounds, uint32_t n_packs, const uint32_t* h_part_bounds, uint32_t n_parts,
                                      const uint8_t* d_quals, const uint64_t* d_base_off);
cl_status cl_compressor_info(const cl_compressor* c, cl_kmer_stats* stats, uint64_t* first_read, uint64_t* n_reads_total, uint64_t* mean_read_len,
                             uint32_t* sparse_range, uint32_t* n_refs_total);
cl_status cl_compressor_verified(const cl_compressor* c, uint64_t* reads, uint64_t* bases);
cl_status cl_compressor_verified_streams(const cl_compressor* c, uint64_t* parts, uint64_t* symbols, uint64_t* bytes);
cl_status cl_compressor_digest(const cl_compressor* c, cl_digest* dna, cl_digest* qual);
cl_status cl_compressor_digest_values(const cl_compressor* c, cl_digest* out);
cl_status cl_compressor_report(const cl_compressor* c, cl_report* out);
cl_status cl_compressor_edit_profile(const cl_compressor* c, cl_edits* out);
cl_status cl_compressor_kmer_spectrum(const cl_compressor* c, cl_kspec* out);
cl_status cl_compressor_kmer_sketch(const cl_compressor* c, cl_sketch* out);
cl_status cl_compressor_overlaps(const cl_compressor* c, cl_overlap* h_out, uint64_t cap, uint64_t* n_out);
cl_status cl_compressor_genome_geometry(cl_compressor* c, const uint64_t* h_seq_len, uint32_t n_seqs, uint32_t read_len, uint32_t overlap);
cl_status cl_compressor_mappings(const cl_compressor* c, cl_overlap* h_out, uint64_t cap, uint64_t* n_out);
cl_status cl_compressor_cigars(const cl_compressor* c, uint32_t* h_rec_ops, uint64_t rec_cap, uint64_t* n_rec, uint32_t* h_ops, uint64_t ops_cap, uint64_t* n_ops);
cl_status cl_compressor_pileup(cl_compressor* c, cl_pileup** out);

cl_status cl_compressor_set_qual_domain_symbols(cl_compressor* c, uint64_t n);
cl_status cl_compressor_qual_domains(const cl_compressor* c, uint64_t* h_first_part, uint64_t cap, uint64_t* n_out);

cl_status cl_genome_encode(const uint8_t* h_codes, const uint64_t* h_off, uint32_t n_seqs, uint8_t* h_out, uint64_t cap, uint64_t* n_out);
cl_status cl_genome_decode(const uint8_t* h_in, uint64_t n_in, uint32_t n_seqs, uint8_t* h_codes, uint64_t cap, uint64_t* h_off, uint64_t* n_out);
cl_status cl_genome_md5(const uint8_t* h_codes, const uint64_t* h_off, uint32_t n_seqs, uint8_t* h_md5_16);

typedef struct cl_dna_decoder cl_dna_decoder;
typedef struct cl_qual_decoder cl_qual_decoder;
typedef struct cl_id_decoder cl_id_decoder;
cl_status cl_dna_decoder_create(uint32_t max_alt_refs, int32_t level, uint32_t start_read_id, uint32_t n_pseudo,
                                int32_t accept_all, uint32_t sparse_range, double sparse_exponent, cl_dna_decoder** out);
void cl_dna_decoder_free(cl_dna_decoder* d);
const char* cl_dna_decoder_error(const cl_dna_decoder* d);
cl_status cl_dna_decoder_add_ref(cl_dna_decoder* d, const uint8_t* h_codes, uint32_t len);
cl_status cl_dna_decoder_new_domain(cl_dna_decoder* d);
cl_status cl_dna_decode_part(cl_dna_decoder* d, const uint8_t* h_in, uint64_t n_in, uint32_t n_reads,
                             uint8_t* h_bases, uint64_t cap, uint64_t* h_off, uint64_t* n_out);
cl_status cl_qual_decoder_create(const cl_qual_params* params, cl_qual_decoder** out);
void cl_qual_decoder_free(cl_qual_decoder* q);
cl_status cl_qual_decoder_new_domain(cl_qual_decoder* q);
cl_status cl_qual_decode_part(cl_qual_decoder* q, const uint8_t* h_in, uint64_t n_in, const uint8_t* h_bases, const uint64_t* h_off,
                              uint32_t n_reads, uint8_t* h_quals);
cl_status cl_qual_decoder_set_digest(cl_qual_decoder* q, int on, uint64_t first_read);
cl_status cl_qual_decoder_digest(const cl_qual_decoder* q, cl_digest* out);
cl_status cl_qual_decode_domains(cl_ctx* ctx, const cl_qual_params* params, const cl_reads* reads, const uint8_t* d_flags,
                                 const uint8_t* d_in, uint64_t n_in, const uint32_t* h_part_bounds, const uint64_t* h_part_sizes, uint32_t n_parts,
                                 const uint32_t* h_domain_first_part, uint32_t n_domains, uint32_t max_domains_per_launch,
                                 uint8_t* d_quals, const uint64_t* d_qual_off, uint64_t quals_cap, uint8_t* d_symbols, uint64_t symbols_cap);
cl_status cl_id_decoder_create(int32_t header_mode, cl_id_decoder** out);
void cl_id_decoder_free(cl_id_decoder* c);
cl_status cl_id_decode_part(cl_id_decoder* c, const uint8_t* h_in, uint64_t n_in, uint32_t n, uint8_t* h_ids, uint64_t cap,
                            uint64_t* h_off, uint8_t* h_plus, uint64_t* n_out);

cl_status cl_reads_compact(cl_ctx* ctx, const cl_reads* reads, uint32_t read, uint8_t* h_out, uint64_t cap, uint64_t* n_out);

cl_status cl_sort_u64(cl_ctx* ctx, uint64_t* d_keys, uint64_t n, uint32_t begin_bit, uint32_t end_bit);
cl_status cl_sort_u64_u32(cl_ctx* ctx, uint64_t* d_keys, uint32_t* d_vals, uint64_t n, uint32_t begin_bit, uint32_t end_bit);
cl_status cl_sort_u32(cl_ctx* ctx, uint32_t* d_keys, uint64_t n, uint32_t begin_bit, uint32_t end_bit);
cl_status cl_sort_u32_u32(cl_ctx* ctx, uint32_t* d_keys, uint32_t* d_vals, uint64_t n, uint32_t begin_bit, uint32_t end_bit);
cl_status cl_sort_swap_u32_u32(cl_ctx* ctx, const uint32_t* d_keys_in, const uint32_t* d_vals_in, uint64_t n, uint32_t begin_bit, uint32_t end_bit,
                               uint32_t* d_keys_out, uint32_t* d_vals_out);
cl_status cl_sort_swap_u64_u32(cl_ctx* ctx, const uint64_t* d_keys_in, const uint32_t* d_vals_in, uint64_t n, uint32_t begin_bit, uint32_t end_bit,
                               uint64_t* d_keys_out, uint32_t* d_vals_out);
cl_status cl_scan_u32(cl_ctx* ctx, uint32_t* d_data, uint64_t n, uint64_t* h_total);
cl_status cl_scan_u32_u64(cl_ctx* ctx, const uint32_t* d_in, uint64_t* d_out, uint64_t n, uint64_t* h_total);
cl_status cl_run_starts_u32(cl_ctx* ctx, const uint32_t* d_keys, uint64_t n, uint32_t shift, uint32_t* d_seg, uint64_t seg_cap, uint64_t* h_n_runs);
cl_status cl_run_starts_u64(cl_ctx* ctx, const uint64_t* d_keys, uint64_t n, uint32_t shift, uint32_t* d_seg, uint64_t seg_cap, uint64_t* h_n_runs);

#ifdef __cplusplus
}
#endif
#endif
```

Baseline: 3.106.

## Classify DNA model runs and evolve short runs in tiled wave kernel

Adds a classification pass over context runs in the DNA encoder. Short runs with small alphabets are processed by a tile-based kernel that handles many runs per wave using ballots. Medium runs are compacted into length-bucketed lists and processed by a persistent grid-stride kernel. Runs whose totals would trigger rescaling fall back to the serial path. This targets poor occupancy from one wave per tiny segment, and it adds extra prep kernels, a host sync per group and fallback bookkeeping. The evolve loop also prefetches the next key/value pair.

```diff
diff --git a/colord_amd/_native.py b/colord_amd/_native.py
--- a/colord_amd/_native.py
+++ b/colord_amd/_native.py
@@ -358,6 +358,7 @@
     "cl_dna_coder_create": (C.c_int32, [_P, C.c_uint32, C.c_int32, C.c_uint32, C.POINTER(_P)]),
     "cl_dna_coder_free": (None, [_P]),
     "cl_dna_coder_model": (C.c_int32, [_P, C.c_uint32, C.c_uint64, _P]),
+    "cl_dna_coder_fallback_runs": (C.c_int32, [_P, _P]),
     "cl_dna_encode": (C.c_int32, [_P, _P, _P, _P, _P, _P, C.c_uint32, _P, C.c_uint32, _P, C.c_uint64, _P, C.POINTER(C.c_uint64)]),
     "cl_sort_u64": (C.c_int32, [_P, _P, C.c_uint64, C.c_uint32, C.c_uint32]),
     "cl_sort_u64_u32": (C.c_int32, [_P, _P, _P, C.c_uint64, C.c_uint32, C.c_uint32]),
diff --git a/colord_amd/csrc/capi.hip b/colord_amd/csrc/capi.hip
--- a/colord_amd/csrc/capi.hip
+++ b/colord_amd/csrc/capi.hip
@@ -139,6 +139,11 @@
 	if (!d || !out) return CL_E_INVALID;
 	return cl_dna_model_read(d, family, context, out);
 }
+extern "C" cl_status cl_dna_coder_fallback_runs(const cl_dna_coder* d, uint64_t* out)
+{
+	if (!d || !out) return CL_E_INVALID;
+	return cl_dna_fallback_read(d, out);
+}
 extern "C" cl_status cl_qual_coder_model(const cl_qual_coder* q, uint32_t family, uint64_t context, uint32_t* out, uint32_t cap, uint32_t* n_out)
 {
 	if (!q || !out || !n_out) return CL_E_INVALID;
diff --git a/colord_amd/csrc/dna.hip b/colord_amd/csrc/dna.hip
--- a/colord_amd/csrc/dna.hip
+++ b/colord_amd/csrc/dna.hip
@@ -710,34 +710,26 @@
 }
 
 template<typename K>
-__global__ __launch_bounds__(256) void k_dna_evolve(const FamTab* __restrict__ ftp, const K* __restrict__ skey, const uint32_t* __restrict__ sval,
-                                                   const uint32_t* __restrict__ seg_start, uint32_t n_seg, uint32_t* __restrict__ state, triple_t* __restrict__ trip)
-{
-	__shared__ uint32_t s_cnt[4][256];
-	__shared__ uint32_t s_pre[4][256];
-	const uint32_t w = threadIdx.x >> 6, lane = threadIdx.x & 63;
-	const uint32_t sg = blockIdx.x * 4 + w;
-	if (sg >= n_seg) return;
-	const uint32_t s = seg_start[sg], e = seg_start[sg + 1];
-	const FamTab& ft = *ftp;
-	const uint32_t gctx = KeyFmt<K>::ctx(skey[s]);
-	uint32_t fam = 0;
-	for (uint32_t f = 1; f < N_FAM; ++f) if (gctx >= ft.ctx_base[f]) fam = f;
+__device__ inline void evolve_run(const FamTab& ft, const K* __restrict__ skey, const uint32_t* __restrict__ sval, uint32_t s, uint32_t e, uint32_t fam, uint32_t gctx,
+                                  uint32_t* __restrict__ state, triple_t* __restrict__ trip, uint32_t* cnt, uint32_t* pre, uint32_t lane)
+{
 	const uint32_t n_sym = ft.n_sym[fam], max_total = ft.max_total[fam], adder = ft.adder[fam];
 	uint32_t* sp = state + ft.state_base[fam] + (uint64_t)(gctx - ft.ctx_base[fam]) * (n_sym + 1);
 	const uint64_t lt = (1ULL << lane) - 1;
+	K k_next = s + lane < e ? skey[s + lane] : (K)0;
+	uint32_t d_next = s + lane < e ? sval[s + lane] : 0u;
 	if (n_sym <= 8)
 	{
-		if (e - s >= ft.long_run) return;
 		uint32_t st[8]; uint32_t tot = sp[n_sym];
 #pragma unroll
 		for (uint32_t a = 0; a < 8; ++a) st[a] = a < n_sym ? sp[a] : 0u;
 		for (uint32_t j0 = s; j0 < e; j0 += 64)
 		{
 			const uint32_t j = j0 + lane; const bool valid = j < e;
+			const K k_cur = k_next; const uint32_t dst = d_next;
+			if (j0 + 64 < e && j + 64 < e) { k_next = skey[j + 64]; d_next = sval[j + 64]; }
 			uint32_t sym = 0xffu, e1 = 15u, e2 = 15u;
-			if (valid) key_decode(fam, KeyFmt<K>::payload(skey[j]), sym, e1, e2);
-			const uint32_t dst = valid ? sval[j] : 0u;
+			if (valid) key_decode(fam, KeyFmt<K>::payload(k_cur), sym, e1, e2);
 			uint64_t m[8];
 #pragma unroll
 			for (uint32_t a = 0; a < 8; ++a) m[a] = __ballot(valid && sym == a);
@@ -782,8 +774,6 @@
 		}
 		return;
 	}
-	if (n_sym <= 32 && e - s >= ft.long_run) return;
-	uint32_t* cnt = s_cnt[w]; uint32_t* pre = s_pre[w];
 #pragma unroll
 	for (uint32_t t = 0; t < 4; ++t) { uint32_t a = lane * 4 + t; cnt[a] = a < n_sym ? sp[a] : 0u; }
 	uint32_t tot = sp[n_sym];
@@ -799,8 +789,9 @@
 	for (uint32_t j0 = s; j0 < e; j0 += 64)
 	{
 		const uint32_t j = j0 + lane; const bool valid = j < e;
-		const uint32_t sym = valid ? KeyFmt<K>::payload(skey[j]) : 0u;
-		const uint32_t dst = valid ? sval[j] : 0u;
+		const uint32_t sym = valid ? KeyFmt<K>::payload(k_next) : 0u;
+		const uint32_t dst = d_next;
+		if (j0 + 64 < e && j + 64 < e) { k_next = skey[j + 64]; d_next = sval[j + 64]; }
 		const uint32_t n_here = (e - j0) < 64 ? (e - j0) : 64;
 		uint32_t start = 0;
 		while (start < n_here)
@@ -835,6 +826,225 @@
 	for (uint32_t t = 0; t < 4; ++t) { uint32_t a = lane * 4 + t; if (a < n_sym) sp[a] = cnt[a]; }
 	if (lane == 0) sp[n_sym] = tot;
 }
+__device__ inline uint32_t fam_of(const FamTab& ft, uint32_t gctx)
+{
+	uint32_t fam = 0;
+	for (uint32_t f = 1; f < N_FAM; ++f) if (gctx >= ft.ctx_base[f]) fam = f;
+	return fam;
+}
+template<typename K>
+__global__ __launch_bounds__(256) void k_dna_evolve(const FamTab* __restrict__ ftp, const K* __restrict__ skey, const uint32_t* __restrict__ sval,
+                                                   const uint32_t* __restrict__ seg_start, uint32_t n_seg, uint32_t* __restrict__ state, triple_t* __restrict__ trip)
+{
+	__shared__ uint32_t s_cnt[4][256];
+	__shared__ uint32_t s_pre[4][256];
+	const uint32_t w = threadIdx.x >> 6, lane = threadIdx.x & 63;
+	const uint32_t sg = blockIdx.x * 4 + w;
+	if (sg >= n_seg) return;
+	const uint32_t s = seg_start[sg], e = seg_start[sg + 1];
+	const FamTab& ft = *ftp;
+	const uint32_t gctx = KeyFmt<K>::ctx(skey[s]);
+	const uint32_t fam = fam_of(ft, gctx);
+	if (ft.n_sym[fam] <= 32 && e - s >= ft.long_run) return;
+	evolve_run<K>(ft, skey, sval, s, e, fam, gctx, state, trip, s_cnt[w], s_pre[w], lane);
+}
+
+struct EvRun { uint32_t s, e, fam, gctx; };
+enum { RC_LONG = 0, RC_SHORT = 1, RC_WAVE = 2 };
+enum { RC_BUCKET0 = 0, RC_N_SHORT = 32, RC_WAVE_SYMS = 33, RC_SHORT_SYMS = 34, RC_N_FB = 35, RC_N_TILES = 36, RC_CURSOR0 = 40, RC_WORDS = 72 };
+__device__ inline uint32_t run_class(const FamTab& ft, uint32_t fam, uint32_t len)
+{
+	const uint32_t ns = ft.n_sym[fam];
+	if (ns <= 32 && len >= ft.long_run) return RC_LONG;
+	return ns <= 8 && len <= 64 ? RC_SHORT : RC_WAVE;
+}
+template<typename K>
+__global__ __launch_bounds__(256) void k_run_count(const uint32_t* __restrict__ seg_start, uint32_t n_seg, const K* __restrict__ skey, const FamTab* __restrict__ ftp, unsigned long long* __restrict__ rc)
+{
+	__shared__ uint32_t l_cnt[33];
+	__shared__ unsigned long long l_syms[2];
+	if (threadIdx.x < 33) l_cnt[threadIdx.x] = 0;
+	if (threadIdx.x < 2) l_syms[threadIdx.x] = 0;
+	__syncthreads();
+	const uint32_t sg = blockIdx.x * blockDim.x + threadIdx.x;
+	if (sg < n_seg)
+	{
+		const uint32_t s = seg_start[sg], len = seg_start[sg + 1] - s;
+		const uint32_t c = run_class(*ftp, fam_of(*ftp, KeyFmt<K>::ctx(skey[s])), len);
+		if (c == RC_SHORT) { atomicAdd(&l_cnt[32], 1u); atomicAdd(&l_syms[1], (unsigned long long)len); }
+		else if (c == RC_WAVE && len) { atomicAdd(&l_cnt[31 - __clz((int)len)], 1u); atomicAdd(&l_syms[0], (unsigned long long)len); }
+	}
+	__syncthreads();
+	if (threadIdx.x < 33 && l_cnt[threadIdx.x]) atomicAdd(rc + RC_BUCKET0 + threadIdx.x, (unsigned long long)l_cnt[threadIdx.x]);
+	if (threadIdx.x < 2 && l_syms[threadIdx.x]) atomicAdd(rc + RC_WAVE_SYMS + threadIdx.x, l_syms[threadIdx.x]);
+}
+template<typename K>
+__global__ __launch_bounds__(256) void k_run_fill(const uint32_t* __restrict__ seg_start, uint32_t n_seg, const K* __restrict__ skey, const FamTab* __restrict__ ftp, unsigned long long* __restrict__ rc,
+                                                 EvRun* __restrict__ runs, uint32_t n_wave)
+{
+	__shared__ uint32_t l_cnt[32], l_base[32];
+	if (threadIdx.x < 32) l_cnt[threadIdx.x] = 0;
+	__syncthreads();
+	const uint32_t sg = blockIdx.x * blockDim.x + threadIdx.x;
+	bool wave = false; uint32_t b = 0, r = 0; EvRun R{ 0, 0, 0, 0 };
+	if (sg < n_seg)
+	{
+		R.s = seg_start[sg]; R.e = seg_start[sg + 1]; R.gctx = KeyFmt<K>::ctx(skey[R.s]); R.fam = fam_of(*ftp, R.gctx);
+		if (R.e != R.s && run_class(*ftp, R.fam, R.e - R.s) == RC_WAVE) { wave = true; b = 31 - __clz((int)(R.e - R.s)); r = atomicAdd(&l_cnt[b], 1u); }
+	}
+	__syncthreads();
+	if (threadIdx.x < 32 && l_cnt[threadIdx.x])
+	{
+		unsigned long long off = 0;
+		for (uint32_t b2 = threadIdx.x + 1; b2 < 32; ++b2) off += rc[RC_BUCKET0 + b2];
+		l_base[threadIdx.x] = (uint32_t)(off + atomicAdd(rc + RC_CURSOR0 + threadIdx.x, (unsigned long long)l_cnt[threadIdx.x]));
+	}
+	__syncthreads();
+	if (wave && l_base[b] + r < n_wave) runs[l_base[b] + r] = R;
+}
+struct ShortTile { uint32_t t, sg0, sgp, pad; };
+__device__ inline uint32_t seg_of(const uint32_t* __restrict__ seg_start, uint32_t n_seg, uint32_t pos)
+{
+	uint32_t lo = 0, hi = n_seg;
+	while (hi - lo > 1) { const uint32_t mid = (lo + hi) >> 1; if (seg_start[mid] <= pos) lo = mid; else hi = mid; }
+	return lo;
+}
+template<typename K>
+__global__ __launch_bounds__(256) void k_short_tiles(const uint32_t* __restrict__ seg_start, uint32_t n_seg, const K* __restrict__ skey, const FamTab* __restrict__ ftp, uint32_t n_tiles,
+                                                    ShortTile* __restrict__ tiles, uint32_t cap, unsigned long long* __restrict__ n_tiles_out)
+{
+	const uint32_t t = blockIdx.x * blockDim.x + threadIdx.x, lane = threadIdx.x & 63;
+	bool act = false; ShortTile T{ t, 0, 0, 0 };
+	if (t < n_tiles)
+	{
+		const uint32_t pos = t * 64;
+		T.sg0 = seg_of(seg_start, n_seg, pos);
+		for (uint32_t sg = T.sg0; sg < n_seg; ++sg)
+		{
+			const uint32_t s = seg_start[sg], e = seg_start[sg + 1];
+			if (s >= pos + 64 || e > pos + 64) break;
+			if (run_class(*ftp, fam_of(*ftp, KeyFmt<K>::ctx(skey[s])), e - s) == RC_SHORT) { act = true; break; }
+		}
+		if (act && t) T.sgp = seg_of(seg_start, n_seg, pos - 64);
+	}
+	const uint64_t m = __ballot(act);
+	uint32_t base = 0;
+	if (lane == 0 && m) base = (uint32_t)atomicAdd(n_tiles_out, (unsigned long long)__popcll(m));
+	base = __shfl(base, 0);
+	if (act) { const uint32_t i = base + (uint32_t)__popcll(m & ((1ULL << lane) - 1)); if (i < cap) tiles[i] = T; }
+}
+template<typename K>
+__global__ void k_run_stats(const uint32_t* __restrict__ seg_start, uint32_t n_seg, const K* __restrict__ skey, const FamTab* __restrict__ ftp, unsigned long long* __restrict__ out )
+{
+	const uint32_t sg = blockIdx.x * blockDim.x + threadIdx.x;
+	if (sg >= n_seg) return;
+	const uint32_t s = seg_start[sg], len = seg_start[sg + 1] - s;
+	if (!len) return;
+	const uint32_t fam = fam_of(*ftp, KeyFmt<K>::ctx(skey[s])), ns = ftp->n_sym[fam];
+	const uint32_t al = ns <= 8 ? 0u : ns <= 32 ? 1u : 2u, b = 31 - __clz((int)len);
+	atomicAdd(out + (al * 32 + b) * 2, 1ULL); atomicAdd(out + (al * 32 + b) * 2 + 1, (unsigned long long)len);
+	if (run_class(*ftp, fam, len) != RC_LONG) atomicMax(out + 192, (unsigned long long)len);
+}
+
+template<typename K>
+__global__ __launch_bounds__(256) void k_dna_evolve_runs(const FamTab* __restrict__ ftp, const K* __restrict__ skey, const uint32_t* __restrict__ sval, const EvRun* __restrict__ runs, uint32_t n_max,
+                                                        const unsigned long long* __restrict__ n_dev, uint32_t* __restrict__ state, triple_t* __restrict__ trip)
+{
+	__shared__ uint32_t s_cnt[4][256];
+	__shared__ uint32_t s_pre[4][256];
+	const uint32_t w = threadIdx.x >> 6, lane = threadIdx.x & 63;
+	uint32_t n = n_max;
+	if (n_dev) { const unsigned long long nd = *n_dev; if (nd < n) n = (uint32_t)nd; }
+	for (uint64_t i = (uint64_t)blockIdx.x * 4 + w; i < n; i += (uint64_t)gridDim.x * 4)
+	{
+		const EvRun R = runs[i];
+		evolve_run<K>(*ftp, skey, sval, R.s, R.e, R.fam, R.gctx, state, trip, s_cnt[w], s_pre[w], lane);
+		__builtin_amdgcn_wave_barrier();
+	}
+}
+
+template<typename K>
+__global__ __launch_bounds__(256) void k_dna_evolve_short(const FamTab* __restrict__ ftp, const K* __restrict__ skey, const uint32_t* __restrict__ sval, const uint32_t* __restrict__ seg_start,
+                                                         const ShortTile* __restrict__ tiles, uint32_t n_tiles_max, const unsigned long long* __restrict__ n_tiles_dev, uint32_t n_syms,
+                                                         uint32_t* __restrict__ state, triple_t* __restrict__ trip,
+                                                         EvRun* __restrict__ fb, uint32_t fb_cap, unsigned long long* __restrict__ n_fb, unsigned long long* __restrict__ fb_total)
+{
+	const uint32_t lane = threadIdx.x & 63;
+	const uint32_t ti = blockIdx.x * 4 + (threadIdx.x >> 6);
+	if (ti >= n_tiles_max || ti >= *n_tiles_dev) return;
+	const FamTab& ft = *ftp;
+	const ShortTile T = tiles[ti];
+	const uint32_t t = T.t, tile0 = t * 64;
+	struct Pos { bool valid, head; uint32_t j, s, e, fam, gctx, sym, e1, e2; };
+	auto locate = [&](uint32_t tt, uint32_t sg0) -> Pos {
+		Pos p; p.j = tt * 64 + lane; p.valid = p.j < n_syms;
+		const K key = p.valid ? skey[p.j] : (K)0;
+		p.gctx = KeyFmt<K>::ctx(key);
+		const uint32_t up = __shfl_up(p.gctx, 1);
+		p.head = seg_start[sg0] == tt * 64;
+		const uint64_t B = __ballot(p.valid && (lane == 0 ? p.head : p.gctx != up));
+		const uint32_t sg = sg0 + (uint32_t)__popcll(B & ((2ULL << lane) - 1)) - (uint32_t)(B & 1);
+		p.s = p.valid ? seg_start[sg] : 0u; p.e = p.valid ? seg_start[sg + 1] : 0u;
+		p.fam = fam_of(ft, p.gctx);
+		p.sym = 0xffu; p.e1 = p.e2 = 15u;
+		if (p.valid) key_decode(p.fam, KeyFmt<K>::payload(key), p.sym, p.e1, p.e2);
+		return p;
+	};
+	auto mine = [&](const Pos& p) { return p.valid && run_class(ft, p.fam, p.e - p.s) == RC_SHORT && p.e > tile0 && p.e - 1 - tile0 < 64; };
+	const Pos c = locate(t, T.sg0);
+	const bool cm = mine(c);
+	if (!__ballot(cm)) return;
+	uint64_t Mc[8], Mp[8];
+#pragma unroll
+	for (uint32_t a = 0; a < 8; ++a) { Mc[a] = __ballot(c.valid && c.sym == a); Mp[a] = 0; }
+	auto bits = [](uint32_t lo, uint32_t hi) -> uint64_t { return (hi >= 64 ? ~0ULL : (1ULL << hi) - 1) & ~(lo >= 64 ? ~0ULL : (1ULL << lo) - 1); };
+	auto emit = [&](const Pos& q, bool in_cur) {
+		const uint32_t ns = ft.n_sym[q.fam], max_total = ft.max_total[q.fam], adder = ft.adder[q.fam];
+		uint32_t* sp = state + ft.state_base[q.fam] + (uint64_t)(q.gctx - ft.ctx_base[q.fam]) * (ns + 1);
+		const uint32_t L = q.e - q.s, tot0 = sp[ns];
+		const bool last = q.j + 1 == q.e;
+		if (tot0 + adder * L >= max_total)
+		{
+			if (last)
+			{
+				const unsigned long long i = atomicAdd(n_fb, 1ULL);
+				atomicAdd(fb_total, 1ULL);
+				if (i < fb_cap) fb[i] = EvRun{ q.s, q.e, q.fam, q.gctx };
+			}
+			return;
+		}
+		const uint64_t mp = q.s < tile0 ? bits(q.s - (tile0 - 64), in_cur ? 64u : lane) : 0ULL;
+		const uint64_t mc = in_cur ? bits(q.s > tile0 ? q.s - tile0 : 0u, lane) : 0ULL;
+		uint32_t cum = 0, freq = 0, excl = 0, fin[8];
+#pragma unroll
+		for (uint32_t a = 0; a < 8; ++a)
+		{
+			const uint32_t v = (a < ns ? sp[a] : 0u) + adder * (uint32_t)(__popcll(Mp[a] & mp) + __popcll(Mc[a] & mc));
+			const bool ex = a == q.e1 || a == q.e2;
+			if (ex) excl += v;
+			if (a < q.sym && !ex) cum += v;
+			if (a == q.sym) freq = v;
+			fin[a] = v + (a == q.sym ? adder : 0u);
+		}
+		trip[sval[q.j]] = pack_triple(cum, freq, tot0 + adder * (q.j - q.s) - excl);
+		if (last)
+		{
+#pragma unroll
+			for (uint32_t a = 0; a < 8; ++a) if (a < ns) sp[a] = fin[a];
+			sp[ns] = tot0 + adder * L;
+		}
+	};
+	if (t != 0 && !c.head)
+	{
+		const Pos p = locate(t - 1, T.sgp);
+#pragma unroll
+		for (uint32_t a = 0; a < 8; ++a) Mp[a] = __ballot(p.valid && p.sym == a);
+		if (mine(p)) emit(p, false);
+		__builtin_amdgcn_s_waitcnt(0);
+		__builtin_amdgcn_fence(__ATOMIC_SEQ_CST, "workgroup");
+	}
+	if (cm) emit(c, true);
+}
 
 __global__ void k_init_fam_state(const FamTab* __restrict__ ftp, uint32_t fam, uint32_t* __restrict__ state)
 {
@@ -867,6 +1077,8 @@
 	DevBuf<uint32_t> sidx, seg;
 	struct LongPrep { uint32_t n_runs = 0; uint64_t steps = 0, groups = 0, eps = 0; DevBuf<LongRun> runs; DevBuf<uint32_t> step_pfx, group_pfx; } lp[2];
 	bool long_ready = false;
+	uint64_t long_syms = 0;
+	struct RunClasses { bool ready = false; uint32_t n_wave = 0, n_short = 0; uint64_t wave_syms = 0, short_syms = 0; DevBuf<EvRun> runs; DevBuf<ShortTile> tiles; uint32_t tile_cap = 0; DevBuf<unsigned long long> rc; } cls;
 };
 struct DnaWalked {
 	const uint8_t* d_es = nullptr; uint32_t n_reads = 0;
@@ -881,6 +1093,8 @@
 	DevBuf<FamTab> d_ft;
 	DevBuf<uint32_t> state;
 	uint32_t ctx_bits = 0; bool narrow = false;
+	bool run_classes = true, run_stats = false;
+	DevBuf<unsigned long long> fb_total;
 	uint32_t cur_read_id = 0;
 	uint32_t prev_types = 0;
 	uint32_t next_read_id = 0, next_prev_types = 0; bool next_valid = false;
@@ -930,8 +1144,12 @@
 	if (cb >= (1ull << 32)) return cl_fail(ctx, CL_E_UNSUPPORTED, "cl_dna_coder_create: context space too large");
 	D->ctx_bits = 1; while ((1ull << D->ctx_bits) < cb) ++D->ctx_bits;
 	D->narrow = D->ctx_bits + 8 <= 32 && !getenv("COLORD_HIP_DNA_WIDE_KEYS");
+	if (const char* v = getenv("COLORD_HIP_DNA_RUN_CLASSES")) D->run_classes = atoi(v) != 0;
+	if (const char* v = getenv("COLORD_HIP_DNA_RUN_STATS")) D->run_stats = atoi(v) != 0;
 	DEV_ALLOC(ctx, D->d_ft, 1);
 	HIP_TRY(ctx, hipMemcpyAsync(D->d_ft.p, &f, sizeof(f), hipMemcpyHostToDevice, ctx->stream));
+	DEV_ALLOC(ctx, D->fb_total, 1);
+	HIP_TRY(ctx, hipMemsetAsync(D->fb_total.p, 0, 8, ctx->stream));
 	DEV_ALLOC(ctx, D->state, sb);
 	for (uint32_t i = 0; i < N_FAM; ++i) LAUNCH(ctx, k_init_fam_state, 2048, 256, (const FamTab*)D->d_ft.p, i, D->state.p);
 	HIP_TRY(ctx, hipGetLastError());
@@ -1046,6 +1264,7 @@
 		DnaGroupPrep::LongPrep& L = G.lp[which];
 		const uint32_t nlr = nlr2[which], NS = which ? 32 : 8;
 		L.n_runs = nlr; L.steps = L.groups = L.eps = 0;
+		if (which == 0) G.long_syms = 0;
 		if (!nlr) continue;
 		std::vector<LongRun> h(nlr);
 		HIP_TRY(ctx, hipMemcpy(h.data(), runs.p + (uint64_t)which * RUN_CAP, nlr * sizeof(LongRun), hipMemcpyDeviceToHost));
@@ -1055,7 +1274,7 @@
 			const uint64_t Ln = r.e - r.s, ns = (Ln + 63) / 64, ngp = (ns + 63) / 64;
 			const uint64_t half = f.max_total[r.fam] / 2 / f.adder[r.fam];
 			r.step0 = L.steps; r.group0 = L.groups; r.epoch0 = L.eps; r.epoch_cap = (uint32_t)(Ln / (half > 80 ? half - 40 : 1) + 8);
-			L.steps += ns; L.groups += ngp; L.eps += r.epoch_cap;
+			L.steps += ns; L.groups += ngp; L.eps += r.epoch_cap; G.long_syms += Ln;
 		}
 		DEV_ALLOC(ctx, L.runs, nlr);
 		HIP_TRY(ctx, hipMemcpyAsync(L.runs.p, h.data(), nlr * sizeof(LongRun), hipMemcpyHostToDevice, ctx->stream));
@@ -1075,6 +1294,61 @@
 		HIP_TRY(ctx, hipStreamSynchronize(ctx->stream));
 	}
 	G.long_ready = true;
+	return CL_OK;
+}
+}
+
+namespace {
+template<typename K>
+cl_status dna_classes_prepare(cl_ctx* ctx, cl_dna_coder* D, const K* gkey, uint64_t n_syms, DnaGroupPrep& G)
+{
+	const uint32_t n_seg = (uint32_t)G.n_seg;
+	if (!n_seg) return CL_OK;
+	const FamTab* ftp = D->d_ft.p;
+	if (D->run_stats)
+	{
+		DevBuf<unsigned long long> st; DEV_ALLOC(ctx, st, 193);
+		HIP_TRY(ctx, hipMemsetAsync(st.p, 0, 193 * 8, ctx->stream));
+		LAUNCH_NAMED(ctx, "k_run_stats", (k_run_stats<K>), grid_for(n_seg, 256), 256, (const uint32_t*)G.seg.p, n_seg, gkey, ftp, st.p);
+		HIP_TRY(ctx, hipGetLastError());
+		std::vector<unsigned long long> h(193);
+		HIP_TRY(ctx, hipMemcpyAsync(h.data(), st.p, 193 * 8, hipMemcpyDeviceToHost, ctx->stream));
+		HIP_TRY(ctx, hipStreamSynchronize(ctx->stream));
+		std::string out = "[dna runs] n_syms " + std::to_string(n_syms) + " n_seg " + std::to_string(n_seg) + " long_run " + std::to_string(D->ft.long_run) + " longest not long " + std::to_string(h[192]) + "\n";
+		out += "[dna runs] log2  runs<=8 symbols<=8  runs<=32 symbols<=32  runs>32 symbols>32\n";
+		for (uint32_t b = 0; b < 32; ++b)
+		{
+			if (!(h[b * 2] | h[(32 + b) * 2] | h[(64 + b) * 2])) continue;
+			out += "[dna runs] " + std::to_string(b);
+			for (uint32_t al = 0; al < 3; ++al) out += "  " + std::to_string(h[(al * 32 + b) * 2]) + " " + std::to_string(h[(al * 32 + b) * 2 + 1]);
+			out += "\n";
+		}
+		fputs(out.c_str(), stderr);
+	}
+	if (!D->run_classes) return CL_OK;
+	DnaGroupPrep::RunClasses& C = G.cls;
+	DEV_ALLOC(ctx, C.rc, RC_WORDS);
+	HIP_TRY(ctx, hipMemsetAsync(C.rc.p, 0, RC_WORDS * 8, ctx->stream));
+	LAUNCH_NAMED(ctx, "k_run_count", (k_run_count<K>), grid_for(n_seg, 256), 256, (const uint32_t*)G.seg.p, n_seg, gkey, ftp, C.rc.p);
+	HIP_TRY(ctx, hipGetLastError());
+	unsigned long long h[RC_CURSOR0];
+	HIP_TRY(ctx, hipMemcpyAsync(h, C.rc.p, sizeof(h), hipMemcpyDeviceToHost, ctx->stream));
+	HIP_TRY(ctx, hipStreamSynchronize(ctx->stream));
+	uint64_t n_wave = 0;
+	for (uint32_t b = 0; b < 32; ++b) n_wave += h[RC_BUCKET0 + b];
+	if (n_wave + h[RC_N_SHORT] > n_seg) return cl_fail(ctx, CL_E_UNSUPPORTED, "cl_dna_encode: run classes hold more runs than the group");
+	C.n_wave = (uint32_t)n_wave; C.n_short = (uint32_t)h[RC_N_SHORT]; C.wave_syms = h[RC_WAVE_SYMS]; C.short_syms = h[RC_SHORT_SYMS];
+	if (C.n_wave + C.n_short) DEV_ALLOC(ctx, C.runs, (uint64_t)C.n_wave + C.n_short);
+	if (C.n_wave) LAUNCH_NAMED(ctx, "k_run_fill", (k_run_fill<K>), grid_for(n_seg, 256), 256, (const uint32_t*)G.seg.p, n_seg, gkey, ftp, C.rc.p, C.runs.p, C.n_wave);
+	if (C.n_short)
+	{
+		const uint32_t n_tiles = (uint32_t)((n_syms + 63) / 64);
+		C.tile_cap = std::min(n_tiles, C.n_short);
+		DEV_ALLOC(ctx, C.tiles, C.tile_cap);
+		LAUNCH_NAMED(ctx, "k_short_tiles", (k_short_tiles<K>), grid_for(n_tiles, 256), 256, (const uint32_t*)G.seg.p, n_seg, gkey, ftp, n_tiles, C.tiles.p, C.tile_cap, C.rc.p + RC_N_TILES);
+	}
+	HIP_TRY(ctx, hipGetLastError());
+	C.ready = true;
 	return CL_OK;
 }
 }
@@ -1131,6 +1405,7 @@
 			else CL_TRY(dev_sort_keys32_pairs(ctx, W.key32.p + s0, G.sidx.p, n_syms, 8, 8 + cbits));
 			CL_TRY(dev_run_starts_u32(ctx, W.key32.p + s0, n_syms, 8, G.seg.p, seg_cap, &G.n_seg));
 			CL_TRY(dna_long_prepare<uint32_t>(ctx, D, W.key32.p + s0, n_syms, G));
+			CL_TRY(dna_classes_prepare<uint32_t>(ctx, D, W.key32.p + s0, n_syms, G));
 		}
 		else
 		{
@@ -1138,6 +1413,7 @@
 			else CL_TRY(dev_sort_pairs(ctx, W.key.p + s0, G.sidx.p, n_syms, 8, 8 + cbits));
 			CL_TRY(dev_run_starts_u64(ctx, W.key.p + s0, n_syms, 8, G.seg.p, seg_cap, &G.n_seg));
 			CL_TRY(dna_long_prepare<uint64_t>(ctx, D, W.key.p + s0, n_syms, G));
+			CL_TRY(dna_classes_prepare<uint64_t>(ctx, D, W.key.p + s0, n_syms, G));
 		}
 	}
 	HIP_TRY(ctx, hipStreamSynchronize(ctx->stream));
@@ -1211,6 +1487,16 @@
 	HIP_TRY(ctx, hipMemcpy(out, D->state.p + f.state_base[family] + context * n, (size_t)n * 4, hipMemcpyDeviceToHost));
 	return CL_OK;
 }
+cl_status cl_dna_fallback_read(const cl_dna_coder* D, uint64_t* out)
+{
+	cl_ctx* ctx = D->ctx;
+	HIP_TRY(ctx, hipSetDevice(ctx->device));
+	HIP_TRY(ctx, hipStreamSynchronize(ctx->stream));
+	unsigned long long v = 0;
+	HIP_TRY(ctx, hipMemcpy(&v, D->fb_total.p, 8, hipMemcpyDeviceToHost));
+	*out = v;
+	return CL_OK;
+}
 void cl_dna_coder_state(const cl_dna_coder* D, uint32_t* prev_types, uint32_t* read_id) { if (prev_types) *prev_types = D->prev_types; if (read_id) *read_id = D->cur_read_id; }
 
 cl_status cl_dna_walk_ahead(cl_ctx* ctx, cl_dna_coder* D, const cl_reads* refs, const uint8_t* d_es, const uint64_t* d_es_off, const uint32_t* d_es_ntuples, uint32_t n_reads)
@@ -1255,8 +1541,20 @@
 			DevBuf<uint32_t>& sidx = GP->sidx; DevBuf<uint32_t>& seg = GP->seg; const uint64_t n_seg = GP->n_seg;
 			auto models = [&](auto* gkey) -> cl_status {
 				typedef std::remove_cv_t<std::remove_pointer_t<decltype(gkey)>> K;
-				LAUNCHB_NAMED(ctx, "k_dna_evolve", n_syms * (12.0 + sizeof(K)), (k_dna_evolve<K>), grid_for(n_seg, 4), 256, (const FamTab*)D->d_ft.p, (const K*)gkey, (const uint32_t*)sidx.p, (const uint32_t*)seg.p,
-					(uint32_t)n_seg, D->state.p, trip.p);
+				DnaGroupPrep::RunClasses& C = GP->cls;
+				if (!C.ready)
+					LAUNCHB_NAMED(ctx, "k_dna_evolve", (double)(n_syms - GP->long_syms) * (12.0 + sizeof(K)), (k_dna_evolve<K>), grid_for(n_seg, 4), 256, (const FamTab*)D->d_ft.p, (const K*)gkey, (const uint32_t*)sidx.p,
+						(const uint32_t*)seg.p, (uint32_t)n_seg, D->state.p, trip.p);
+				if (C.ready && C.n_wave)
+					LAUNCHB_NAMED(ctx, "k_dna_evolve_runs", (double)C.wave_syms * (12.0 + sizeof(K)), (k_dna_evolve_runs<K>), grid_for(C.n_wave, 4), 256, (const FamTab*)D->d_ft.p, (const K*)gkey, (const uint32_t*)sidx.p,
+						(const EvRun*)C.runs.p, C.n_wave, (const unsigned long long*)nullptr, D->state.p, trip.p);
+				if (C.ready && C.n_short)
+				{
+					LAUNCHB_NAMED(ctx, "k_dna_evolve_short", (double)C.short_syms * (12.0 + sizeof(K)), (k_dna_evolve_short<K>), grid_for(C.tile_cap, 4), 256, (const FamTab*)D->d_ft.p, (const K*)gkey,
+						(const uint32_t*)sidx.p, (const uint32_t*)seg.p, (const ShortTile*)C.tiles.p, C.tile_cap, (const unsigned long long*)(C.rc.p + RC_N_TILES), (uint32_t)n_syms, D->state.p, trip.p, C.runs.p + C.n_wave, C.n_short, C.rc.p + RC_N_FB, D->fb_total.p);
+					LAUNCH_NAMED(ctx, "k_dna_evolve_fallback", (k_dna_evolve_runs<K>), std::min(grid_for(C.n_short, 4), 16384u), 256, (const FamTab*)D->d_ft.p, (const K*)gkey, (const uint32_t*)sidx.p,
+						(const EvRun*)(C.runs.p + C.n_wave), C.n_short, (const unsigned long long*)(C.rc.p + RC_N_FB), D->state.p, trip.p);
+				}
 				HIP_TRY(ctx, hipGetLastError());
 				for (int which = 0; which < 2; ++which)
 				{
diff --git a/colord_amd/csrc/objects.hpp b/colord_amd/csrc/objects.hpp
--- a/colord_amd/csrc/objects.hpp
+++ b/colord_amd/csrc/objects.hpp
@@ -84,6 +84,7 @@
 void cl_dna_set_ahead(cl_dna_coder* D, DnaWalked* W);
 void cl_dna_coder_state(const cl_dna_coder* D, uint32_t* prev_types, uint32_t* read_id);
 cl_status cl_dna_model_read(const cl_dna_coder* D, uint32_t family, uint64_t context, uint32_t* out);
+cl_status cl_dna_fallback_read(const cl_dna_coder* D, uint64_t* out);
 cl_status cl_qual_model_read(const cl_qual_coder* Q, uint32_t family, uint64_t context, uint32_t* out, uint32_t cap, uint32_t* n_out);
 cl_status cl_dna_batch_types(cl_ctx* ctx, const uint8_t* d_es, const uint64_t* d_es_off, uint32_t n_reads, uint64_t es_bytes, uint32_t prev_types, uint32_t* out);
 struct QualPrepared;
diff --git a/colord_amd/device.py b/colord_amd/device.py
--- a/colord_amd/device.py
+++ b/colord_amd/device.py
@@ -1006,6 +1006,11 @@
         _check(self.ctx, self.ctx.lib.cl_dna_coder_model(self.h, family, context, out.ctypes.data))
         return out[:(self.N_SYM[family] or self.max_alt_refs) + 1].copy()
 
+    def fallback_runs(self) -> int:
+        n = C.c_uint64(0)
+        _check(self.ctx, self.ctx.lib.cl_dna_coder_fallback_runs(self.h, C.byref(n)))
+        return int(n.value)
+
 
 class Anchors(_Obj):
     _free = "cl_anchors_free"
diff --git a/include/colord_hip.h b/include/colord_hip.h
--- a/include/colord_hip.h
+++ b/include/colord_hip.h
@@ -273,6 +273,7 @@
 cl_status cl_dna_coder_create(cl_ctx* ctx, uint32_t max_alt_refs, int32_t level, uint32_t start_read_id, cl_dna_coder** out);
 void cl_dna_coder_free(cl_dna_coder* d);
 cl_status cl_dna_coder_model(const cl_dna_coder* d, uint32_t family, uint64_t context, uint32_t* out);
+cl_status cl_dna_coder_fallback_runs(const cl_dna_coder* d, uint64_t* out);
 cl_status cl_dna_encode(cl_ctx* ctx, cl_dna_coder* d, const cl_reads* refs, const uint8_t* d_es, const uint64_t* d_es_off,
                         const uint32_t* d_es_ntuples, uint32_t n_reads, const uint32_t* h_part_bounds, uint32_t n_parts,
                         uint8_t* d_out, uint64_t cap, uint64_t* h_part_sizes, uint64_t* n_out);
```

Result: no change. 3.091 (-0.5%).
